# skit-ai/N-Best-ASR-Transformer

Measured on AMD Instinct MI355X. Metric: utterances/sec fine-tune (bert-base, seq128, n_best=5), higher is better.
Workload: dtype bf16

## Files before the change

include/nbest_hip.h:

```cpp
#ifndef NBEST_HIP_H
#define NBEST_HIP_H

#include <stddef.h>
#include <stdint.h>

#ifdef __cplusplus
extern "C" {
#endif

#define NBEST_ABI_VERSION 1

enum { NBEST_OK = 0, NBEST_ERR_ARG = -1, NBEST_ERR_SHAPE = -2, NBEST_ERR_DTYPE = -3, NBEST_ERR_ALIGN = -4,
       NBEST_ERR_LAUNCH = -5, NBEST_ERR_WORKSPACE = -6 };
enum { NBEST_F32 = 0, NBEST_BF16 = 1 };

typedef void* nbest_stream_t;

int nbest_version(void);
int nbest_last_error(char* buf, size_t n);

int nbest_embed_ln_fwd(const int64_t* ids, const int64_t* seg, const int64_t* pos, const void* word,
                       const void* type, const void* ptab, const float* gamma, const float* beta, void* out,
                       float* stats, int64_t M, int H, float eps, int dtype, float drop_p, uint64_t seed,
                       uint32_t drop_stream, nbest_stream_t stream);
// ... 192 lines not shown

int nbest_cls_grad_scatter(const float* dcls, void* dhidden, int B, int S, int H, int dtype,
                           nbest_stream_t stream);

int nbest_stc_decode(const float* top, const float* bott, const nbest_label_space* ls,
                     const uint8_t* none_flag, int32_t* pred, int B, nbest_stream_t stream);
int nbest_stream_stamp(int32_t* flag, int32_t value, nbest_stream_t stream);

typedef struct nbest_tensor_desc {
  int64_t offset;
  int64_t numel;
  float lr;
  float wd;
  int32_t active;
  int32_t block_start;
} nbest_tensor_desc;
int nbest_bertadam_chunk(void);
int nbest_bertadam_step(float* p, float* g, float* m, float* v, void* p_lowp, const nbest_tensor_desc* descs,
                        int n_tensors, int n_blocks, float lr_mult, float b1, float b2, float eps,
                        float max_grad_norm, void* ws, size_t ws_bytes, nbest_stream_t stream);
int nbest_bertadam_norms(const float* g, const nbest_tensor_desc* descs, int n_tensors, int n_blocks, int blk_lo, int blk_hi,
                         float* partial, nbest_stream_t stream);
int nbest_bertadam_update(float* p, const float* g, float* m, float* v, void* p_lowp, const nbest_tensor_desc* descs,
                          int n_tensors, int n_blocks, int blk_lo, int blk_hi, const float* partial, float* coef,
                          float lr_mult, float b1, float b2, float eps, float max_grad_norm, nbest_stream_t stream);
enum { NBEST_ADAM_L2 = 0, NBEST_ADAMW = 1 };
int nbest_adam_clip_coef(const float* partial, int n_partial, float max_grad_norm, float* clip, nbest_stream_t stream);
int nbest_adam_update(int mode, float* p, const float* g, float* m, float* v, void* p_lowp, const nbest_tensor_desc* descs,
                      int n_tensors, int n_blocks, int blk_lo, int blk_hi, const float* clip, float lr_mult, float bc1,
                      float bc2_sqrt, double b1, double b2, float eps, nbest_stream_t stream);
int nbest_adam_step(int mode, float* p, float* g, float* m, float* v, void* p_lowp, const nbest_tensor_desc* descs,
                    int n_tensors, int n_blocks, float lr_mult, float bc1, float bc2_sqrt, double b1, double b2, float eps,
                    float max_grad_norm, void* ws, size_t ws_bytes, nbest_stream_t stream);
int nbest_ema_update(float* ema, const float* p, const nbest_tensor_desc* descs, int n_tensors, int n_blocks,
                     float one_minus_decay, nbest_stream_t stream);
int nbest_ema_exchange(float* p, float* ema, void* p_lowp, const nbest_tensor_desc* descs, int n_tensors, int n_blocks,
                       nbest_stream_t stream);
typedef struct nbest_matrix_desc {
  int64_t offset;
  int32_t rows, cols;
  int32_t tile_start, pad;
} nbest_matrix_desc;
#define NBEST_AMAX_TENSOR_WORDS 1024
int nbest_fp8_amax_fold(void* slots, void* out, int32_t n_tensors, nbest_stream_t stream);
int nbest_quantize_weights_fp8(const float* master, void* w8, void* w8t, const nbest_matrix_desc* descs, int n_matrices,
                               int n_tiles, float* inv_scale, void* ws, size_t ws_bytes, nbest_stream_t stream);
int nbest_transpose_weights(const void* src, void* dst, const nbest_matrix_desc* descs, int n_matrices, int n_tiles,
                            nbest_stream_t stream);
int nbest_pack_bn(int64_t N);
int nbest_pack_bn_fp8(int64_t N, int64_t K);
int nbest_pack_weights_fp8(const void* src, void* dst, const nbest_matrix_desc* descs, int n_matrices, int n_stages, nbest_stream_t stream);
int nbest_pack_weights(const void* src, void* dst, const nbest_matrix_desc* descs, int n_matrices, int n_stages, nbest_stream_t stream);
int nbest_cast_f32_to_bf16(const float* src, void* dst, int64_t n, nbest_stream_t stream);

typedef struct nbest_layer_offsets {
  int64_t wqkv, bqkv, wo, bo, ln1_g, ln1_b, w1, b1, w2, b2, ln2_g, ln2_b;
} nbest_layer_offsets;
typedef struct nbest_encoder_desc {
  int32_t dtype, B, S, H, L, heads, F;
  int32_t vocab, max_pos, n_types;
  float ln_eps, hidden_drop, attn_drop;
  int64_t word_pad_id, pos_pad_id;
  int64_t off_word, off_pos, off_type, off_emb_ln_g, off_emb_ln_b;
  const nbest_layer_offsets* layers_host;
  uint64_t seed;
  uint32_t drop_stream_base;
  int32_t wgrad_events_n;
  void** wgrad_events;
  const void* w8;
  const float* w8_inv_scale;
  const void* w8t;
  const uint32_t* gamax_prev;
  uint32_t* gamax_new;
  int32_t fp8_bwd;
  int32_t pad2;
  const void* wpk;
  const void* wpkt;
  const void* w8p;
  const void* w8tp;
  const int32_t* word_perm;
  const uint32_t* aamax_prev;
  uint32_t* aamax_new;
  int32_t fp8_act;
  int32_t pad4;
  int32_t first_trainable;
  int32_t no_input_grad;
  const uint8_t* wgrad_skip_host;
  const float* head_gate;
  float* head_gate_grad;
  const int64_t* base_ids;
  const float* alpha;
  int32_t no_param_grad;
  int32_t wgrad_group;
} nbest_encoder_desc;
enum { NBEST_WGRAD_GROUP_PLAN = 0, NBEST_WGRAD_GROUP_NEVER = 1, NBEST_WGRAD_GROUP_ALWAYS = 2, NBEST_WGRAD_GROUP_WINDOW = 3 };
size_t nbest_encoder_act_bytes(const nbest_encoder_desc* d);
int nbest_encoder_act_view(const nbest_encoder_desc* d, void* act, int layer, void** qkv, float** lse);
size_t nbest_encoder_ws_bytes(const nbest_encoder_desc* d);
int nbest_encoder_wgrad_launches_per_layer(const nbest_encoder_desc* d);
int nbest_encoder_wgrad_plan(const nbest_encoder_desc* d, int layer_begin, int layer_end, int32_t* out, int cap);
int nbest_encoder_forward(const nbest_encoder_desc* d, const void* wts, const float* prm, const int64_t* ids,
                          const int64_t* seg, const int64_t* pos, const uint8_t* key_mask, void* act,
                          size_t act_bytes, void* ws, size_t ws_bytes, void** hidden_out, nbest_stream_t stream);
int nbest_encoder_backward(const nbest_encoder_desc* d, const void* wts, const void* wts_t, const float* prm, float* grad,
                           const int64_t* ids, const int64_t* seg, const int64_t* pos, const uint8_t* key_mask,
                           void* act, size_t act_bytes, void* dhidden, void* ws, size_t ws_bytes, int accumulate,
                           int layer_begin, int layer_end, int with_embeddings, nbest_stream_t stream);

size_t nbest_encoder_infer_ws_bytes(const nbest_encoder_desc* d);
int nbest_encoder_infer(const nbest_encoder_desc* d, const void* wts, const float* prm, const int64_t* ids, const int64_t* seg,
                        const int64_t* pos, const uint8_t* key_mask, void* ws, size_t ws_bytes, void* cls_out, nbest_stream_t stream);
int nbest_encoder_infer_attn(const nbest_encoder_desc* d, const void* wts, const float* prm, const int64_t* ids, const int64_t* seg,
                             const int64_t* pos, const uint8_t* key_mask, void* ws, size_t ws_bytes, void* cls_out, float* cls_attn,
                             nbest_stream_t stream);

#ifdef __cplusplus
}
#endif
#endif
```

n-best-asr-transformer_amd/csrc/attention.hip:

```cpp
#include "common.h"

namespace {

__device__ __forceinline__ int crow(int reg, int hh) { return (reg & 3) + 8 * (reg >> 2) + 4 * hh; }
__device__ __forceinline__ int gsw(int row) { return ((row >> 2) & 3) | (((row >> 1) & 1) << 2); }

__global__ __launch_bounds__(128) void attn_fwd_f32_kernel(const float* __restrict__ qkv, const uint8_t* __restrict__ mask,
                                                           float* __restrict__ ctx, float* __restrict__ lse, int S, int heads,
                                                           int H, float scale, DropCfg drop) {
  const int bh = blockIdx.x, b = bh / heads, h = bh - b * heads;
  const int i = blockIdx.y * blockDim.x + threadIdx.x;
  if (i >= S) return;
  const int64_t ld = 3 * (int64_t)H;
  const float* base = qkv + (int64_t)b * S * ld;
  const float* qp = base + i * ld + h * 64;
  float q[64];
#pragma unroll
  for (int d = 0; d < 64; ++d) q[d] = qp[d];
  float mx = -INFINITY, l = 0.f;
  for (int j = 0; j < S; ++j) {
    if (!mask[b * S + j]) continue;
    const float* kp = base + j * ld + H + h * 64;
    float s = 0.f;
#pragma unroll
// ... 1017 lines not shown
      for (int r = 0; r < 16; ++r) { ck0 += dk0[r]; ck1 += dk1[r]; cv0 += dv0[r]; cv1 += dv1[r]; }
      const int r0 = key0 + 32 * wave;
      const int64_t goff = ((int64_t)b * S + r0) * ld + h * 64;
      bf16* g = dqkv ? dqkv + goff : nullptr;
      uint8_t* g8 = f8.out8 ? f8.out8 + goff : nullptr;
      store_tile(Kt + wave * 4096, 0, dk0, dk1, lane, g ? g + H : nullptr, ld, S - r0, g8 ? g8 + H : nullptr, s8, amax8, am);
      store_tile(Kt + wave * 4096, 0, dv0, dv1, lane, g ? g + 2 * H : nullptr, ld, S - r0, g8 ? g8 + 2 * H : nullptr, s8, amax8, am);
    }
  }
  __syncthreads();
  if (colpart) {
    float* cs = (float*)dSb;
    float cq0 = 0.f, cq1 = 0.f;
#pragma unroll
    for (int r = 0; r < 16; ++r) { cq0 += dqa0[r] + dqb0[r]; cq1 += dqa1[r] + dqb1[r]; }
    float v6[6] = {cq0, cq1, ck0, ck1, cv0, cv1};
#pragma unroll
    for (int t6 = 0; t6 < 6; ++t6) {
      float x = v6[t6];
      x += __shfl_xor(x, 32, 64);
      if (lane < 32) cs[(wave * 3 + (t6 >> 1)) * 64 + (t6 & 1) * 32 + lane] = x;
    }
    __syncthreads();
    if (tid < 192) {
      const int which = tid >> 6, dcol = tid & 63;
      float x = 0.f;
#pragma unroll
      for (int w2 = 0; w2 < NW; ++w2) x += cs[(w2 * 3 + which) * 64 + dcol];
      colpart[(int64_t)b * 3 * H + which * H + h * 64 + dcol] = x;
    }
  }
  if (wave < nkb) {
    const int r0 = 32 * wave;
    const int64_t goff = ((int64_t)b * S + r0) * ld + h * 64;
    store_tile(Kt + wave * 4096, 0, dqa0, dqa1, lane, dqkv ? dqkv + goff : nullptr, ld, S - r0, f8.out8 ? f8.out8 + goff : nullptr, s8, amax8, am);
  }
  if (wave + 8 < nkb) {
    const int r0 = 32 * (wave + 8);
    const int64_t goff = ((int64_t)b * S + r0) * ld + h * 64;
    store_tile(Kt + wave * 4096, 0, dqb0, dqb1, lane, dqkv ? dqkv + goff : nullptr, ld, S - r0, f8.out8 ? f8.out8 + goff : nullptr, s8, amax8, am);
  }
  if (f8.amax_new) {
    amax8 = wave_max(amax8);
    if (lane == 0) amax_update(f8.amax_new, amax8);
  }
}

static size_t bwd2_lds_bytes(int nkb) {
  const int Sp = nkb * 32;
  return (size_t)Sp * 128 * 4 + (size_t)Sp * 8 + (size_t)nkb * Sp * 4;
}
template <int NKB>
static void launch_bwd2(const bf16* qkv, const uint8_t* mask, const bf16* ctx, const bf16* dctx, const float* lse, bf16* dqkv,
                        float* colpart, int B, int S, int heads, int H, float scale, DropCfg d, hipStream_t st, Fp8Grad f8,
                        const uint32_t* keep) {
  const size_t sm = bwd2_lds_bytes(NKB);
  if (keep && d.thr16) {
    (void)hipFuncSetAttribute((const void*)attn_bwd2_bf16_kernel<NKB, true>, hipFuncAttributeMaxDynamicSharedMemorySize, (int)sm);
    attn_bwd2_bf16_kernel<NKB, true><<<B * heads, (NKB <= 4 ? 4 : 8) * 64, sm, st>>>(qkv, mask, ctx, dctx, lse, dqkv, colpart, S, heads, H, scale, d, f8, keep);
  } else {
    (void)hipFuncSetAttribute((const void*)attn_bwd2_bf16_kernel<NKB, false>, hipFuncAttributeMaxDynamicSharedMemorySize, (int)sm);
    attn_bwd2_bf16_kernel<NKB, false><<<B * heads, (NKB <= 4 ? 4 : 8) * 64, sm, st>>>(qkv, mask, ctx, dctx, lse, dqkv, colpart, S, heads, H, scale, d, f8, nullptr);
  }
}

static size_t fwd_lds_bytes(int nkb) {
  const size_t kv = (size_t)nkb * 32 * 256, madd = (size_t)nkb * 32 * 4;
  return (nkb <= 4) ? kv + madd : kv + madd + 4 * 4096;
}

template <int NKB>
static void launch_fwd(const bf16* qkv, const uint8_t* mask, bf16* ctx, float* lse, int B, int S, int heads, int H, float scale,
                       DropCfg d, hipStream_t st, uint8_t* ctx8, uint32_t* keep, const uint32_t* a_prev, uint32_t* a_new) {
  const size_t sm = fwd_lds_bytes(NKB);
  if (d.thr16) {
    (void)hipFuncSetAttribute((const void*)attn_fwd_bf16_kernel<NKB, true>, hipFuncAttributeMaxDynamicSharedMemorySize, (int)sm);
    attn_fwd_bf16_kernel<NKB, true><<<B * heads, 256, sm, st>>>(qkv, mask, ctx, lse, S, heads, H, scale, d, ctx8, keep, a_prev, a_new);
  } else {
    (void)hipFuncSetAttribute((const void*)attn_fwd_bf16_kernel<NKB, false>, hipFuncAttributeMaxDynamicSharedMemorySize, (int)sm);
    attn_fwd_bf16_kernel<NKB, false><<<B * heads, 256, sm, st>>>(qkv, mask, ctx, lse, S, heads, H, scale, d, ctx8, keep, a_prev, a_new);
  }
}

template <typename T, bool PROBS>
__global__ __launch_bounds__(256) void attn_cls_fwd_kernel(const T* __restrict__ q, int64_t ldq, const T* __restrict__ kv, int64_t ldkv,
                                                           const uint8_t* __restrict__ mask, T* __restrict__ ctx, int64_t ldctx, int S,
                                                           int heads, int H, float scale, float* __restrict__ probs, int64_t ldp) {
  constexpr bool kF32 = sizeof(T) == 4;
  constexpr int VEC = 16 / (int)sizeof(T);
  constexpr int LPK = 64 / VEC;
  constexpr int KPP = 256 / LPK;
  __shared__ float sc[512];
  __shared__ float qs[64];
  __shared__ float part[KPP][65];
  __shared__ float red[8];
  const int tid = threadIdx.x, sub = tid % LPK, kg = tid / LPK, lane = tid & 63, wave = tid >> 6;
  const int bh = blockIdx.x, b = bh / heads, h = bh - b * heads;
  auto load = [](const T* p, float* v) {
    if constexpr (kF32) {
      const f32x4 x = *(const f32x4*)p;
#pragma unroll
      for (int e = 0; e < 4; ++e) v[e] = x[e];
    } else {
      const bf16x8 x = __builtin_bit_cast(bf16x8, *(const i32x4*)p);
#pragma unroll
      for (int e = 0; e < 8; ++e) v[e] = (float)x[e];
    }
  };
  if (tid < 64) qs[tid] = (float)q[(int64_t)b * ldq + h * 64 + tid];
  __syncthreads();
  const T* kbase = kv + (int64_t)b * S * ldkv + h * 64;
  const T* vbase = kbase + H;
  const uint8_t* mk = mask + (int64_t)b * S;
  const bool log2u = !kF32 && S <= 256;
  const float sf = log2u ? scale * 1.4426950408889634f : scale;
  float mloc = -INFINITY;
  for (int j = tid; j < S; j += 256) {
    const T* kp = kbase + (int64_t)j * ldkv;
    float d = 0.f;
#pragma unroll
    for (int c = 0; c < 64; c += VEC) {
      float kr[VEC];
      load(kp + c, kr);
#pragma unroll
      for (int e = 0; e < VEC; ++e) d = fmaf(qs[c + e], kr[e], d);
    }
    const float sv = mk[j] ? d * sf : -INFINITY;
    sc[j] = sv;
    mloc = fmaxf(mloc, sv);
  }
  mloc = wave_max(mloc);
  if (lane == 0) red[wave] = mloc;
  __syncthreads();
  const float mx = fmaxf(fmaxf(red[0], red[1]), fmaxf(red[2], red[3]));
  const float mxs = (mx == -INFINITY) ? 0.f : mx;
  auto ex = [&](float v) { return log2u ? __builtin_amdgcn_exp2f(v - mxs) : (kF32 ? expf(v - mxs) : __expf(v - mxs)); };
  float sum = 0.f;
  for (int j = tid; j < S; j += 256) sum += ex(sc[j]);
  sum = wave_sum(sum);
  if (lane == 0) red[4 + wave] = sum;
  __syncthreads();
  sum = (red[4] + red[5]) + (red[6] + red[7]);
  const float lse = mxs + logf(sum), inv = 1.0f / sum;
  if constexpr (PROBS) {
    float* pr = probs + (int64_t)bh * ldp;
    for (int j = tid; j < S; j += 256) {
      const float v = sc[j];
      pr[j] = (v == -INFINITY) ? 0.f : (kF32 ? expf(v - lse) : ex(v) * inv);
    }
    return;
  }
  for (int j = tid; j < S; j += 256) {
    const float v = sc[j];
    sc[j] = kF32 ? (v == -INFINITY ? 0.f : expf(v - lse)) : (float)(bf16)(ex(v) * inv);
  }
  __syncthreads();
  float o[VEC];
#pragma unroll
  for (int e = 0; e < VEC; ++e) o[e] = 0.f;
#pragma unroll 4
  for (int j = kg; j < S; j += KPP) {
    float vr[VEC];
    load(vbase + (int64_t)j * ldkv + sub * VEC, vr);
    const float pv = sc[j];
#pragma unroll
    for (int e = 0; e < VEC; ++e) o[e] = fmaf(pv, vr[e], o[e]);
  }
#pragma unroll
  for (int e = 0; e < VEC; ++e) part[kg][sub * VEC + e] = o[e];
  __syncthreads();
  if (tid < 64) {
    float acc = 0.f;
#pragma unroll
    for (int g = 0; g < KPP; ++g) acc += part[g][tid];
    T* op = ctx + (int64_t)b * ldctx + h * 64 + tid;
    if constexpr (kF32) *op = acc;
    else *op = (bf16)acc;
  }
}

template <bool VEC>
__global__ __launch_bounds__(256) void attn_probs_bf16_kernel(const bf16* __restrict__ qkv, const uint8_t* __restrict__ mask,
                                                              const float* __restrict__ lse, float* __restrict__ probs, int S,
                                                              int heads, int H, float scale) {
  constexpr int LDI = 68;
  __shared__ __attribute__((aligned(16))) float img[4][16 * LDI];
  const int tid = threadIdx.x, lane = tid & 63, wave = tid >> 6, c = lane & 15, g = lane >> 4;
  const int bh = blockIdx.x, b = bh / heads, h = bh - b * heads;
  const int q0 = 64 * blockIdx.y + 16 * wave;
  if (q0 >= S) return;
  const int64_t ld = 3 * (int64_t)H;
  const bf16* base = qkv + (int64_t)b * S * ld;
  const uint8_t* mk = mask + (int64_t)b * S;
  float* im = img[wave];
  const int qrow = q0 + c;
  bf16x8 qf[2];
#pragma unroll
  for (int ks = 0; ks < 2; ++ks) {
    const i32x4 raw = (qrow < S) ? *(const i32x4*)(base + (int64_t)qrow * ld + h * 64 + 32 * ks + 8 * g) : i32x4{0, 0, 0, 0};
    qf[ks] = __builtin_bit_cast(bf16x8, raw);
  }
  const float lq = (qrow < S) ? lse[(int64_t)bh * S + qrow] : 0.f;
  float* out = probs + (int64_t)bh * S * S;
  const int nkb = (S + 63) / 64;
  for (int kb = 0; kb < nkb; ++kb) {
    f32x4 acc[4];
#pragma unroll
    for (int t = 0; t < 4; ++t) {
      const int key = 64 * kb + 16 * t + c;
      acc[t] = f32x4{0.f, 0.f, 0.f, 0.f};
#pragma unroll
      for (int ks = 0; ks < 2; ++ks) {
        const i32x4 raw = (key < S) ? *(const i32x4*)(base + (int64_t)key * ld + H + h * 64 + 32 * ks + 8 * g) : i32x4{0, 0, 0, 0};
        acc[t] = __builtin_amdgcn_mfma_f32_16x16x32_bf16(__builtin_bit_cast(bf16x8, raw), qf[ks], acc[t], 0, 0, 0);
      }
    }
#pragma unroll
    for (int t = 0; t < 4; ++t) {
      f32x4 p;
#pragma unroll
      for (int r = 0; r < 4; ++r) {
        const int key = 64 * kb + 16 * t + 4 * g + r;
        p[r] = (key < S && mk[key]) ? expf(acc[t][r] * scale - lq) : 0.f;
      }
      *(f32x4*)(im + c * LDI + 16 * t + 4 * g) = p;
    }
    asm volatile("s_waitcnt lgkmcnt(0)" ::: "memory");
#pragma unroll
    for (int i = 0; i < 4; ++i) {
      const int row = 4 * i + g, q = q0 + row, key = 64 * kb + 4 * c;
      const f32x4 v = *(const f32x4*)(im + row * LDI + 4 * c);
      if (q < S && key < S) {
        float* dst = out + (int64_t)q * S + key;
        if (VEC) {
          *(f32x4*)dst = v;
        } else {
#pragma unroll
          for (int e = 0; e < 4; ++e)
            if (key + e < S) dst[e] = v[e];
        }
      }
    }
    asm volatile("s_waitcnt lgkmcnt(0)" ::: "memory");
  }
}

template <bool VEC>
__global__ __launch_bounds__(256) void attn_probs_f32_kernel(const float* __restrict__ qkv, const uint8_t* __restrict__ mask,
                                                             const float* __restrict__ lse, float* __restrict__ probs, int S, int heads,
                                                             int H, float scale) {
  const int bh = blockIdx.x, b = bh / heads, h = bh - b * heads;
  const int n4 = (S + 3) / 4;
  const int idx = blockIdx.y * 256 + threadIdx.x;
  if (idx >= S * n4) return;
  const int i = idx / n4, j0 = 4 * (idx - i * n4);
  const int64_t ld = 3 * (int64_t)H;
  const float* base = qkv + (int64_t)b * S * ld;
  const float* qp = base + i * ld + h * 64;
  float q[64];
#pragma unroll
  for (int d = 0; d < 64; d += 4) {
    const f32x4 x = *(const f32x4*)(qp + d);
    q[d] = x[0]; q[d + 1] = x[1]; q[d + 2] = x[2]; q[d + 3] = x[3];
  }
  const float lse_i = lse[(int64_t)bh * S + i];
  f32x4 p;
#pragma unroll
  for (int e = 0; e < 4; ++e) {
    const int j = j0 + e;
    float pv = 0.f;
    if (j < S && mask[b * S + j]) {
      const float* kp = base + j * ld + H + h * 64;
      float s = 0.f;
#pragma unroll
      for (int d = 0; d < 64; ++d) s = fmaf(q[d], kp[d], s);
      pv = expf(s * scale - lse_i);
    }
    p[e] = pv;
  }
  float* dst = probs + ((int64_t)bh * S + i) * S + j0;
  if (VEC) {
    *(f32x4*)dst = p;
  } else {
#pragma unroll
    for (int e = 0; e < 4; ++e)
      if (j0 + e < S) dst[e] = p[e];
  }
}

static int check_common(const char* who, int B, int S, int heads, int d, int dtype) {
  NB_CHECK(B > 0 && S > 0 && heads > 0, NBEST_ERR_SHAPE, "%s: bad shape", who);
  NB_CHECK(d == 64, NBEST_ERR_SHAPE, "%s: head dimension %d not supported (64 only)", who, d);
  NB_CHECK(dtype == NBEST_F32 || dtype == NBEST_BF16, NBEST_ERR_DTYPE, "%s: bad dtype %d", who, dtype);
  NB_CHECK((int64_t)B * heads * S * S < ((int64_t)1 << 32), NBEST_ERR_SHAPE, "%s: B*heads*S*S overflows the dropout counter", who);
  return NBEST_OK;
}

}

size_t nbest_internal_attention_keep_bytes(int B, int S, int heads) {
  const size_t nkb = (size_t)(S + 31) / 32;
  return (S <= 256) ? (size_t)B * heads * nkb * nkb * 32 * sizeof(uint32_t) : 0;
}
int nbest_internal_attention_fwd8(const void* qkv, const uint8_t* key_mask, void* ctx, void* ctx8, float* lse, int B, int S, int heads,
                                  int d, int dtype, float drop_p, uint64_t seed, uint32_t drop_stream, nbest_stream_t stream,
                                  uint32_t* keep, const uint32_t* a_prev, uint32_t* a_new) {
  NB_CHECK(qkv && key_mask && ctx && lse, NBEST_ERR_ARG, "attention_fwd: null pointer");
  if (int e = check_common("attention_fwd", B, S, heads, d, dtype)) return e;
  hipStream_t st = (hipStream_t)stream;
  const int H = heads * d;
  const float scale = 1.0f / sqrtf((float)d);
  const DropCfg dc = make_drop(drop_p, seed, drop_stream);
  if (dtype == NBEST_F32) {
    NB_CHECK(S <= 512, NBEST_ERR_SHAPE, "attention_fwd(f32): S=%d > 512", S);
    attn_fwd_f32_kernel<<<dim3(B * heads, (S + 127) / 128), 128, 0, st>>>((const float*)qkv, key_mask, (float*)ctx, lse, S, heads, H, scale, dc);
  } else {
    NB_CHECK(S <= 512, NBEST_ERR_SHAPE, "attention_fwd(bf16): S=%d > 512", S);
    NB_CHECK((int64_t)S * 3 * H * 2 < ((int64_t)1 << 31), NBEST_ERR_SHAPE, "attention_fwd: sequence too large");
    const int nkb = (S + 31) / 32;
    if (nkb > 8) {
      const size_t sm = fwd_lds_bytes(nkb);
      (void)hipFuncSetAttribute((const void*)attn_fwd_long_bf16_kernel, hipFuncAttributeMaxDynamicSharedMemorySize, (int)sm);
      attn_fwd_long_bf16_kernel<<<B * heads, 256, sm, st>>>((const bf16*)qkv, key_mask, (bf16*)ctx, lse, S, nkb, heads, H, scale, dc, (uint8_t*)ctx8, a_prev, a_new);
      NB_LAUNCH_CHECK();
      return NBEST_OK;
    }
#define F(N) case N: launch_fwd<N>((const bf16*)qkv, key_mask, (bf16*)ctx, lse, B, S, heads, H, scale, dc, st, (uint8_t*)ctx8, keep, a_prev, a_new); break;
    switch (nkb) { F(1) F(2) F(3) F(4) F(5) F(6) F(7) F(8) }
#undef F
  }
  NB_LAUNCH_CHECK();
  return NBEST_OK;
}

extern "C" int nbest_attention_fwd(const void* qkv, const uint8_t* key_mask, void* ctx, float* lse, int B, int S, int heads,
                                   int d, int dtype, float drop_p, uint64_t seed, uint32_t drop_stream, nbest_stream_t stream) {
  return nbest_internal_attention_fwd8(qkv, key_mask, ctx, nullptr, lse, B, S, heads, d, dtype, drop_p, seed, drop_stream, stream, nullptr, nullptr, nullptr);
}

int nbest_attention_cls_fwd_internal(const void* q, int64_t ldq, const void* kv, int64_t ldkv, const uint8_t* key_mask, void* ctx,
                                     int64_t ldctx, int B, int S, int heads, int d, int dtype, nbest_stream_t stream) {
  NB_CHECK(q && kv && key_mask && ctx, NBEST_ERR_ARG, "attention_cls_fwd: null pointer");
  NB_CHECK(B > 0 && S > 0 && heads > 0, NBEST_ERR_SHAPE, "attention_cls_fwd: bad shape");
  NB_CHECK(d == 64, NBEST_ERR_SHAPE, "attention_cls_fwd: head dimension %d not supported (64 only)", d);
  NB_CHECK(dtype == NBEST_F32 || dtype == NBEST_BF16, NBEST_ERR_DTYPE, "attention_cls_fwd: bad dtype %d", dtype);
  NB_CHECK(S <= 512, NBEST_ERR_SHAPE, "attention_cls_fwd: S=%d > 512", S);
  const int H = heads * d;
  const int vec = dtype == NBEST_BF16 ? 8 : 4;
  NB_CHECK(ldq >= H && ldkv >= 2 * H && ldctx >= H && ldq % vec == 0 && ldkv % vec == 0, NBEST_ERR_ALIGN,
           "attention_cls_fwd: leading dimensions must cover the heads and be multiples of %d elements", vec);
  NB_CHECK(((uintptr_t)q & 15) == 0 && ((uintptr_t)kv & 15) == 0, NBEST_ERR_ALIGN, "attention_cls_fwd: q and kv must be 16-byte aligned");
  const float scale = 1.0f / sqrtf((float)d);
  hipStream_t st = (hipStream_t)stream;
  if (dtype == NBEST_F32)
    attn_cls_fwd_kernel<float, false><<<B * heads, 256, 0, st>>>((const float*)q, ldq, (const float*)kv, ldkv, key_mask, (float*)ctx, ldctx, S,
                                                                 heads, H, scale, nullptr, 0);
  else
    attn_cls_fwd_kernel<bf16, false><<<B * heads, 256, 0, st>>>((const bf16*)q, ldq, (const bf16*)kv, ldkv, key_mask, (bf16*)ctx, ldctx, S,
                                                                heads, H, scale, nullptr, 0);
  NB_LAUNCH_CHECK();
  return NBEST_OK;
}

extern "C" int nbest_attention_cls_fwd(const void* q, int64_t ldq, const void* kv, int64_t ldkv, const uint8_t* key_mask, void* ctx,
                                       int64_t ldctx, int B, int S, int heads, int d, int dtype, nbest_stream_t stream) {
  return nbest_attention_cls_fwd_internal(q, ldq, kv, ldkv, key_mask, ctx, ldctx, B, S, heads, d, dtype, stream);
}

extern "C" int nbest_attention_probs(const void* qkv, const uint8_t* key_mask, const float* lse, float* probs, int B, int S, int heads,
                                     int d, int dtype, nbest_stream_t stream) {
  NB_CHECK(qkv && key_mask && lse && probs, NBEST_ERR_ARG, "attention_probs: null pointer");
  if (int e = check_common("attention_probs", B, S, heads, d, dtype)) return e;
  NB_CHECK(S <= 512, NBEST_ERR_SHAPE, "attention_probs: S=%d > 512", S);
  NB_CHECK(((uintptr_t)qkv & 15) == 0, NBEST_ERR_ALIGN, "attention_probs: qkv must be 16-byte aligned");
  hipStream_t st = (hipStream_t)stream;
  const int H = heads * d;
  const float scale = 1.0f / sqrtf((float)d);
  const bool vec = (S % 4) == 0 && ((uintptr_t)probs & 15) == 0;
  if (dtype == NBEST_F32) {
    const dim3 grid(B * heads, (S * ((S + 3) / 4) + 255) / 256);
    if (vec) attn_probs_f32_kernel<true><<<grid, 256, 0, st>>>((const float*)qkv, key_mask, lse, probs, S, heads, H, scale);
    else attn_probs_f32_kernel<false><<<grid, 256, 0, st>>>((const float*)qkv, key_mask, lse, probs, S, heads, H, scale);
  } else {
    const dim3 grid(B * heads, (S + 63) / 64);
    if (vec) attn_probs_bf16_kernel<true><<<grid, 256, 0, st>>>((const bf16*)qkv, key_mask, lse, probs, S, heads, H, scale);
    else attn_probs_bf16_kernel<false><<<grid, 256, 0, st>>>((const bf16*)qkv, key_mask, lse, probs, S, heads, H, scale);
  }
  NB_LAUNCH_CHECK();
  return NBEST_OK;
}

int nbest_internal_attention_cls_probs(const void* q, int64_t ldq, const void* kv, int64_t ldkv, const uint8_t* key_mask, float* probs,
                                       int64_t ldp, int B, int S, int heads, int d, int dtype, nbest_stream_t stream) {
  NB_CHECK(q && kv && key_mask && probs, NBEST_ERR_ARG, "attention_cls_probs: null pointer");
  NB_CHECK(B > 0 && S > 0 && heads > 0, NBEST_ERR_SHAPE, "attention_cls_probs: bad shape");
  NB_CHECK(d == 64, NBEST_ERR_SHAPE, "attention_cls_probs: head dimension %d not supported (64 only)", d);
  NB_CHECK(dtype == NBEST_F32 || dtype == NBEST_BF16, NBEST_ERR_DTYPE, "attention_cls_probs: bad dtype %d", dtype);
  NB_CHECK(S <= 512, NBEST_ERR_SHAPE, "attention_cls_probs: S=%d > 512", S);
  const int H = heads * d;
  const int vec = dtype == NBEST_BF16 ? 8 : 4;
  NB_CHECK(ldq >= H && ldkv >= 2 * H && ldp >= S && ldq % vec == 0 && ldkv % vec == 0, NBEST_ERR_ALIGN,
           "attention_cls_probs: leading dimensions must cover the heads / keys and be multiples of %d elements", vec);
  NB_CHECK(((uintptr_t)q & 15) == 0 && ((uintptr_t)kv & 15) == 0, NBEST_ERR_ALIGN, "attention_cls_probs: q and kv must be 16-byte aligned");
  const float scale = 1.0f / sqrtf((float)d);
  hipStream_t st = (hipStream_t)stream;
  if (dtype == NBEST_F32)
    attn_cls_fwd_kernel<float, true><<<B * heads, 256, 0, st>>>((const float*)q, ldq, (const float*)kv, ldkv, key_mask, nullptr, 0, S,
                                                                heads, H, scale, probs, ldp);
  else
    attn_cls_fwd_kernel<bf16, true><<<B * heads, 256, 0, st>>>((const bf16*)q, ldq, (const bf16*)kv, ldkv, key_mask, nullptr, 0, S,
                                                               heads, H, scale, probs, ldp);
  NB_LAUNCH_CHECK();
  return NBEST_OK;
}

extern "C" int nbest_attention_cls_probs(const void* q, int64_t ldq, const void* kv, int64_t ldkv, const uint8_t* key_mask, float* probs,
                                         int64_t ldp, int B, int S, int heads, int d, int dtype, nbest_stream_t stream) {
  return nbest_internal_attention_cls_probs(q, ldq, kv, ldkv, key_mask, probs, ldp, B, S, heads, d, dtype, stream);
}

extern "C" size_t nbest_attention_bwd_ws_bytes(int B, int S, int heads) {
  const size_t a = (size_t)B * 3 * heads * 64 * sizeof(float);
  const size_t b = nbest_rowred_ws_bytes((int64_t)B * S, (int64_t)3 * heads * 64);
  return a > b ? a : b;
}

int nbest_internal_attention_bwd8(const void* qkv, const uint8_t* key_mask, const void* ctx, const void* dctx, const float* lse,
                                  void* dqkv, float* dbias, int accumulate, void* ws, size_t ws_bytes, int B, int S, int heads,
                                  int d, int dtype, float drop_p, uint64_t seed, uint32_t drop_stream, nbest_stream_t stream, Fp8Grad f8,
                                  const uint32_t* keep) {
  NB_CHECK(qkv && key_mask && ctx && dctx && lse && (dqkv || (f8.out8 && dtype == NBEST_BF16)), NBEST_ERR_ARG, "attention_bwd: null pointer");
  if (int e = check_common("attention_bwd", B, S, heads, d, dtype)) return e;
  NB_CHECK(!dbias || (ws && ws_bytes >= nbest_attention_bwd_ws_bytes(B, S, heads)), NBEST_ERR_WORKSPACE,
           "attention_bwd: bias-gradient workspace too small");
  hipStream_t st = (hipStream_t)stream;
  const int H = heads * d;
  const float scale = 1.0f / sqrtf((float)d);
  const DropCfg dc = make_drop(drop_p, seed, drop_stream);
  if (dtype == NBEST_F32) {
    NB_CHECK(S <= 512, NBEST_ERR_SHAPE, "attention_bwd(f32): S=%d > 512", S);
    attn_bwd_f32_kernel<<<dim3(B * heads, (S + 127) / 128), 128, 0, st>>>((const float*)qkv, key_mask, (const float*)ctx,
                                                                          (const float*)dctx, lse, (float*)dqkv, S, heads, H, scale, dc);
    NB_LAUNCH_CHECK();
    attn_bwd_f32_kv_kernel<<<dim3(B * heads, (S + 127) / 128), 128, 0, st>>>((const float*)qkv, key_mask, (const float*)ctx,
                                                                             (const float*)dctx, lse, (float*)dqkv, S, heads, H, scale, dc);
    NB_LAUNCH_CHECK();
    if (dbias) return nbest_colsum(dqkv, dbias, (int64_t)B * S, 3 * H, 3 * H, NBEST_F32, accumulate, ws, ws_bytes, stream);
    return NBEST_OK;
  }
  NB_CHECK(S <= 512, NBEST_ERR_SHAPE, "attention_bwd(bf16): S=%d > 512", S);
  const int nkb = (S + 31) / 32;
  float* colpart = dbias ? (float*)ws : nullptr;
  if (nkb > 8) {
    const size_t sm = (size_t)2 * 4096 * 2 + 256 * 128 + 2 * 32 * 512 + (size_t)nkb * 32 * 8;
    (void)hipFuncSetAttribute((const void*)attn_bwd_long_bf16_kernel, hipFuncAttributeMaxDynamicSharedMemorySize, (int)sm);
    attn_bwd_long_bf16_kernel<<<B * heads, 512, sm, st>>>((const bf16*)qkv, key_mask, (const bf16*)ctx, (const bf16*)dctx, lse,
                                                         (bf16*)dqkv, colpart, S, nkb, heads, H, scale, dc, f8);
    NB_LAUNCH_CHECK();
    if (dbias) return nbest_internal_partial_rows_sum(colpart, B, 3 * H, dbias, accumulate, st);
    return NBEST_OK;
  }
  if (nkb == 4) {
    const size_t sm = bwd2_lds_bytes(4);
#define G(K_)                                                                                                                           \
    do {                                                                                                                                \
      (void)hipFuncSetAttribute((const void*)attn_bwd3_bf16_kernel<4, K_>, hipFuncAttributeMaxDynamicSharedMemorySize, (int)sm);        \
      attn_bwd3_bf16_kernel<4, K_><<<B * heads, 4 * 128, sm, st>>>((const bf16*)qkv, key_mask, (const bf16*)ctx, (const bf16*)dctx, lse, \
                                                                   (bf16*)dqkv, colpart, S, heads, H, scale, dc, f8, K_ ? keep : nullptr); \
    } while (0)
    if (keep && dc.thr16) G(true); else G(false);
#undef G
  } else {
#define F(N) case N: launch_bwd2<N>((const bf16*)qkv, key_mask, (const bf16*)ctx, (const bf16*)dctx, lse, (bf16*)dqkv, colpart, B, S, heads, H, scale, dc, st, f8, keep); break;
    switch (nkb) { F(1) F(2) F(3) F(5) F(6) F(7) F(8) }
#undef F
  }
  NB_LAUNCH_CHECK();
  if (dbias) return nbest_internal_partial_rows_sum(colpart, B, 3 * H, dbias, accumulate, st);
  return NBEST_OK;
}

extern "C" int nbest_attention_bwd(const void* qkv, const uint8_t* key_mask, const void* ctx, const void* dctx, const float* lse,
                                   void* dqkv, float* dbias, int accumulate, void* ws, size_t ws_bytes, int B, int S, int heads,
                                   int d, int dtype, float drop_p, uint64_t seed, uint32_t drop_stream, nbest_stream_t stream) {
  return nbest_internal_attention_bwd8(qkv, key_mask, ctx, dctx, lse, dqkv, dbias, accumulate, ws, ws_bytes, B, S, heads, d, dtype, drop_p,
                                       seed, drop_stream, stream, Fp8Grad{nullptr, nullptr, nullptr}, nullptr);
}

extern "C" size_t nbest_attention_keep_bytes(int B, int S, int heads) { return nbest_internal_attention_keep_bytes(B, S, heads); }
extern "C" int nbest_attention_fwd_keep(const void* qkv, const uint8_t* key_mask, void* ctx, float* lse, int B, int S, int heads,
                                        int d, int dtype, float drop_p, uint64_t seed, uint32_t drop_stream, void* keep,
                                        nbest_stream_t stream) {
  const bool ok = keep && dtype == NBEST_BF16 && nbest_internal_attention_keep_bytes(B, S, heads) > 0;
  return nbest_internal_attention_fwd8(qkv, key_mask, ctx, nullptr, lse, B, S, heads, d, dtype, drop_p, seed, drop_stream, stream,
// ... 11 lines not shown
```

n-best-asr-transformer_amd/csrc/encoder.hip:

```cpp
#include <algorithm>
#include <vector>

#include "common.h"

namespace {

static inline size_t al(size_t x) { return (x + 255) & ~(size_t)255; }
static inline size_t take(size_t& o, size_t bytes) { const size_t at = o; o += bytes; return at; }

struct Sizes {
  size_t esz, MH, MF, M3H, MH8, MF8, st, lse;
  int64_t M;
};

static Sizes sizes(const nbest_encoder_desc* d) {
  Sizes z;
  z.esz = d->dtype == NBEST_BF16 ? 2 : 4;
  z.M = (int64_t)d->B * d->S;
  const size_t MHe = (size_t)z.M * d->H, MFe = (size_t)z.M * d->F;
  z.MH = al(MHe * z.esz); z.MF = al(MFe * z.esz); z.M3H = al(3 * MHe * z.esz);
  z.MH8 = al(MHe); z.MF8 = al(MFe);
  z.st = al((size_t)z.M * 2 * sizeof(float));
  z.lse = al((size_t)d->B * d->heads * d->S * sizeof(float));
  return z;
// ... 104 lines not shown
  }
  std::vector<WinEntry> q;
  size_t head = 0;
  int64_t pending = 0;
  auto emit = [&](int after) {
    WinLaunch w = {};
    w.after_layer = after;
    while (head < q.size() && w.tiles < kWinTiles && w.n < kWinEntries) {
      WinEntry& f = q[head];
      const int c = std::min(f.count, kWinTiles - w.tiles);
      w.e[w.n++] = WinEntry{f.layer, f.j, f.first, c};
      w.tiles += c; f.first += c; f.count -= c; pending -= c;
      if (f.count == 0) ++head;
    }
    wp.launches.push_back(w);
  };
  for (int l = layer_end - 1; l >= layer_begin; --l) {
    const int n_live = head < q.size() ? q[head].layer - l : 0;
    wp.max_live = std::max(wp.max_live, n_live);
    if (n_live >= sets)
      while (pending > 0) emit(l + 1);
    for (int j = 0; j < 4; ++j)
      if (live(l, j) && !(l == wp.peel_layer && j < 2)) { q.push_back(WinEntry{l, j, 0, t[j]}); pending += t[j]; }
    while (pending >= kWinTiles) emit(l);
  }
  while (pending > 0) emit(layer_begin);
  return wp;
}
static bool window_shapes_ok(const nbest_encoder_desc* d) {
  if (d->dtype != NBEST_BF16 || d->w8 || d->H % 256 || d->F % 256) return false;
  return (4 * (int64_t)d->H * d->H + 2 * (int64_t)d->H * d->F) / (256 * 256) <= kWinTiles;
}
struct WindowModel { int sets; double us; };
static WindowModel window_model(const nbest_encoder_desc* d) {
  const int64_t H = d->H, M = (int64_t)d->B * d->S;
  const WinPlan wp = window_plan(d, first_trainable(d), d->L, nullptr, false, true, kMaxSets);
  const double round = kWgA + kWgB * (double)((M + 31) / 32);
  double us = 0.0;
  if (wp.peel_layer >= 0) us = wgrad_paired(d, false) ? wgrad_splitk_us(4 * H, H, M) : wgrad_splitk_us(3 * H, H, M) + wgrad_splitk_us(H, H, M);
  for (const WinLaunch& w : wp.launches) us += round * (w.tiles > 216 ? kWgFull : 1.0);
  return WindowModel{std::min(wp.max_live + 1, kMaxSets), us};
}

struct WgradMode { int mode, gl, sets; };
static WgradMode wgrad_mode(const nbest_encoder_desc* d) {
  const WgradMode never = {NBEST_WGRAD_GROUP_NEVER, 0, 0};
  if (d->wgrad_group == NBEST_WGRAD_GROUP_NEVER) return never;
  if (d->dtype != NBEST_BF16 || d->w8 || d->H % 256 || d->F % 256) return never;
  const int64_t H = d->H, F = d->F, M = (int64_t)d->B * d->S;
  const int64_t tiles = (4 * H * H + 2 * H * F) / (256 * 256);
  if (d->wgrad_group == NBEST_WGRAD_GROUP_ALWAYS) return WgradMode{NBEST_WGRAD_GROUP_ALWAYS, 2 * tiles <= 256 ? 2 : 1, 0};
  if (d->wgrad_group == NBEST_WGRAD_GROUP_WINDOW)
    return window_shapes_ok(d) ? WgradMode{NBEST_WGRAD_GROUP_WINDOW, 0, window_model(d).sets} : never;
  const int nl = d->L - first_trainable(d);
  const double today = wgrad_splitk_us(4 * H, H, M) + wgrad_splitk_us(F, H, M) + wgrad_splitk_us(H, F, M);
  const double round = kWgA + kWgB * (double)((M + 31) / 32);
  if (window_shapes_ok(d) && nl > 0) {
    const int gl = 2 * tiles <= 256 ? 2 : 1;
    const WindowModel wm = window_model(d);
    if (wm.us < 0.95 * std::min(today * nl, round * ((nl + gl - 1) / gl))) return WgradMode{NBEST_WGRAD_GROUP_WINDOW, 0, wm.sets};
  }
  if (2 * tiles > 256 || !wgrad_paired(d, false)) return never;
  return round / 2.0 < 0.95 * today ? WgradMode{NBEST_WGRAD_GROUP_ALWAYS, 2, 0} : never;
}
static WsLayout ws_layout(const nbest_encoder_desc* d, const Sizes& z, const WgradMode& wm) {
  WsLayout w;
  const int64_t M = z.M;
  size_t o = 0;
  w.dR = take(o, z.MH); w.dRd = take(o, z.MH); w.dB1 = take(o, z.MH); w.dctx = take(o, z.MH);
  w.dBig = take(o, z.MF); w.dqkv = take(o, z.M3H);
  static_assert(sizeof(w.gset) / sizeof(w.gset[0]) == kMaxSets, "one row per buffer set");
  for (int s = 0; s < kMaxSets; ++s) { w.gset[s][0] = w.dRd; w.gset[s][1] = w.dBig; w.gset[s][2] = w.dRd; w.gset[s][3] = w.dqkv; }
  const int n_sets = wm.gl + wm.sets;
  if (n_sets > 0) {
    w.gset[0][2] = take(o, z.MH);
    for (int s = 1; s < n_sets; ++s) { w.gset[s][0] = take(o, z.MH); w.gset[s][1] = take(o, z.MF); w.gset[s][2] = take(o, z.MH); w.gset[s][3] = take(o, z.M3H); }
  }
  const int64_t maxN = d->F > 3 * d->H ? d->F : 3 * d->H;
  w.red_bytes = al(nbest_rowred_ws_bytes(M, maxN));
  w.red_bytes = std::max(w.red_bytes, al(nbest_attention_bwd_ws_bytes(d->B, d->S, d->heads)));
  w.red_bytes = std::max(w.red_bytes, al((size_t)((M + 127) / 128) * 2 * d->F * sizeof(float)));
  w.red = take(o, 4 * w.red_bytes);
  w.slab_bytes = al(max_splitk_bytes(d, M));
  w.slab = take(o, w.slab_bytes);
  w.emb_bytes = al(nbest_embed_bwd_ws_bytes(M, d->H));
  w.emb = take(o, w.emb_bytes);
  w.f8_bytes = (d->dtype == NBEST_BF16) ? 4 * z.MH8 + z.MF8 : 0;
  w.f8 = take(o, w.f8_bytes);
  w.fz_x0 = w.fz_x1 = w.fz_emb_stats = w.fz_lse = w.fz_st1 = w.fz_st2 = w.fz_u = o;
  if (first_trainable(d) > 0) {
    w.fz_x0 = take(o, z.MH); w.fz_x1 = take(o, z.MH); w.fz_emb_stats = take(o, z.st);
    w.fz_lse = take(o, z.lse); w.fz_st1 = take(o, z.st); w.fz_st2 = take(o, z.st);
    w.fz_u = take(o, d->w8 ? z.MF8 : 0);
  }
  w.total = o;
  return w;
}

static bool fp8_forward_active(const nbest_encoder_desc* d) {
  return d->dtype == NBEST_BF16 && d->w8 && d->w8_inv_scale && d->fp8_act && d->aamax_prev;
}
static bool fp8_backward_active(const nbest_encoder_desc* d) {
  return fp8_forward_active(d) && d->fp8_bwd && d->w8t && d->gamax_prev && d->gamax_new;
}

static int check_desc(const nbest_encoder_desc* d) {
  NB_CHECK(d && d->layers_host, NBEST_ERR_ARG, "encoder: null descriptor");
  NB_CHECK(d->dtype == NBEST_F32 || d->dtype == NBEST_BF16, NBEST_ERR_DTYPE, "encoder: bad dtype %d", d->dtype);
  NB_CHECK(d->B > 0 && d->S > 0 && d->L > 0 && d->heads > 0, NBEST_ERR_SHAPE, "encoder: bad shape");
  NB_CHECK(d->H == d->heads * 64, NBEST_ERR_SHAPE, "encoder: hidden %d != heads %d x 64", d->H, d->heads);
  NB_CHECK(d->S + (d->pos_pad_id >= 0 ? (int)d->pos_pad_id + 1 : 0) <= d->max_pos, NBEST_ERR_SHAPE,
           "encoder: S=%d does not fit the position table (%d rows)", d->S, d->max_pos);
  NB_CHECK(d->S <= 512, NBEST_ERR_SHAPE, "encoder: S=%d > 512", d->S);
  if (d->dtype == NBEST_BF16)
    NB_CHECK(d->H % 128 == 0 && d->F % 128 == 0, NBEST_ERR_SHAPE, "encoder(bf16): H and F must be multiples of 128");
  if (d->w8) NB_CHECK(d->dtype == NBEST_BF16 && d->w8_inv_scale && d->H % 256 == 0 && d->H <= 1024 && d->F % 256 == 0, NBEST_ERR_SHAPE,
                      "encoder(fp8 forward): needs the bf16 path, inverse scales and H, F multiples of 256");
  NB_CHECK(0 <= d->first_trainable && d->first_trainable <= d->L, NBEST_ERR_ARG, "encoder: first_trainable %d outside [0, L=%d]",
           d->first_trainable, d->L);
  NB_CHECK(!d->base_ids == !d->alpha, NBEST_ERR_ARG, "encoder: interpolated embeddings need both base_ids and alpha (or neither)");
  NB_CHECK(!d->head_gate || !d->w8, NBEST_ERR_ARG, "encoder: head_gate is not supported with the fp8 forward (desc.w8)");
  NB_CHECK(!d->head_gate || d->first_trainable == 0, NBEST_ERR_ARG, "encoder: head_gate needs first_trainable == 0 (got %d)", d->first_trainable);
  NB_CHECK(!d->head_gate_grad || d->head_gate, NBEST_ERR_ARG, "encoder: head_gate_grad without head_gate");
  return NBEST_OK;
}

struct Ptrs {
  const char* wts;
  const float* prm;
  size_t esz;
  const void* W(int64_t off) const { return wts + (size_t)off * esz; }
  const float* P(int64_t off) const { return prm + off; }
};

#define RUN(x) do { int rc__ = (x); if (rc__) return rc__; } while (0)

static nbest_gemm_args gemm_nt(int dtype, const void* A, const void* B, void* C, int64_t M, int64_t N, int64_t K) {
  nbest_gemm_args g = {};
  g.A = A; g.B = B; g.C = C; g.dtype = dtype;
  g.M = M; g.N = N; g.K = K; g.lda = K; g.ldb = K; g.ldc = N;
  return g;
}

static void use_packed(nbest_gemm_args& g, const void* arena, int64_t off) {
  if (!arena || g.dtype != NBEST_BF16 || g.trans_a || g.trans_b) return;
  g.B_packed = (const char*)arena + off * 2;
  g.b_pack_bn = nbest_pack_bn(g.N);
}
static void use_packed(nbest_gemm_fp8_args& g, const void* arena, int64_t off) {
  if (!arena) return;
  g.B_packed = (const uint8_t*)arena + off;
  g.b_pack_bn = nbest_pack_bn_fp8(g.N, g.K);
}

struct GemmPass {
  int dtype; int64_t M; nbest_stream_t stream;
  uint64_t seed;
  Ptrs W; const void* packed; bool b_kn;
  bool fp8; const void *w8, *w8_packed; const float* inv_scale; const uint32_t* amax_prev; uint32_t* amax_new;
  void* colsum_ws; size_t colsum_ws_bytes; int accumulate;
};
struct GemmOp {
  const void* A; const uint8_t* A8; int a_idx;
  int64_t w_off; int mat;
  void* C; int64_t N, K; int epilogue;
  const float* bias;
  const void* R; float drop_p; uint32_t drop_stream;
  void* U; float* colsum;
  uint8_t* C8; int c_idx;
};

static int layer_gemm(const GemmPass& c, const GemmOp& o) {
  if (c.fp8) {
    nbest_gemm_fp8_args g = {};
    g.A = o.A8; g.B = (const uint8_t*)c.w8 + o.w_off; g.C = o.C; g.bias = o.bias; g.R = o.R; g.U = o.U; g.C8 = o.C8;
    g.M = c.M; g.N = o.N; g.K = o.K;
    g.lda = g.ldb = o.K; g.ldc = g.ldr = g.ldu = g.ldc8 = o.N;
    use_packed(g, c.w8_packed, o.w_off);
    g.epilogue = o.epilogue; g.out_scale = 1.f; g.out_scale_dev = c.inv_scale + o.mat;
    g.drop_p = o.drop_p; g.drop_stream = o.drop_stream; g.seed = c.seed;
    g.a_amax = c.amax_prev + o.a_idx;
    if (o.C8) {
      g.c8_amax_prev = c.amax_prev + o.c_idx;
      g.c8_amax_new = c.amax_new ? c.amax_new + (int64_t)o.c_idx * NBEST_AMAX_TENSOR_WORDS : nullptr;
    }
    g.colsum_out = o.colsum; g.colsum_accumulate = c.accumulate; g.ws = c.colsum_ws; g.ws_bytes = c.colsum_ws_bytes;
    return nbest_gemm_fp8(&g, c.stream);
  }
  nbest_gemm_args g = gemm_nt(c.dtype, o.A, c.W.W(o.w_off), o.C, c.M, o.N, o.K);
  if (c.b_kn) { g.trans_b = 1; g.ldb = o.N; }
  g.epilogue = o.epilogue; g.bias = o.bias;
  if (o.R) { g.R = o.R; g.ldr = o.N; }
  if (o.epilogue == NBEST_EPI_BIAS_DROP_RES) { g.drop_p = o.drop_p; g.drop_stream = o.drop_stream; g.seed = c.seed; }
  if (o.epilogue == NBEST_EPI_BIAS_GELU || o.epilogue == NBEST_EPI_DGELU) { g.U = o.U; g.ldu = o.N; }
  if (o.epilogue == NBEST_EPI_DGELU) {
    g.colsum_out = o.colsum; g.colsum_accumulate = g.accumulate = c.accumulate; g.ws = c.colsum_ws; g.ws_bytes = c.colsum_ws_bytes;
  }
  use_packed(g, c.packed, o.w_off);
  return nbest_gemm(&g, c.stream);
}

struct LayerBufs {
  void *qkv, *ctx, *r1, *x1, *u, *hact, *r2;
  float *lse, *st1, *st2;
  uint32_t* keep;
  uint8_t *x8, *ctx8, *x18, *h8;
};
// ... 8 lines not shown
  if (a.keep_bytes && d->attn_drop > 0.f) b.keep = (uint32_t*)(Lb + a.o_keep);
  if (fp8_forward_active(d)) {
    b.x8 = (uint8_t*)(Lb + a.o_x8); b.ctx8 = (uint8_t*)(Lb + a.o_ctx8);
    b.x18 = (uint8_t*)(Lb + a.o_x18); b.h8 = (uint8_t*)(Lb + a.o_h8);
  }
  return b;
}

static LayerBufs frozen_layer(const nbest_encoder_desc* d, const WsLayout& w, const Sizes& z, void* ws) {
  char* W = (char*)ws;
  const bool f8 = fp8_forward_active(d);
  LayerBufs b = {};
  b.qkv = W + w.dqkv; b.ctx = W + w.dctx; b.lse = (float*)(W + w.fz_lse);
  b.r1 = W + w.dR; b.st1 = (float*)(W + w.fz_st1); b.x1 = W + w.dRd;
  b.r2 = W + w.dB1; b.st2 = (float*)(W + w.fz_st2);
  b.u = f8 ? W + w.fz_u : nullptr; b.hact = f8 ? nullptr : W + w.dBig;
  if (f8) { b.x8 = (uint8_t*)(W + w.f8); b.ctx8 = b.x8 + z.MH8; b.x18 = b.ctx8 + z.MH8; b.h8 = b.x18 + z.MH8; }
  return b;
}

struct Fwd {
  const nbest_encoder_desc* d;
  GemmPass g;
  const uint8_t* key_mask;
  bool arec;
  void* gated_ctx;
  const uint32_t* AP(int idx) const { return g.fp8 ? d->aamax_prev + idx : nullptr; }
  uint32_t* AN(int idx) const { return (g.fp8 && arec) ? d->aamax_new + (int64_t)idx * NBEST_AMAX_TENSOR_WORDS : nullptr; }
  int calib(const void* t, int64_t n, int idx) const {
    if (!arec || g.fp8) return NBEST_OK;
    return nbest_internal_amax_bf16(t, n, d->aamax_new + (int64_t)idx * NBEST_AMAX_TENSOR_WORDS, (hipStream_t)g.stream);
  }
};

static Fwd make_fwd(const nbest_encoder_desc* d, const void* wts, const float* prm, const Sizes& z, const uint8_t* key_mask,
                    nbest_stream_t stream) {
  const GemmPass g = {d->dtype, z.M, stream, d->seed, Ptrs{(const char*)wts, prm, z.esz}, d->wpk, false, fp8_forward_active(d),
                      d->w8, d->w8p, d->w8_inv_scale, d->aamax_prev, d->aamax_new, nullptr, 0, 0};
  return Fwd{d, g, key_mask, d->w8 && d->aamax_new && d->dtype == NBEST_BF16, nullptr};
}

static int layer_forward(const Fwd& c, int l, const void* xin, void* xout, const LayerBufs& b, uint8_t* x8_next, float* cls_probs) {
  const nbest_encoder_desc* d = c.d;
  const nbest_layer_offsets& o = d->layers_host[l];
  const Ptrs& P = c.g.W;
  const nbest_stream_t stream = c.g.stream;
  const int64_t M = c.g.M;
  const int H = d->H, F = d->F, dt = d->dtype, t = 4 * l;
  const uint32_t s0 = d->drop_stream_base + 1 + 4 * l;
  if (c.g.fp8 && l == 0)
    RUN(nbest_internal_cast_bf16_to_fp8(xin, b.x8, M * H, c.AP(0), c.AN(0), (hipStream_t)stream));
  const GemmOp wqkv = {xin, b.x8, t + 0, o.wqkv, t + 0, b.qkv, 3 * H, H, NBEST_EPI_BIAS, P.P(o.bqkv)};
  RUN(layer_gemm(c.g, wqkv));
  if (cls_probs)
    RUN(nbest_internal_attention_cls_probs(b.qkv, (int64_t)d->S * H * 3, (const char*)b.qkv + H * P.esz, 3 * H, c.key_mask, cls_probs, d->S,
                                           d->B, d->S, d->heads, 64, dt, stream));
  RUN(c.calib(xin, M * H, t + 0));
  RUN(nbest_internal_attention_fwd8(b.qkv, c.key_mask, b.ctx, b.ctx8, b.lse, d->B, d->S, d->heads, 64, dt, d->attn_drop, d->seed, s0 + 0,
                                    stream, b.keep, c.AP(t + 1), c.AN(t + 1)));
  RUN(c.calib(b.ctx, M * H, t + 1));
  const void* ctx = b.ctx;
  if (d->head_gate) {
    void* gated = c.gated_ctx ? c.gated_ctx : b.ctx;
    RUN(nbest_head_gate_fwd(b.ctx, H, gated, H, d->head_gate + (int64_t)l * d->heads, M, d->heads, 64, dt, stream));
    ctx = gated;
  }
  GemmOp wo = {ctx, b.ctx8, t + 1, o.wo, t + 1, b.r1, H, H, NBEST_EPI_BIAS_DROP_RES, P.P(o.bo)};
  wo.R = xin; wo.drop_p = d->hidden_drop; wo.drop_stream = s0 + 1;
  RUN(layer_gemm(c.g, wo));
  RUN(nbest_internal_layernorm_fwd8(b.r1, P.P(o.ln1_g), P.P(o.ln1_b), b.x1, b.x18, b.st1, M, H, d->ln_eps, dt, stream, c.AP(t + 2), c.AN(t + 2)));
  RUN(c.calib(b.x1, M * H, t + 2));
  GemmOp w1 = {b.x1, b.x18, t + 2, o.w1, t + 2, b.hact, F, H, NBEST_EPI_BIAS_GELU, P.P(o.b1)};
  w1.U = b.u; w1.C8 = b.h8; w1.c_idx = t + 3;
  RUN(layer_gemm(c.g, w1));
  GemmOp w2 = {b.hact, b.h8, t + 3, o.w2, t + 3, b.r2, H, F, NBEST_EPI_BIAS_DROP_RES, P.P(o.b2)};
  w2.R = b.x1; w2.drop_p = d->hidden_drop; w2.drop_stream = s0 + 2;
  RUN(layer_gemm(c.g, w2));
  RUN(c.calib(b.hact, M * F, t + 3));
  RUN(nbest_internal_layernorm_fwd8(b.r2, P.P(o.ln2_g), P.P(o.ln2_b), xout, x8_next, b.st2, M, H, d->ln_eps, dt, stream,
                                    x8_next ? c.AP(t + 4) : nullptr, x8_next ? c.AN(t + 4) : nullptr));
  return NBEST_OK;
}

}

extern "C" size_t nbest_encoder_act_bytes(const nbest_encoder_desc* d) { return d ? act_layout(d, sizes(d)).total : 0; }

extern "C" int nbest_encoder_act_view(const nbest_encoder_desc* d, void* act, int layer, void** qkv, float** lse) {
  RUN(check_desc(d));
  NB_CHECK(act && qkv && lse, NBEST_ERR_ARG, "encoder_act_view: null pointer");
  NB_CHECK(0 <= layer && layer < d->L, NBEST_ERR_ARG, "encoder_act_view: layer %d outside [0, L=%d)", layer, d->L);
  const ActLayout a = act_layout(d, sizes(d));
  NB_CHECK(layer >= a.K, NBEST_ERR_ARG, "encoder_act_view: layer %d < first_trainable %d (frozen layers are not stashed)", layer, a.K);
  const LayerBufs b = stashed_layer(d, a, act, layer);
  *qkv = b.qkv; *lse = b.lse;
  return NBEST_OK;
}
extern "C" size_t nbest_encoder_ws_bytes(const nbest_encoder_desc* d) { return d ? ws_layout(d, sizes(d), wgrad_mode(d)).total : 0; }
extern "C" int nbest_encoder_wgrad_launches_per_layer(const nbest_encoder_desc* d) {
  if (!d) return 0;
  const WgradMode wm = wgrad_mode(d);
  if (wm.gl > 0 || wm.sets > 0) return 1;
  return wgrad_paired(d, fp8_backward_active(d)) ? 3 : 4;
}

extern "C" int nbest_encoder_wgrad_plan(const nbest_encoder_desc* d, int layer_begin, int layer_end, int32_t* out, int cap) {
  NB_CHECK(d && d->B > 0 && d->S > 0 && d->L > 0 && d->H > 0 && d->F > 0, NBEST_ERR_ARG, "encoder_wgrad_plan: bad descriptor");
  NB_CHECK(first_trainable(d) <= layer_begin && layer_begin <= layer_end && layer_end <= d->L, NBEST_ERR_ARG, "encoder_wgrad_plan: bad layer range");
  NB_CHECK(out || cap <= 0, NBEST_ERR_ARG, "encoder_wgrad_plan: null pointer");
  const WgradMode wm = wgrad_mode(d);
  std::vector<int32_t> v = {wm.mode, wm.gl + wm.sets, -1, 0};
  if (wm.sets > 0) {
    const WinPlan wp = window_plan(d, layer_begin, layer_end, d->wgrad_skip_host, d->no_param_grad != 0, true, wm.sets);
    v[2] = wp.peel_layer; v[3] = (int32_t)wp.launches.size();
    for (const WinLaunch& w : wp.launches) {
      v.insert(v.end(), {w.after_layer, w.tiles, w.n});
      for (int i = 0; i < w.n; ++i) v.insert(v.end(), {w.e[i].layer, w.e[i].j, w.e[i].first, w.e[i].count});
    }
  }
  if ((int)v.size() <= cap) std::copy(v.begin(), v.end(), out);
  return (int)v.size();
}

extern "C" int nbest_encoder_forward(const nbest_encoder_desc* d, const void* wts, const float* prm, const int64_t* ids,
                                     const int64_t* seg, const int64_t* pos, const uint8_t* key_mask, void* act, size_t act_bytes,
                                     void* ws, size_t ws_bytes, void** hidden_out, nbest_stream_t stream) {
  RUN(check_desc(d));
  NB_CHECK(wts && prm && ids && pos && key_mask && act, NBEST_ERR_ARG, "encoder_forward: null pointer");
  const Sizes z = sizes(d);
  const ActLayout a = act_layout(d, z);
  NB_CHECK(act_bytes >= a.total, NBEST_ERR_WORKSPACE, "encoder_forward: activation stash too small (%zu < %zu)", act_bytes, a.total);
  Fwd c = make_fwd(d, wts, prm, z, key_mask, stream);
  const WsLayout wl = ws_layout(d, z, wgrad_mode(d));
  const int FT = a.K;
  if (c.g.fp8 || FT > 0 || d->head_gate)
    NB_CHECK(ws && ws_bytes >= wl.total, NBEST_ERR_WORKSPACE, "encoder_forward(%s): workspace too small (%zu < %zu)",
             FT > 0 ? "first_trainable > 0" : d->head_gate ? "head_gate" : "fp8", ws_bytes, wl.total);
  if (d->head_gate) c.gated_ctx = (char*)ws + wl.dctx;
  const Ptrs& P = c.g.W;
  char *A = (char*)act, *W = (char*)ws;
  const int H = d->H, dt = d->dtype;
  auto X = [&](int l) { return l >= FT ? (void*)(A + a.X + (size_t)(l - FT) * z.MH) : (void*)(W + ((l & 1) ? wl.fz_x1 : wl.fz_x0)); };
  auto bufs = [&](int l) { return l >= FT ? stashed_layer(d, a, act, l) : frozen_layer(d, wl, z, ws); };

  float* emb_stats = (float*)(FT > 0 ? W + wl.fz_emb_stats : A + a.emb_stats);
  if (d->base_ids)
    RUN(nbest_embed_ln_fwd_interp(ids, d->base_ids, d->alpha, seg, pos, P.W(d->off_word), P.W(d->off_type), P.W(d->off_pos),
                                  P.P(d->off_emb_ln_g), P.P(d->off_emb_ln_b), X(0), emb_stats, d->B, d->S, H, d->ln_eps, dt,
                                  d->hidden_drop, d->seed, d->drop_stream_base, (hipStream_t)stream));
  else
    RUN(nbest_embed_ln_fwd(ids, seg, pos, P.W(d->off_word), P.W(d->off_type), P.W(d->off_pos), P.P(d->off_emb_ln_g),
                           P.P(d->off_emb_ln_b), X(0), emb_stats, z.M, H, d->ln_eps, dt, d->hidden_drop, d->seed, d->drop_stream_base,
                           (hipStream_t)stream));
  for (int l = 0; l < d->L; ++l) {
    uint8_t* x8_next = (l + 1 < d->L) ? bufs(l + 1).x8 : nullptr;
    RUN(layer_forward(c, l, X(l), X(l + 1), bufs(l), x8_next, nullptr));
  }
  if (hidden_out) *hidden_out = X(d->L);
  return NBEST_OK;
}

namespace {
struct WGrad {
  const void *dY, *X;
  const uint8_t *dY8, *X8;
  int64_t w_off, rows, cols;
  int g_idx, a_idx;
};
}

extern "C" int nbest_encoder_backward(const nbest_encoder_desc* d, const void* wts, const void* wts_t, const float* prm, float* grad,
                                      const int64_t* ids, const int64_t* seg, const int64_t* pos, const uint8_t* key_mask,
                                      void* act, size_t act_bytes, void* dhidden, void* ws, size_t ws_bytes, int accumulate,
                                      int layer_begin, int layer_end, int with_embeddings, nbest_stream_t stream) {
  RUN(check_desc(d));
  NB_CHECK(0 <= layer_begin && layer_begin <= layer_end && layer_end <= d->L, NBEST_ERR_ARG, "encoder_backward: bad layer range");
  const bool npg = d->no_param_grad != 0;
  NB_CHECK(!npg || (!with_embeddings && d->first_trainable == 0 && !d->no_input_grad && !d->w8), NBEST_ERR_ARG,
           "encoder_backward: no_param_grad refuses with_embeddings (%d), first_trainable > 0 (%d), no_input_grad (%d) and the fp8 "
           "forward (w8): it forms the input gradient only, of a full stash", with_embeddings, d->first_trainable, d->no_input_grad);
  NB_CHECK(!d->head_gate || npg, NBEST_ERR_ARG, "encoder_backward: head_gate needs no_param_grad (the attention-output weight gradient would "
           "need the gated context, which the forward does not keep)");
  NB_CHECK(wts && prm && (grad || npg) && ids && pos && key_mask && act && dhidden && ws, NBEST_ERR_ARG, "encoder_backward: null pointer");
  NB_CHECK(!with_embeddings || d->word_perm, NBEST_ERR_ARG, "encoder_backward: desc.word_perm (stable argsort of this pass's ids) is required");
  NB_CHECK(layer_begin >= d->first_trainable, NBEST_ERR_ARG, "encoder_backward: layer_begin %d < first_trainable %d (those layers are not stashed)",
           layer_begin, d->first_trainable);
  NB_CHECK(!with_embeddings || (d->first_trainable == 0 && !d->no_input_grad), NBEST_ERR_ARG,
           "encoder_backward: with_embeddings needs first_trainable == 0 and no_input_grad == 0");
  const Sizes z = sizes(d);
  const ActLayout a = act_layout(d, z);
  const WgradMode wm = wgrad_mode(d);
  const WsLayout w = ws_layout(d, z, wm);
  NB_CHECK(act_bytes >= a.total, NBEST_ERR_WORKSPACE, "encoder_backward: activation stash too small");
  NB_CHECK(ws_bytes >= w.total, NBEST_ERR_WORKSPACE, "encoder_backward: workspace too small (%zu < %zu)", ws_bytes, w.total);
  hipStream_t st = (hipStream_t)stream;
  const Ptrs P{(const char*)wts, prm, z.esz};
  const bool wt = (wts_t != nullptr);
  char *A = (char*)act, *W = (char*)ws;
  const int64_t M = z.M;
  const int H = d->H, F = d->F, dt = d->dtype;
  const int FT = a.K;
  auto X = [&](int l) { return (void*)(A + a.X + (size_t)(l - FT) * z.MH); };
  auto G = [&](int64_t off) { return grad + off; };
  auto GP = [&](int64_t off) -> float* { return npg ? nullptr : grad + off; };
  auto skip = [&](int l, int j) -> bool { return npg || (d->wgrad_skip_host && d->wgrad_skip_host[4 * l + j]); };
  void* dA = dhidden; void* dR = W + w.dR;
  const bool hdrop = d->hidden_drop > 0.f;
  void* dRd = hdrop ? (void*)(W + w.dRd) : dR;
  void* dB1 = W + w.dB1; void* dctx = W + w.dctx; void* dBig = W + w.dBig; void* dqkv = W + w.dqkv;
  void* red = W + w.red; void* slab = W + w.slab;
  void* red1 = W + w.red + w.red_bytes; void* red2 = W + w.red + 2 * w.red_bytes; void* red3 = W + w.red + 3 * w.red_bytes;
  const bool f8b = fp8_backward_active(d);
  const bool paired = wgrad_paired(d, f8b);
  const int gl = wm.gl;
  const bool grouped = gl > 0, window = wm.sets > 0, deferred = grouped || window;
  int ev_i = (deferred ? 1 : paired ? 3 : 4) * (d->L - layer_end);
  auto stamp = [&](int which) {
    if (d->wgrad_events && 2 * ev_i + which < d->wgrad_events_n) (void)hipEventRecord((hipEvent_t)d->wgrad_events[2 * ev_i + which], st);
    ev_i += which;
  };

  const bool rec = !npg && d->gamax_new && dt == NBEST_BF16;
  uint8_t* dqkv8 = f8b ? (uint8_t*)W + w.f8 : nullptr;
  uint8_t* dBig8 = f8b ? dqkv8 + 3 * z.MH8 : nullptr;
  uint8_t* dRd8 = f8b ? dBig8 + z.MF8 : nullptr;
  auto GN = [&](int idx) { return d->gamax_new + (int64_t)idx * NBEST_AMAX_TENSOR_WORDS; };
  auto fg = [&](uint8_t* out8, int idx) -> Fp8Grad {
    if (!rec) return Fp8Grad{nullptr, nullptr, nullptr};
    return Fp8Grad{f8b ? out8 : nullptr, f8b ? d->gamax_prev + idx : nullptr, GN(idx)};
  };
  const GemmPass dg = {dt, M, stream, 0, Ptrs{(const char*)(wt ? wts_t : wts), prm, z.esz}, wt ? d->wpkt : nullptr, !wt, f8b,
                       d->w8t, d->w8tp, d->w8_inv_scale, d->gamax_prev, d->gamax_new, red1, w.red_bytes, accumulate};
  auto wgrad_args_of = [&](const WGrad* x) {
    nbest_gemm_args g = wgrad_args(dt, x->rows, x->cols, M);
    g.A = x->dY; g.B = x->X; g.C = G(x->w_off); g.accumulate = accumulate;
    return g;
  };
  auto wgrad_launch = [&](int l, const WGrad* wg, int j, int j2) -> int {
    const WGrad* p = skip(l, j) ? nullptr : wg + j;
    const WGrad* q = (j2 >= 0 && !skip(l, j2)) ? wg + j2 : nullptr;
    if (!p) { p = q; q = nullptr; }
    if (p && f8b) {
      const uint32_t *gp = d->gamax_prev, *ap = d->aamax_prev;
      if (q)
        RUN(nbest_wgrad_fp8_pair(p->dY8, p->X8, G(p->w_off), p->rows, p->rows, p->cols, p->cols, gp + p->g_idx, ap + p->a_idx, q->dY8, q->X8,
                                 G(q->w_off), q->rows, q->rows, q->cols, q->cols, gp + q->g_idx, ap + q->a_idx, p->cols, M, accumulate, slab,
                                 w.slab_bytes, stream));
      else
        RUN(nbest_wgrad_fp8(p->dY8, p->X8, G(p->w_off), p->rows, p->cols, M, p->rows, p->cols, p->cols, gp + p->g_idx, ap + p->a_idx,
                            accumulate, slab, w.slab_bytes, stream));
    } else if (p) {
      nbest_gemm_args g1 = wgrad_args_of(p), g2 = wgrad_args_of(q ? q : p);
      g1.ws = slab; g1.ws_bytes = w.slab_bytes;
      RUN(q ? nbest_wgrad_pair(&g1, &g2, stream) : nbest_gemm(&g1, stream));
    }
    return NBEST_OK;
  };
  auto wgrad = [&](int l, const WGrad* wg, int j, int j2) -> int {
    stamp(0);
    RUN(wgrad_launch(l, wg, j, j2));
    stamp(1);
    return NBEST_OK;
  };
  nbest_gemm_args pend[8];
  int n_pend = 0;
  const int nl = layer_end - layer_begin;
  WinPlan wp;
  std::vector<nbest_gemm_args> wargs;
  if (window) {
    wp = window_plan(d, layer_begin, layer_end, d->wgrad_skip_host, npg, true, wm.sets);
    wargs.resize((size_t)4 * nl);
  }
  size_t wi = 0;
  int pairs_used = 0;
  bool pair_open = false;
  auto pair_begin = [&] { if (!pair_open && pairs_used < nl) { stamp(0); pair_open = true; } };
  auto pair_end = [&] { if (pair_open) { stamp(1); ++pairs_used; pair_open = false; } };

  struct BatchGuard { ~BatchGuard() { nbest_internal_rowred_batch_abort(); } } batch_guard;
  for (int l = layer_end - 1; l >= layer_begin; --l) {
    const nbest_layer_offsets& o = d->layers_host[l];
    const LayerBufs b = stashed_layer(d, a, act, l);
    const bool input_grad = !(d->no_input_grad && l == FT);
    const int t = 4 * l;
    const uint32_t s0 = d->drop_stream_base + 1 + 4 * l;
    const int gpos = grouped ? (layer_end - 1 - l) % gl : window ? (layer_end - 1 - l) % wm.sets : 0;
    const bool group_ends = grouped && (gpos == gl - 1 || l == layer_begin);
    void *dR2 = dR, *dR1 = dR, *dRd2 = dRd, *dRd1 = dRd, *dBigL = dBig, *dqkvL = dqkv;
    if (deferred) {
      dRd2 = W + w.gset[gpos][0]; dBigL = W + w.gset[gpos][1]; dRd1 = W + w.gset[gpos][2]; dqkvL = W + w.gset[gpos][3];
      if (!hdrop) { dR2 = dRd2; dR1 = dRd1; }
    }
    const WGrad wg[4] = {{dqkvL, X(l), dqkv8, b.x8, o.wqkv, 3 * H, H, t + 3, t + 0},
                         {dRd1, b.ctx, dRd8, b.ctx8, o.wo, H, H, t + 2, t + 1},
                         {dBigL, b.x1, dBig8, b.x18, o.w1, F, H, t + 1, t + 2},
                         {dRd2, b.hact, dRd8, b.h8, o.w2, H, F, t + 0, t + 3}};
    if (!npg) nbest_internal_rowred_batch_begin();
    RUN(nbest_internal_layernorm_bwd8(dA, b.r2, b.st2, P.P(o.ln2_g), dR2, (hdrop && !f8b) ? dRd2 : nullptr, GP(o.ln2_g), GP(o.ln2_b), GP(o.b2), M, H,
                                      dt, accumulate, d->hidden_drop, d->seed, s0 + 2, red, w.red_bytes, stream, fg(dRd8, t + 0)));
    GemmOp dw2 = {dRd2, dRd8, t + 0, o.w2, t + 3, f8b ? nullptr : dBigL, F, H, NBEST_EPI_DGELU};
    dw2.U = b.u; dw2.colsum = GP(o.b1); dw2.C8 = dBig8; dw2.c_idx = t + 1;
    RUN(layer_gemm(dg, dw2));
    if (rec && !f8b) RUN(nbest_internal_amax_bf16(dBigL, M * F, GN(t + 1), st));
    if (!deferred) RUN(wgrad(l, wg, 3, -1));
    GemmOp dw1 = {dBigL, dBig8, t + 1, o.w1, t + 2, dB1, H, F, NBEST_EPI_RES};
    dw1.R = dR2;
    RUN(layer_gemm(dg, dw1));
    if (!deferred) RUN(wgrad(l, wg, 2, -1));
    RUN(nbest_internal_layernorm_bwd8(dB1, b.r1, b.st1, P.P(o.ln1_g), dR1, (hdrop && !f8b) ? dRd1 : nullptr, GP(o.ln1_g), GP(o.ln1_b), GP(o.bo), M, H,
                                      dt, accumulate, d->hidden_drop, d->seed, s0 + 1, red2, w.red_bytes, stream, fg(dRd8, t + 2)));
    const GemmOp dwo = {dRd1, dRd8, t + 2, o.wo, t + 1, dctx, H, H, NBEST_EPI_NONE};
    RUN(layer_gemm(dg, dwo));
    if (!paired && !deferred) RUN(wgrad(l, wg, 1, -1));
    if (d->head_gate)
      RUN(nbest_head_gate_bwd(b.ctx, dctx, d->head_gate + (int64_t)l * d->heads,
                              d->head_gate_grad ? d->head_gate_grad + (int64_t)l * d->B * d->heads : nullptr, d->B, d->S, d->heads, 64, dt, stream));
    RUN(nbest_internal_attention_bwd8(b.qkv, key_mask, b.ctx, dctx, b.lse, f8b ? nullptr : dqkvL, GP(o.bqkv), accumulate, red3, w.red_bytes, d->B, d->S,
                                      d->heads, 64, dt, d->attn_drop, d->seed, s0 + 0, stream, fg(dqkv8, t + 3), b.keep));
    if (input_grad) {
      GemmOp dwqkv = {dqkvL, dqkv8, t + 3, o.wqkv, t + 0, dA, H, 3 * H, NBEST_EPI_RES};
      dwqkv.R = dR1;
      RUN(layer_gemm(dg, dwqkv));
    }
    if (window) {
      for (int j = 0; j < 4; ++j)
        if (!skip(l, j)) wargs[(size_t)4 * (layer_end - 1 - l) + j] = wgrad_args_of(wg + j);
      if (l == wp.peel_layer) {
        pair_begin();
        if (!paired) RUN(wgrad_launch(l, wg, 1, -1));
        RUN(wgrad_launch(l, wg, 0, paired ? 1 : -1));
      }
      for (; wi < wp.launches.size() && wp.launches[wi].after_layer == l; ++wi) {
        const WinLaunch& wl = wp.launches[wi];
        nbest_gemm_args tab[kWinEntries];
        int32_t first[kWinEntries], count[kWinEntries];
        for (int i = 0; i < wl.n; ++i) {
          tab[i] = wargs[(size_t)4 * (layer_end - 1 - wl.e[i].layer) + wl.e[i].j];
          first[i] = wl.e[i].first; count[i] = wl.e[i].count;
        }
        pair_begin();
        RUN(nbest_wgrad_window(tab, first, count, wl.n, stream));
        pair_end();
      }
      pair_end();
      if (l == layer_begin)
        for (; pairs_used < nl; ++pairs_used) { stamp(0); stamp(1); }
    } else if (!grouped) {
      RUN(wgrad(l, wg, 0, paired ? 1 : -1));
    } else if (group_ends && gpos + 1 < gl && d->wgrad_group != NBEST_WGRAD_GROUP_ALWAYS) {
      stamp(0);
      RUN(wgrad_launch(l, wg, 3, -1));
      RUN(wgrad_launch(l, wg, 2, -1));
      if (!paired) RUN(wgrad_launch(l, wg, 1, -1));
      RUN(wgrad_launch(l, wg, 0, paired ? 1 : -1));
      stamp(1);
    } else {
      for (int j = 0; j < 4; ++j)
        if (!skip(l, j)) pend[n_pend++] = wgrad_args_of(wg + j);
      if (group_ends) {
        stamp(0);
        if (n_pend) RUN(nbest_wgrad_group(pend, n_pend, stream));
        stamp(1);
        for (int i = 0; i < gpos; ++i) { stamp(0); stamp(1); }
        n_pend = 0;
      }
    }
    if (!npg) RUN(nbest_internal_rowred_batch_flush(st));
  }
  if (!with_embeddings) return NBEST_OK;
  if (!accumulate) {
    hipError_t e = hipMemsetAsync(G(d->off_word), 0, (size_t)d->vocab * H * sizeof(float), st);
    if (e == hipSuccess) e = hipMemsetAsync(G(d->off_pos), 0, (size_t)d->max_pos * H * sizeof(float), st);
    if (e == hipSuccess) e = hipMemsetAsync(G(d->off_type), 0, (size_t)d->n_types * H * sizeof(float), st);
    NB_CHECK(e == hipSuccess, NBEST_ERR_LAUNCH, "encoder_backward: memset failed: %s", hipGetErrorString(e));
  }
  RUN(nbest_embed_ln_bwd(ids, seg, pos, d->word_perm, P.W(d->off_word), P.W(d->off_type), P.W(d->off_pos), P.P(d->off_emb_ln_g),
                         (const float*)(A + a.emb_stats), dA, G(d->off_word), G(d->off_type), G(d->off_pos), G(d->off_emb_ln_g),
                         G(d->off_emb_ln_b), d->B, d->S, H, d->n_types, dt, d->word_pad_id, d->pos_pad_id, accumulate, accumulate,
                         d->hidden_drop, d->seed, d->drop_stream_base, W + w.emb, w.emb_bytes, stream));
  return NBEST_OK;
}

namespace {
struct InferLayout {
  size_t X0, X1, emb_stats, qkv, ctx, r1, x1, r2, hact, lse, st1, st2, total;
};
static InferLayout infer_layout(const Sizes& z) {
  InferLayout w;
  size_t o = 0;
  w.X0 = take(o, z.MH); w.X1 = take(o, z.MH); w.emb_stats = take(o, z.st);
  w.qkv = take(o, z.M3H); w.ctx = take(o, z.MH); w.r1 = take(o, z.MH); w.x1 = take(o, z.MH); w.r2 = take(o, z.MH);
  w.hact = take(o, z.MF); w.lse = take(o, z.lse); w.st1 = take(o, z.st); w.st2 = take(o, z.st);
  w.total = o;
  return w;
}
static LayerBufs infer_layer(const InferLayout& w, void* ws) {
  char* W = (char*)ws;
  LayerBufs b = {};
  b.qkv = W + w.qkv; b.ctx = W + w.ctx; b.lse = (float*)(W + w.lse);
  b.r1 = W + w.r1; b.st1 = (float*)(W + w.st1); b.x1 = W + w.x1;
  b.hact = W + w.hact; b.r2 = W + w.r2; b.st2 = (float*)(W + w.st2);
  return b;
}
}

extern "C" size_t nbest_encoder_infer_ws_bytes(const nbest_encoder_desc* d) { return d ? infer_layout(sizes(d)).total : 0; }

extern "C" int nbest_encoder_infer_attn(const nbest_encoder_desc* d, const void* wts, const float* prm, const int64_t* ids, const int64_t* seg,
                                        const int64_t* pos, const uint8_t* key_mask, void* ws, size_t ws_bytes, void* cls_out,
                                        float* cls_attn, nbest_stream_t stream) {
  RUN(check_desc(d));
  NB_CHECK(d->hidden_drop == 0.f && d->attn_drop == 0.f, NBEST_ERR_ARG,
           "encoder_infer: dropout must be 0 (hidden_drop=%g, attn_drop=%g): inference has no dropout", d->hidden_drop, d->attn_drop);
  NB_CHECK(!d->w8, NBEST_ERR_ARG, "encoder_infer: the fp8 forward (desc.w8) is not supported; pass the bf16 weights without w8");
  NB_CHECK(!d->base_ids && !d->alpha, NBEST_ERR_ARG, "encoder_infer: interpolated embeddings (desc.base_ids / alpha) are not supported; "
                                                     "run nbest_encoder_forward");
  NB_CHECK(wts && prm && ids && pos && key_mask && ws && cls_out, NBEST_ERR_ARG, "encoder_infer: null pointer");
  const Sizes z = sizes(d);
  const InferLayout w = infer_layout(z);
  NB_CHECK(ws_bytes >= w.total, NBEST_ERR_WORKSPACE, "encoder_infer: workspace too small (%zu < %zu)", ws_bytes, w.total);
  const Fwd c = make_fwd(d, wts, prm, z, key_mask, stream);
  const Ptrs& P = c.g.W;
  char* W = (char*)ws;
  const int64_t M = z.M, B = d->B, SH = (int64_t)d->S * d->H;
  const int H = d->H, F = d->F, dt = d->dtype;
  void* X[2] = {W + w.X0, W + w.X1};
  const LayerBufs b = infer_layer(w, ws);
  auto probs = [&](int l) { return cls_attn ? cls_attn + (int64_t)l * B * d->heads * d->S : nullptr; };

  RUN(nbest_embed_ln_fwd(ids, seg, pos, P.W(d->off_word), P.W(d->off_type), P.W(d->off_pos), P.P(d->off_emb_ln_g), P.P(d->off_emb_ln_b),
                         X[0], (float*)(W + w.emb_stats), M, H, d->ln_eps, dt, d->hidden_drop, d->seed, d->drop_stream_base,
                         (hipStream_t)stream));
  for (int l = 0; l + 1 < d->L; ++l) RUN(layer_forward(c, l, X[l & 1], X[(l + 1) & 1], b, nullptr, probs(l)));
  const int l = d->L - 1;
  const nbest_layer_offsets& o = d->layers_host[l];
  const void* xin = X[l & 1];
  void* kv = b.qkv; void* q = b.ctx; void* cctx = b.r1; void* cx1 = b.x1; void* ch = b.hact; void* cr = b.r2;
  nbest_gemm_args g = gemm_nt(dt, xin, P.W(o.wqkv + (int64_t)H * H), kv, M, 2 * H, H);
  g.epilogue = NBEST_EPI_BIAS; g.bias = P.P(o.bqkv + H);
  RUN(nbest_gemm(&g, stream));
  g = gemm_nt(dt, xin, P.W(o.wqkv), q, B, H, H);
  g.lda = SH; g.epilogue = NBEST_EPI_BIAS; g.bias = P.P(o.bqkv);
  RUN(nbest_gemm(&g, stream));
  if (cls_attn) RUN(nbest_internal_attention_cls_probs(q, H, kv, 2 * H, key_mask, probs(l), d->S, d->B, d->S, d->heads, 64, dt, stream));
  RUN(nbest_attention_cls_fwd_internal(q, H, kv, 2 * H, key_mask, cctx, H, d->B, d->S, d->heads, 64, dt, stream));
  if (d->head_gate) RUN(nbest_head_gate_fwd(cctx, H, cctx, H, d->head_gate + (int64_t)l * d->heads, B, d->heads, 64, dt, stream));
  g = gemm_nt(dt, cctx, P.W(o.wo), cr, B, H, H);
  g.epilogue = NBEST_EPI_BIAS_DROP_RES; g.bias = P.P(o.bo); g.R = xin; g.ldr = SH;
  RUN(nbest_gemm(&g, stream));
  RUN(nbest_internal_layernorm_fwd8(cr, P.P(o.ln1_g), P.P(o.ln1_b), cx1, nullptr, b.st1, B, H, d->ln_eps, dt, stream, nullptr, nullptr));
  g = gemm_nt(dt, cx1, P.W(o.w1), ch, B, F, H);
  g.epilogue = NBEST_EPI_BIAS_GELU; g.bias = P.P(o.b1); g.ldu = F;
  RUN(nbest_gemm(&g, stream));
  g = gemm_nt(dt, ch, P.W(o.w2), cr, B, H, F);
  g.epilogue = NBEST_EPI_BIAS_DROP_RES; g.bias = P.P(o.b2); g.R = cx1; g.ldr = H;
  RUN(nbest_gemm(&g, stream));
  RUN(nbest_internal_layernorm_fwd8(cr, P.P(o.ln2_g), P.P(o.ln2_b), cls_out, nullptr, b.st2, B, H, d->ln_eps, dt, stream, nullptr, nullptr));
  return NBEST_OK;
}

extern "C" int nbest_encoder_infer(const nbest_encoder_desc* d, const void* wts, const float* prm, const int64_t* ids, const int64_t* seg,
                                   const int64_t* pos, const uint8_t* key_mask, void* ws, size_t ws_bytes, void* cls_out,
                                   nbest_stream_t stream) {
  return nbest_encoder_infer_attn(d, wts, prm, ids, seg, pos, key_mask, ws, ws_bytes, cls_out, nullptr, stream);
}
```

n-best-asr-transformer_amd/csrc/internal.h:

```cpp
#pragma once
#include <hip/hip_runtime_api.h>
#include <stddef.h>
#include <stdint.h>

#include "../../include/nbest_hip.h"

struct Fp8Grad;

void nbest_set_error(const char* fmt, ...);

int nbest_internal_layernorm_fwd8(const void* x, const float* gamma, const float* beta, void* y, void* y8, float* stats,
                                  int64_t M, int H, float eps, int dtype, nbest_stream_t stream, const uint32_t* a_prev, uint32_t* a_new);
int nbest_internal_layernorm_bwd8(const void* dy, const void* x, const float* stats, const float* gamma, void* dx,
                                  void* dx_drop, float* dgamma, float* dbeta, float* dbias, int64_t M, int H, int dtype,
                                  int accumulate, float drop_p, uint64_t seed, uint32_t drop_stream, void* ws,
                                  size_t ws_bytes, nbest_stream_t stream, Fp8Grad f8);
int nbest_internal_partial_rows_sum(const float* part, int nrows, int N, float* out, int accumulate, hipStream_t st);
void nbest_internal_rowred_batch_begin();
void nbest_internal_rowred_batch_abort();
int nbest_internal_rowred_batch_flush(hipStream_t st);

int nbest_internal_attention_fwd8(const void* qkv, const uint8_t* key_mask, void* ctx, void* ctx8, float* lse, int B, int S, int heads,
                                  int d, int dtype, float drop_p, uint64_t seed, uint32_t drop_stream, nbest_stream_t stream,
                                  uint32_t* keep, const uint32_t* a_prev, uint32_t* a_new);
int nbest_internal_attention_bwd8(const void* qkv, const uint8_t* key_mask, const void* ctx, const void* dctx, const float* lse,
                                  void* dqkv, float* dbias, int accumulate, void* ws, size_t ws_bytes, int B, int S, int heads,
                                  int d, int dtype, float drop_p, uint64_t seed, uint32_t drop_stream, nbest_stream_t stream, Fp8Grad f8,
                                  const uint32_t* keep);
size_t nbest_internal_attention_keep_bytes(int B, int S, int heads);
int nbest_attention_cls_fwd_internal(const void* q, int64_t ldq, const void* kv, int64_t ldkv, const uint8_t* key_mask, void* ctx,
                                     int64_t ldctx, int B, int S, int heads, int d, int dtype, nbest_stream_t stream);
int nbest_internal_attention_cls_probs(const void* q, int64_t ldq, const void* kv, int64_t ldkv, const uint8_t* key_mask, float* probs,
                                       int64_t ldp, int B, int S, int heads, int d, int dtype, nbest_stream_t stream);

void nb_splitk_plan(int64_t tiles, int64_t K, int64_t slots, int64_t min_blocks, int* splits, int64_t* k_per_split);
int nbest_internal_splitk_reduce(const float* slab, float* C, int64_t M, int64_t N, int64_t ldc, int splits, int accumulate,
                                 float* C2, int64_t m_split, int64_t ldc2, hipStream_t st);

int nbest_gemm_f32_resolve(const nbest_gemm_args* a, nbest_gemm_plan_info* out);
int nbest_gemm_bf16_resolve(const nbest_gemm_args* a, nbest_gemm_plan_info* out);
int nbest_gemm_bf16_v2_resolve(const nbest_gemm_args* a, nbest_gemm_plan_info* out);
int nbest_gemm_f32(const nbest_gemm_args* a, hipStream_t st);
size_t nbest_gemm_bf16_ws_bytes(const nbest_gemm_args* a);
int nbest_gemm_bf16(const nbest_gemm_args* a, hipStream_t st);
size_t nbest_gemm_bf16_v2_ws_bytes(const nbest_gemm_args* a);
int nbest_gemm_bf16_v2(const nbest_gemm_args* a, hipStream_t st);
bool nbest_gemm_bf16_v2_wins(const nbest_gemm_args* a);
size_t nbest_wgrad_pair_bf16_ws_bytes(const nbest_gemm_args* a, const nbest_gemm_args* b);
int nbest_wgrad_pair_bf16(const nbest_gemm_args* a, const nbest_gemm_args* b, hipStream_t st);
int nbest_wgrad_group_bf16(const nbest_gemm_args* problems, int n, hipStream_t st);
int nbest_wgrad_window_bf16(const nbest_gemm_args* problems, const int32_t* tile_first, const int32_t* tile_count, int n, hipStream_t st);
int nbest_pack_bn_internal(int64_t N);
int nbest_pack_weights_bf16(const void* src, void* dst, const nbest_matrix_desc* descs, int n_matrices, int n_stages, hipStream_t st);

int nbest_internal_amax_bf16(const void* x, int64_t n, uint32_t* out, hipStream_t st);
int nbest_internal_cast_bf16_to_fp8(const void* src, void* dst, int64_t n, const uint32_t* a_prev, uint32_t* a_new, hipStream_t st);
```

n-best-asr-transformer_amd/csrc/norm_embed.hip:

```cpp
#include "common.h"

namespace {

constexpr int kMaxRowredBlocks = 512;
constexpr int kMaxLnBwdBlocks = 1024;
static inline int rowred_blocks(int64_t M) {
  int64_t b = (M + 31) / 32;
  if (b < 1) b = 1;
  if (b > kMaxRowredBlocks) b = kMaxRowredBlocks;
  return (int)b;
}

__device__ __forceinline__ float sum4(f32x4 v) { return (v[0] + v[1]) + (v[2] + v[3]); }

template <typename T, int VPL>
__global__ __launch_bounds__(256) void ln_fwd_kernel(const T* __restrict__ x, const float* __restrict__ gamma,
                                                     const float* __restrict__ beta, T* __restrict__ y,
                                                     float* __restrict__ stats, int64_t M, int H, float eps) {
  const int lane = threadIdx.x & 63, wpb = blockDim.x >> 6, nvec = H >> 2;
  const float invH = 1.0f / (float)H;
  for (int64_t row = (int64_t)blockIdx.x * wpb + (threadIdx.x >> 6); row < M; row += (int64_t)gridDim.x * wpb) {
    const T* xr = x + row * H;
    f32x4 v[VPL];
    float s = 0.f;
// ... 1279 lines not shown
  int Y = kMaxLnBwdBlocks / S;
  if (Y > B) Y = B;
  if (Y < 1) Y = 1;
  NB_CHECK((int64_t)S * Y <= kMaxLnBwdBlocks, NBEST_ERR_SHAPE, "embed_ln_bwd: S = %d exceeds %d", S, kMaxLnBwdBlocks);
  float* part = (float*)ws;
  int64_t* colkey = (int64_t*)(part + (size_t)5 * kMaxLnBwdBlocks * H);
  int* mixed = (int*)(colkey + kMaxLnBwdBlocks);
  int* shared = mixed + kMaxLnBwdBlocks;
  float* wpart = (float*)(shared + kMaxLnBwdBlocks);
  const size_t smem = (size_t)5 * H * sizeof(float);
  const dim3 grid(S, Y);
  const int64_t chunks = (M + kEmbTpc - 1) / kEmbTpc;
  const unsigned wgrid = (unsigned)((chunks + 3) / 4);
  int* fixlist = (int*)(wpart + (size_t)chunks * 2 * H);
#define NB_EMB_BWD2(TT, FULL)                                                                                                   \
  DISPATCH_VPL(H, ((void)hipFuncSetAttribute((const void*)embed_bwd_pos_kernel<TT, VPL, FULL>, hipFuncAttributeMaxDynamicSharedMemorySize, (int)smem), \
                   embed_bwd_pos_kernel<TT, VPL, FULL><<<grid, 256, smem, st>>>(ids, seg, pos, (const TT*)word, (const TT*)type, (const TT*)ptab, gamma, \
                                                                                 stats, (const TT*)dout, dtype_tab, dptab, part, fixlist, colkey, mixed, \
                                                                                 shared, B, S, H, pos_pad_id, d), \
                   embed_bwd_word_kernel<TT, VPL, FULL><<<wgrid, 256, 0, st>>>(perm, ids, seg, pos, (const TT*)word, (const TT*)type, (const TT*)ptab, \
                                                                                gamma, stats, (const TT*)dout, dword, wpart, fixlist, M, H,  \
                                                                                kEmbTpc, word_pad_id, tables_accumulate, d)))
#define NB_EMB_BWD(TT)                                   \
  do {                                                   \
    if (H % 256 == 0 && H <= 1024) NB_EMB_BWD2(TT, true); \
    else NB_EMB_BWD2(TT, false);                         \
  } while (0)
  embed_bwd_colkey_kernel<<<S, 256, 0, st>>>(seg, pos, B, S, H, pos_pad_id, tables_accumulate, colkey, mixed, dptab, dtype_tab);
  if (dtype == NBEST_F32) NB_EMB_BWD(float);
  else if (dtype == NBEST_BF16) NB_EMB_BWD(bf16);
  else NB_CHECK(false, NBEST_ERR_DTYPE, "embed_ln_bwd: bad dtype %d", dtype);
#undef NB_EMB_BWD2
#undef NB_EMB_BWD
  NB_LAUNCH_CHECK();
  embed_bwd_wordfix_kernel<<<(unsigned)(chunks < 2048 ? chunks : 2048), 256, (size_t)4 * H * sizeof(float), st>>>(perm, ids, wpart, fixlist, dword, M, H,
                                                                                                                    kEmbTpc, tables_accumulate);
  embed_bwd_finalize_kernel<<<dim3((H + 31) / 32, 4 + (S + 31) / 32), dim3(32, 32), 0, st>>>(part, colkey, shared, S, Y, H, n_types, pos_pad_id, dgamma, dbeta,
                                                                                             dtype_tab, dptab, accumulate, tables_accumulate);
  NB_LAUNCH_CHECK();
  return NBEST_OK;
}

extern "C" int nbest_rows_gather(const float* table, const int64_t* rows, int64_t n_rows, int64_t cap, int64_t* ids_out,
                                 float* vals_out, int H, nbest_stream_t stream) {
  NB_CHECK(table && ids_out && vals_out && (rows || n_rows == 0) && n_rows >= 0 && cap >= n_rows && H > 0 && H % 4 == 0, NBEST_ERR_ARG,
           "rows_gather: bad arguments");
  if (cap == 0) return NBEST_OK;
  rows_gather_kernel<<<(unsigned)cap, 256, 0, (hipStream_t)stream>>>(table, rows, n_rows, ids_out, vals_out, H);
  NB_LAUNCH_CHECK();
  return NBEST_OK;
}

extern "C" int nbest_rows_zero(float* table, const int64_t* ids, int64_t n, int H, nbest_stream_t stream) {
  NB_CHECK(table && (ids || n == 0) && n >= 0 && H > 0 && H % 4 == 0, NBEST_ERR_ARG, "rows_zero: bad arguments");
  if (n == 0) return NBEST_OK;
  rows_update_kernel<<<(unsigned)n, 256, 0, (hipStream_t)stream>>>(table, ids, nullptr, H);
  NB_LAUNCH_CHECK();
  return NBEST_OK;
}

extern "C" int nbest_rows_add(float* table, const int64_t* ids, const float* vals, int64_t n, int H, nbest_stream_t stream) {
  NB_CHECK(table && ((ids && vals) || n == 0) && n >= 0 && H > 0 && H % 4 == 0, NBEST_ERR_ARG, "rows_add: bad arguments");
  if (n == 0) return NBEST_OK;
  rows_update_kernel<<<(unsigned)n, 256, 0, (hipStream_t)stream>>>(table, ids, vals, H);
  NB_LAUNCH_CHECK();
  return NBEST_OK;
}

extern "C" int nbest_cls_grad_scatter(const float* dcls, void* dhidden, int B, int S, int H, int dtype,
                                      nbest_stream_t stream) {
  if (int e = check_h(H)) return e;
  NB_CHECK(dcls && dhidden && B > 0 && S > 0, NBEST_ERR_ARG, "cls_grad_scatter: bad arguments");
  hipStream_t st = (hipStream_t)stream;
  const int64_t nv = (int64_t)B * S * (H >> 2);
  int grid = (int)((nv + 255) / 256);
  if (grid > 4096) grid = 4096;
  if (dtype == NBEST_F32) cls_scatter_kernel<float><<<grid, 256, 0, st>>>(dcls, (float*)dhidden, nv, S, H);
  else if (dtype == NBEST_BF16) cls_scatter_kernel<bf16><<<grid, 256, 0, st>>>(dcls, (bf16*)dhidden, nv, S, H);
  else NB_CHECK(false, NBEST_ERR_DTYPE, "cls_grad_scatter: bad dtype %d", dtype);
  NB_LAUNCH_CHECK();
  return NBEST_OK;
}

extern "C" int nbest_cast_f32_to_bf16(const float* src, void* dst, int64_t n, nbest_stream_t stream) {
  NB_CHECK(src && dst && n >= 0, NBEST_ERR_ARG, "cast: bad arguments");
  if (n == 0) return NBEST_OK;
  int64_t g = ((n >> 3) + 255) / 256;
  if (g > 8192) g = 8192;
  if (g < 1) g = 1;
  cast_bf16_kernel<<<(int)g, 256, 0, (hipStream_t)stream>>>(src, (bf16*)dst, n);
  NB_LAUNCH_CHECK();
  return NBEST_OK;
}
```

n-best-asr-transformer_amd/hipabi.py:

```python
import collections
import ctypes as C
import os

import torch

_HERE = os.path.dirname(os.path.abspath(__file__))
LIB_PATH = os.environ.get("NBEST_LIB") or os.path.join(_HERE, "csrc", "libnbest_hip.so")

F32, BF16 = 0, 1
ADAM_L2, ADAMW = 0, 1
EPI_NONE, EPI_BIAS, EPI_BIAS_GELU, EPI_BIAS_DROP_RES, EPI_DGELU, EPI_RES, EPI_F32_SPLITK = range(7)

EXPORTS = [
    "nbest_version", "nbest_last_error", "nbest_embed_ln_fwd", "nbest_embed_ln_bwd", "nbest_embed_bwd_ws_bytes", "nbest_rows_gather", "nbest_rows_zero", "nbest_rows_add",
    "nbest_gemm_ws_bytes", "nbest_gemm", "nbest_gemm_plan", "nbest_wgrad_pair_ws_bytes", "nbest_wgrad_pair", "nbest_wgrad_group", "nbest_wgrad_window", "nbest_pack_bn", "nbest_pack_weights", "nbest_pack_bn_fp8", "nbest_pack_weights_fp8", "nbest_attention_fwd", "nbest_attention_bwd", "nbest_attention_bwd_ws_bytes", "nbest_attention_keep_bytes", "nbest_attention_fwd_keep", "nbest_attention_bwd_keep", "nbest_layernorm_fwd",
    "nbest_layernorm_bwd", "nbest_rowred_ws_bytes", "nbest_colsum", "nbest_heads_ws_bytes", "nbest_stc_heads", "nbest_stc_heads_kd", "nbest_stc_heads_kd_t", "nbest_stc_heads_logits", "nbest_stc_heads_rdrop",
    "nbest_stc_heads_vjp", "nbest_cls_mse", "nbest_cls_grad_scatter", "nbest_stc_decode", "nbest_stream_stamp", "nbest_fp8_amax_fold", "nbest_bertadam_chunk", "nbest_bertadam_step", "nbest_bertadam_norms", "nbest_bertadam_update",
    "nbest_adam_clip_coef", "nbest_adam_update", "nbest_adam_step", "nbest_ema_update", "nbest_ema_exchange",
    "nbest_cast_f32_to_bf16", "nbest_transpose_weights", "nbest_encoder_act_bytes", "nbest_encoder_ws_bytes", "nbest_encoder_wgrad_launches_per_layer", "nbest_encoder_wgrad_plan", "nbest_encoder_forward",
    "nbest_encoder_backward", "nbest_gemm_fp8", "nbest_gemm_fp8_ws_bytes", "nbest_wgrad_fp8", "nbest_wgrad_fp8_ws_bytes", "nbest_wgrad_fp8_pair", "nbest_wgrad_fp8_pair_ws_bytes", "nbest_cast_bf16_to_fp8", "nbest_quantize_weights_fp8",
    "nbest_attention_cls_fwd", "nbest_encoder_infer_ws_bytes", "nbest_encoder_infer",
    "nbest_attention_probs", "nbest_attention_cls_probs", "nbest_encoder_act_view", "nbest_encoder_infer_attn",
    "nbest_embed_ln_fwd_interp", "nbest_embed_attrib",
    "nbest_head_gate_fwd", "nbest_head_gate_bwd",
]


class GemmArgs(C.Structure):
    _fields_ = [("A", C.c_void_p), ("B", C.c_void_p), ("C", C.c_void_p), ("bias", C.c_void_p), ("R", C.c_void_p),
                ("U", C.c_void_p), ("ws", C.c_void_p), ("ws_bytes", C.c_size_t),
                ("M", C.c_int64), ("N", C.c_int64), ("K", C.c_int64),
                ("lda", C.c_int64), ("ldb", C.c_int64), ("ldc", C.c_int64), ("ldr", C.c_int64), ("ldu", C.c_int64),
                ("trans_a", C.c_int32), ("trans_b", C.c_int32), ("epilogue", C.c_int32), ("dtype", C.c_int32),
                ("accumulate", C.c_int32), ("drop_p", C.c_float), ("drop_stream", C.c_uint32), ("seed", C.c_uint64),
                ("colsum_out", C.c_void_p), ("colsum_accumulate", C.c_int32), ("flags", C.c_int32),
                ("B_packed", C.c_void_p), ("b_pack_bn", C.c_int32), ("pad_", C.c_int32)]


class GemmPlanInfo(C.Structure):
    _fields_ = [("generation", C.c_int32), ("bm", C.c_int32), ("bn", C.c_int32), ("bk", C.c_int32),
                ("wave_rows", C.c_int32), ("wave_cols", C.c_int32), ("stages", C.c_int32), ("form", C.c_int32),
                ("reg_epilogue", C.c_int32), ("splits", C.c_int32), ("k_per_split", C.c_int64),
                ("b_packed", C.c_int32), ("kernel_epilogue", C.c_int32)]


class GemmFp8Args(C.Structure):
    _fields_ = [("A", C.c_void_p), ("B", C.c_void_p), ("C", C.c_void_p), ("bias", C.c_void_p), ("R", C.c_void_p), ("U", C.c_void_p),
                ("C8", C.c_void_p), ("M", C.c_int64), ("N", C.c_int64), ("K", C.c_int64),
                ("lda", C.c_int64), ("ldb", C.c_int64), ("ldc", C.c_int64), ("ldr", C.c_int64), ("ldu", C.c_int64), ("ldc8", C.c_int64),
                ("epilogue", C.c_int32), ("out_scale", C.c_float), ("drop_p", C.c_float), ("drop_stream", C.c_uint32), ("seed", C.c_uint64),
                ("out_scale_dev", C.c_void_p), ("a_amax", C.c_void_p), ("c8_amax_prev", C.c_void_p), ("c8_amax_new", C.c_void_p),
                ("colsum_out", C.c_void_p), ("colsum_accumulate", C.c_int32), ("pad", C.c_int32), ("ws", C.c_void_p), ("ws_bytes", C.c_size_t),
                ("B_packed", C.c_void_p), ("b_pack_bn", C.c_int32), ("pad3", C.c_int32)]


class LabelSpaceC(C.Structure):
    _fields_ = [("n_top", C.c_int32), ("n_bottom", C.c_int32), ("n_rows", C.c_int32),
                ("bottom_off", C.c_void_p), ("bottom_ids", C.c_void_p), ("head_row", C.c_void_p)]


class TensorDesc(C.Structure):
    _fields_ = [("offset", C.c_int64), ("numel", C.c_int64), ("lr", C.c_float), ("wd", C.c_float),
                ("active", C.c_int32), ("block_start", C.c_int32)]


class MatrixDesc(C.Structure):
    _fields_ = [("offset", C.c_int64), ("rows", C.c_int32), ("cols", C.c_int32), ("tile_start", C.c_int32), ("pad", C.c_int32)]


class LayerOffsets(C.Structure):
    _fields_ = [(n, C.c_int64) for n in ("wqkv", "bqkv", "wo", "bo", "ln1_g", "ln1_b", "w1", "b1", "w2", "b2", "ln2_g", "ln2_b")]


class EncoderDesc(C.Structure):
    _fields_ = [("dtype", C.c_int32), ("B", C.c_int32), ("S", C.c_int32), ("H", C.c_int32), ("L", C.c_int32),
                ("heads", C.c_int32), ("F", C.c_int32), ("vocab", C.c_int32), ("max_pos", C.c_int32), ("n_types", C.c_int32),
                ("ln_eps", C.c_float), ("hidden_drop", C.c_float), ("attn_drop", C.c_float),
                ("word_pad_id", C.c_int64), ("pos_pad_id", C.c_int64),
                ("off_word", C.c_int64), ("off_pos", C.c_int64), ("off_type", C.c_int64),
                ("off_emb_ln_g", C.c_int64), ("off_emb_ln_b", C.c_int64),
                ("layers_host", C.POINTER(LayerOffsets)), ("seed", C.c_uint64), ("drop_stream_base", C.c_uint32),
                ("wgrad_events_n", C.c_int32), ("wgrad_events", C.POINTER(C.c_void_p)),
                ("w8", C.c_void_p), ("w8_inv_scale", C.c_void_p), ("w8t", C.c_void_p), ("gamax_prev", C.c_void_p),
                ("gamax_new", C.c_void_p), ("fp8_bwd", C.c_int32), ("pad2", C.c_int32),
                ("wpk", C.c_void_p), ("wpkt", C.c_void_p), ("w8p", C.c_void_p), ("w8tp", C.c_void_p),
                ("word_perm", C.c_void_p), ("aamax_prev", C.c_void_p), ("aamax_new", C.c_void_p), ("fp8_act", C.c_int32), ("pad4", C.c_int32),
                ("first_trainable", C.c_int32), ("no_input_grad", C.c_int32), ("wgrad_skip_host", C.c_void_p),
                ("head_gate", C.c_void_p), ("head_gate_grad", C.c_void_p),
                ("base_ids", C.c_void_p), ("alpha", C.c_void_p), ("no_param_grad", C.c_int32), ("pad5", C.c_int32)]
    wgrad_group = property(lambda self: self.pad5, lambda self, v: setattr(self, "pad5", int(v)))


_lib = None


def lib():
    global _lib
    if _lib is None:
        if not os.path.exists(LIB_PATH):
            raise RuntimeError("nbest_amd: %s is missing - build it with `make -C %s` (hipcc, gfx950). "
                               "There is no CPU fallback for the product path." % (LIB_PATH, os.path.dirname(LIB_PATH)))
        L = C.CDLL(LIB_PATH)
        for name in EXPORTS:
            if not hasattr(L, name):
                raise RuntimeError("nbest_amd: %s does not export %s" % (LIB_PATH, name))
        for name in ("nbest_embed_bwd_ws_bytes", "nbest_gemm_ws_bytes", "nbest_wgrad_pair_ws_bytes", "nbest_rowred_ws_bytes", "nbest_heads_ws_bytes",
                     "nbest_attention_bwd_ws_bytes", "nbest_attention_keep_bytes",
                     "nbest_encoder_act_bytes", "nbest_encoder_ws_bytes", "nbest_encoder_infer_ws_bytes"):
            getattr(L, name).restype = C.c_size_t
        L.nbest_embed_bwd_ws_bytes.argtypes = [C.c_int64, C.c_int64]
        L.nbest_rows_gather.argtypes = [C.c_void_p, C.c_void_p, C.c_int64, C.c_int64, C.c_void_p, C.c_void_p, C.c_int, C.c_void_p]
        L.nbest_rows_zero.argtypes = [C.c_void_p, C.c_void_p, C.c_int64, C.c_int, C.c_void_p]
        L.nbest_rows_add.argtypes = [C.c_void_p, C.c_void_p, C.c_void_p, C.c_int64, C.c_int, C.c_void_p]
        L.nbest_rowred_ws_bytes.argtypes = [C.c_int64, C.c_int64]
        L.nbest_heads_ws_bytes.argtypes = [C.c_int, C.c_int, C.c_int]
        L.nbest_gemm_ws_bytes.argtypes = [C.POINTER(GemmArgs)]
        L.nbest_gemm.argtypes = [C.POINTER(GemmArgs), C.c_void_p]
        L.nbest_gemm_plan.argtypes = [C.POINTER(GemmArgs), C.POINTER(GemmPlanInfo)]
        L.nbest_wgrad_pair_ws_bytes.argtypes = [C.POINTER(GemmArgs), C.POINTER(GemmArgs)]
        L.nbest_wgrad_pair.argtypes = [C.POINTER(GemmArgs), C.POINTER(GemmArgs), C.c_void_p]
        L.nbest_wgrad_group.argtypes = [C.POINTER(GemmArgs), C.c_int32, C.c_void_p]
        L.nbest_wgrad_window.argtypes = [C.POINTER(GemmArgs), C.POINTER(C.c_int32), C.POINTER(C.c_int32), C.c_int32, C.c_void_p]
        L.nbest_encoder_act_bytes.argtypes = [C.POINTER(EncoderDesc)]
        L.nbest_encoder_ws_bytes.argtypes = [C.POINTER(EncoderDesc)]
        L.nbest_encoder_wgrad_launches_per_layer.argtypes = [C.POINTER(EncoderDesc)]
        L.nbest_encoder_wgrad_plan.argtypes = [C.POINTER(EncoderDesc), C.c_int32, C.c_int32, C.POINTER(C.c_int32), C.c_int32]
        vp, i64, i32, f32, u64, u32, sz = C.c_void_p, C.c_int64, C.c_int, C.c_float, C.c_uint64, C.c_uint32, C.c_size_t
        L.nbest_embed_ln_fwd.argtypes = [vp] * 10 + [i64, i32, f32, i32, f32, u64, u32, vp]
        L.nbest_embed_ln_bwd.argtypes = [vp] * 15 + [i32, i32, i32, i32, i32, i64, i64, i32, i32, f32, u64, u32, vp, sz, vp]
        L.nbest_embed_ln_fwd_interp.argtypes = [vp] * 12 + [i32, i32, i32, f32, i32, f32, u64, u32, vp]
        L.nbest_embed_attrib.argtypes = [vp] * 11 + [i32, i32, i32, i32, f32, i32, vp]
        L.nbest_head_gate_fwd.argtypes = [vp, i64, vp, i64, vp, i64, i32, i32, i32, vp]
        L.nbest_head_gate_bwd.argtypes = [vp, vp, vp, vp, i32, i32, i32, i32, i32, vp]
        L.nbest_attention_fwd.argtypes = [vp] * 4 + [i32] * 5 + [f32, u64, u32, vp]
        L.nbest_attention_bwd.argtypes = [vp] * 7 + [i32, vp, sz] + [i32] * 5 + [f32, u64, u32, vp]
        L.nbest_attention_bwd_ws_bytes.argtypes = [i32, i32, i32]
        L.nbest_attention_keep_bytes.argtypes = [i32, i32, i32]
        L.nbest_attention_fwd_keep.argtypes = [vp] * 4 + [i32] * 5 + [f32, u64, u32, vp, vp]
        L.nbest_attention_bwd_keep.argtypes = [vp] * 7 + [i32, vp, sz] + [i32] * 5 + [f32, u64, u32, vp, vp]
        L.nbest_layernorm_fwd.argtypes = [vp] * 5 + [i64, i32, f32, i32, vp]
        L.nbest_layernorm_bwd.argtypes = [vp] * 9 + [i64, i32, i32, i32, f32, u64, u32, vp, sz, vp]
        L.nbest_colsum.argtypes = [vp, vp, i64, i64, i64, i32, i32, vp, sz, vp]
        L.nbest_stc_heads.argtypes = [vp, i64, vp, vp, C.POINTER(LabelSpaceC)] + [vp] * 8 + [i32] * 5 + [f32, u64, u32, vp, sz, vp]
        L.nbest_stc_heads_kd.argtypes = [vp, i64, vp, vp, C.POINTER(LabelSpaceC)] + [vp] * 4 + [f32] + [vp] * 7 + [i32] * 5 + [f32, u64, u32, vp, sz, vp]
        L.nbest_stc_heads_kd_t.argtypes = [vp, i64, vp, vp, C.POINTER(LabelSpaceC)] + [vp] * 2 + [f32, f32] + [vp] * 7 + [i32] * 5 + [f32, u64, u32, vp, sz, vp]
        L.nbest_stc_heads_rdrop.argtypes = [vp, i64, vp, vp, C.POINTER(LabelSpaceC), vp, f32] + [vp] * 7 + [i32] * 5 + [f32, u64, u32, vp, sz, vp]
        L.nbest_stc_heads_logits.argtypes = [vp, i64, vp, vp, C.POINTER(LabelSpaceC), vp, i32, i32, i32, vp]
        L.nbest_stc_heads_vjp.argtypes = [vp, C.POINTER(LabelSpaceC)] + [vp] * 8 + [i32, i32, i32, f32, u64, u32, vp, sz, vp]
        L.nbest_cls_mse.argtypes = [vp, i64, vp, i64, vp, vp, vp, i32, i32, i32, f32, vp]
        L.nbest_cls_grad_scatter.argtypes = [vp, vp, i32, i32, i32, i32, vp]
        L.nbest_stc_decode.argtypes = [vp, vp, C.POINTER(LabelSpaceC), vp, vp, i32, vp]
        L.nbest_stream_stamp.argtypes = [vp, i32, vp]
        L.nbest_fp8_amax_fold.argtypes = [vp, vp, i32, vp]
        L.nbest_bertadam_step.argtypes = [vp] * 6 + [i32, i32, f32, f32, f32, f32, f32, vp, sz, vp]
        L.nbest_bertadam_norms.argtypes = [vp, vp, i32, i32, i32, i32, vp, vp]
        L.nbest_bertadam_update.argtypes = [vp] * 6 + [i32, i32, i32, i32, vp, vp, f32, f32, f32, f32, f32, vp]
        L.nbest_adam_clip_coef.argtypes = [vp, i32, f32, vp, vp]
        f64 = C.c_double
        L.nbest_adam_update.argtypes = [i32] + [vp] * 6 + [i32, i32, i32, i32, vp, f32, f32, f32, f64, f64, f32, vp]
        L.nbest_adam_step.argtypes = [i32] + [vp] * 6 + [i32, i32, f32, f32, f32, f64, f64, f32, f32, vp, sz, vp]
        L.nbest_ema_update.argtypes = [vp, vp, vp, i32, i32, f32, vp]
        L.nbest_ema_exchange.argtypes = [vp, vp, vp, vp, i32, i32, vp]
        L.nbest_cast_f32_to_bf16.argtypes = [vp, vp, i64, vp]
        L.nbest_encoder_forward.argtypes = [C.POINTER(EncoderDesc)] + [vp] * 7 + [sz, vp, sz, C.POINTER(C.c_void_p), vp]
        L.nbest_encoder_infer_ws_bytes.argtypes = [C.POINTER(EncoderDesc)]
        L.nbest_encoder_infer.argtypes = [C.POINTER(EncoderDesc)] + [vp] * 7 + [sz, vp, vp]
        L.nbest_attention_cls_fwd.argtypes = [vp, i64, vp, i64, vp, vp, i64, i32, i32, i32, i32, i32, vp]
        L.nbest_encoder_infer_attn.argtypes = [C.POINTER(EncoderDesc)] + [vp] * 7 + [sz, vp, vp, vp]
        L.nbest_encoder_act_view.argtypes = [C.POINTER(EncoderDesc), vp, i32, C.POINTER(C.c_void_p), C.POINTER(C.c_void_p)]
# ... 659 lines not shown
```

n-best-asr-transformer_amd/model.py:

```python
import collections
import ctypes as C
import math
import os

import torch
import torch.nn as nn

from . import hipabi as hb
from .arena import ParamArena
from .config import EncoderConfig, LabelSpace, NAMED


def position_ids_for(cfg, input_ids):
    B, S = input_ids.shape
    if cfg.family in ("roberta", "xlm-roberta"):
        nonpad = input_ids.ne(cfg.pad_token_id).long()
        return (torch.cumsum(nonpad, dim=1) * nonpad + cfg.pad_token_id).contiguous()
    return torch.arange(S, dtype=torch.long, device=input_ids.device).unsqueeze(0).expand(B, S).contiguous()


class _Holder(nn.Module):
    """module tree node that only carries arena-backed parameters under HF names"""


def _attach(root, dotted, param):
    mod = root
    parts = dotted.split(".")
    for p in parts[:-1]:
        if not hasattr(mod, p):
            mod.add_module(p, _Holder())
        mod = getattr(mod, p)
    mod.register_parameter(parts[-1], param)


class FreezePlan(collections.namedtuple("FreezePlan", "key trainable first_trainable no_input_grad with_embeddings skip")):
    __slots__ = ()

    @property
    def skip_ptr(self):
        return None if self.skip is None else C.cast(self.skip, C.c_void_p)


def freeze_plan(model):
    flags = tuple(p.requires_grad and "pooler" not in n for n, p in model._params)
    plan = model._plans.get(flags)
    if plan is not None:
        return plan
    trainable = frozenset(n for (n, _), f in zip(model._params, flags) if f)
    L = model.cfg.num_hidden_layers
    emb = any(n.startswith("bert_encoder.embeddings.") for n in trainable)
    layer = [any(n.startswith("bert_encoder.encoder.layer.%d." % l) for n in trainable) for l in range(L)]
    first = 0 if emb else next((l for l in range(L) if layer[l]), L)
    pre = "bert_encoder.encoder.layer.%d."
    mats = (["attention.self.%s.weight" % q for q in ("query", "key", "value")], ["attention.output.dense.weight"],
            ["intermediate.dense.weight"], ["output.dense.weight"])
    skip = [int(not any((pre % l) + m in trainable for m in ms)) for l in range(L) for ms in mats]
    plan = FreezePlan(flags, trainable, first, int(not emb), emb, (C.c_uint8 * len(skip))(*skip) if any(skip) else None)
    if len(model._plans) >= 64:
        model._plans.clear()
    model._plans[flags] = plan
    return plan


class _Pass:

    def __init__(self, model, B, S, slot, first_trainable=0):
        a, cfg = model.arena, model.cfg
        train = isinstance(slot, int)
        d = hb.EncoderDesc()
        d.dtype = hb.dtype_code(model.compute_dtype)
        d.B, d.S, d.H, d.L, d.heads, d.F = B, S, cfg.hidden_size, cfg.num_hidden_layers, cfg.num_attention_heads, cfg.intermediate_size
        d.vocab, d.max_pos, d.n_types = cfg.vocab_size, cfg.max_position_embeddings, cfg.type_vocab_size
        d.ln_eps = cfg.layer_norm_eps
        d.word_pad_id = cfg.pad_token_id
        d.pos_pad_id = cfg.pad_token_id if cfg.family in ("roberta", "xlm-roberta") else -1
        pre = "bert_encoder.embeddings."
        d.off_word = a.by_name[pre + "word_embeddings.weight"].offset
        d.off_pos = a.by_name[pre + "position_embeddings.weight"].offset
        d.off_type = a.by_name[pre + "token_type_embeddings.weight"].offset
        d.off_emb_ln_g = a.by_name[pre + "LayerNorm.weight"].offset
        d.off_emb_ln_b = a.by_name[pre + "LayerNorm.bias"].offset
        d.layers_host = C.cast(a.layer_offsets, C.POINTER(hb.LayerOffsets))
        d.drop_stream_base = 1000 * slot if train else 0
        d.first_trainable = first_trainable
        d.wgrad_group = model.wgrad_group
        if model.fp8_forward and train:
            d.w8, d.w8_inv_scale = a.w8.data_ptr(), a.w8_inv_scale.data_ptr()
        self.desc = d
        self.act_bytes = hb.lib().nbest_encoder_act_bytes(C.byref(d))
        self.B, self.S = B, S


class _PassRecord(collections.namedtuple("_PassRecord", "ps slot inputs perm hidden gen plan")):
    __slots__ = ()

    @property
    def cls(self):
        return self.hidden.view(self.ps.B, self.ps.S, -1)[:, 0, :]


class _STCBridge(torch.autograd.Function):

    @staticmethod
    def forward(ctx, anchor, model, input_ids, trans_input_ids, seg_ids, trans_seg_ids, feats_from_transcript):
        ctx.set_materialize_grads(False)
        from_t = bool(feats_from_transcript and trans_input_ids is not None)
        ws = hb.heads_ws(input_ids.shape[0], model.dls.n_rows, model.cfg.hidden_size, model.device)
        plan = model._training_plan()
        ra, rt, (top, bott, fin, _, _, _, _) = model._passes_and_heads(input_ids, seg_ids, trans_input_ids, trans_seg_ids, True,
                                                                       from_transcript=from_t, ws=ws, plan=plan)
        ctx.model, ctx.ra, ctx.rt, ctx.ws, ctx.seed, ctx.from_t = model, ra, rt, ws, model._step_seed(), from_t
        ctx.save_for_backward(top, bott)
        trans_cls = rt.cls.float() if rt is not None else torch.zeros(0, device=model.device)
        return top, bott, fin, ra.cls.float(), trans_cls

    @staticmethod
    def backward(ctx, dtop, dbott, dfin, dasr, dtrans):
        m = ctx.model
        m._check_stash(ctx.ra, ctx.rt)
        _require_trainable(ctx.ra.plan)
        top, bott = ctx.saved_tensors
        B, H = top.shape[0], m.cfg.hidden_size
        z = lambda g, like: torch.zeros_like(like) if g is None else g.contiguous().float()
        fin_like = torch.empty(B, m.labels.n_bottom, dtype=torch.float32, device=m.device)
        dWh, dbh = m.arena.heads_grad_wb()
        dcls = hb.stc_heads_vjp(m.arena.heads_wb()[0], m.dls, top, bott, z(dtop, top), z(dbott, bott), z(dfin, fin_like), B, H, dWh, dbh, ctx.ws,
                                accumulate=True, drop_p=m.dropout, seed=ctx.seed, drop_stream=900)
        d_asr = dasr.contiguous().float() if dasr is not None else None
        d_tr = dtrans.contiguous().float() if (dtrans is not None and ctx.rt is not None) else None
        if ctx.from_t:
            d_tr = dcls if d_tr is None else d_tr + dcls
        else:
            d_asr = dcls if d_asr is None else d_asr + dcls
        if d_tr is not None and ctx.rt is not None:
            m._backward_pass(ctx.rt, d_tr, accumulate=True)
        if d_asr is not None:
            m._backward_pass(ctx.ra, d_asr, accumulate=True)
        m._end_of_step(True)
        return (None,) * 7


def _check_distill(distill, B, dls):
    if not isinstance(distill, dict) or set(distill) not in ({"top", "bott", "final", "alpha"}, {"logits", "alpha", "temperature"}):
        raise ValueError("nbest_amd: distill must be dict(top=, bott=, final=, alpha=) (a teacher's predict() scores and the weight "
                         "of the soft loss) or dict(logits=, alpha=, temperature=) (its predict(return_logits=True) logits)")
    alpha = float(distill["alpha"])
    if not 0.0 <= alpha <= 1.0:
        raise ValueError("nbest_amd: distill alpha %r: must be in [0, 1]" % (distill["alpha"],))
    if "logits" in distill:
        try:
            T = float(distill["temperature"])
        except (TypeError, ValueError):
            T = float("nan")
        if not (T > 0.0 and math.isfinite(T)):
            raise ValueError("nbest_amd: distill temperature %r: must be a finite number > 0" % (distill["temperature"],))
        t = distill["logits"]
        if not torch.is_tensor(t) or t.dtype != torch.float32 or not t.is_cuda or tuple(t.shape) != (B, dls.n_rows):
            raise ValueError("nbest_amd: distill['logits'] must be an fp32 device tensor of shape [%d, %d] (the teacher's "
                             "predict(return_logits=True)['logits'])" % (B, dls.n_rows))
        return dict(logits=t.contiguous(), alpha=alpha, temperature=T)
    widths = dict(top=dls.labels.n_top, bott=dls.n_rows - dls.labels.n_top, final=dls.labels.n_bottom)
    for k in ("top", "bott", "final"):
        t = distill[k]
        if not torch.is_tensor(t) or t.dtype != torch.float32 or not t.is_cuda or tuple(t.shape) != (B, widths[k]):
            raise ValueError("nbest_amd: distill[%r] must be an fp32 device tensor of shape [%d, %d] (the teacher's predict()[%r])"
                             % (k, B, widths[k], k))
    return dict(top=distill["top"].contiguous(), bott=distill["bott"].contiguous(), final=distill["final"].contiguous(), alpha=alpha)


def _check_rdrop(rdrop, B, distill=None):
    if not isinstance(rdrop, dict) or set(rdrop) != {"alpha"}:
        raise ValueError("nbest_amd: rdrop must be dict(alpha=) (the weight of the twins' consistency term)")
    if distill is not None:
        raise ValueError("nbest_amd: rdrop together with distill is not built (one soft term per step: loss_parts[3] carries it)")
    try:
        alpha = float(rdrop["alpha"])
    except (TypeError, ValueError):
        alpha = float("nan")
    if not (alpha >= 0.0 and math.isfinite(alpha)):
        raise ValueError("nbest_amd: rdrop alpha %r: must be a finite number >= 0" % (rdrop["alpha"],))
    if B < 2 or B % 2:
        raise ValueError("nbest_amd: rdrop needs a batch of 2 P rows (rows b and b + P are twins), got %d rows" % B)
    return dict(alpha=alpha)


def _require_trainable(plan):
    if plan is not None and not plan.trainable:
        raise RuntimeError("nbest_amd: no parameter requires grad: a backward has nothing to compute (every tensor of the model "
                           "has requires_grad=False)")


class NBestSTCModel(nn.Module):
    def __init__(self, cfg: EncoderConfig, labels: LabelSpace, device="cuda", compute_dtype=torch.bfloat16, dropout=0.0,
                 seed=999, fp8_forward=False, fp8_backward=None, wgrad_group=hb.WGRAD_GROUP_PLAN):
        super().__init__()
        self.cfg, self.labels, self.compute_dtype = cfg, labels, compute_dtype
        self.dropout = float(dropout)
        self.device = torch.device(device)
        self.wgrad_group = int(wgrad_group)
        self.arena = ParamArena(cfg, labels, self.device, compute_dtype)
        self.fp8_forward = bool(fp8_forward)
        self.fp8_backward = self.fp8_forward if fp8_backward is None else bool(fp8_backward)
        self._gamax_valid = False
        self._aamax_valid = False
        if self.fp8_forward:
            if compute_dtype != torch.bfloat16:
                raise RuntimeError("nbest_amd: fp8_forward rides on the bf16 path")
            self.arena.enable_fp8_forward()
        elif self.fp8_backward:
            raise RuntimeError("nbest_amd: fp8_backward needs fp8_forward (it shares the e4m3 weight copy)")
        self.bert_encoder = _Holder()
        self.clf = _Holder()
        for s in self.arena.slots:
            p = nn.Parameter(self.arena.view(self.arena.p, s.name), requires_grad="pooler" not in s.name)
            if p.requires_grad:
                p.grad = self.arena.view(self.arena.g, s.name)
            root, rest = s.name.split(".", 1)
            _attach(getattr(self, root), rest, p)
        self._params = [(s.name, self.get_parameter(s.name)) for s in self.arena.slots]
        self._plans = {}
        self._plan_key = None
        self.dls = hb.DeviceLabelSpace(labels, self.device)
        self.seed = int(seed)
        self.step_counter = 0
        self._passes = {}
        self._stash = {}
        self._stash_gen = collections.Counter()
        self._ws = None
        self._dh = None
        self._infer_ws = None
        self._anchor = None
        self._head_mask = None

    def zero_grad(self, set_to_none=False):
        self.arena.g.zero_()

    def _drop_fp8_history(self):
        if self.fp8_backward and self._gamax_valid:
            self._gamax_valid = False
            self.arena.gamax.zero_()
            self.arena.gamax_slots.zero_()
        if self.fp8_forward and self._aamax_valid:
            self._aamax_valid = False
            self.arena.aamax.zero_()
            self.arena.aamax_slots.zero_()

    def load_reference_state(self, sd, strict=True):
        self._drop_fp8_history()
        return self.arena.load_state(sd, strict)

    def save_model(self, path):
        torch.save({k: v.detach().cpu() for k, v in self.state_dict().items()}, path)

    def load_model(self, path):
        self._drop_fp8_history()
        self.arena.load_state(torch.load(path, map_location="cpu", weights_only=True))

    def load_pretrained_encoder(self, path):
        import os
        if os.path.isdir(path):
            cands = [os.path.join(path, f) for f in ("model.safetensors", "pytorch_model.bin")]
            found = [c for c in cands if os.path.exists(c)]
            if not found:
                raise FileNotFoundError("no model.safetensors / pytorch_model.bin under %s" % path)
            path = found[0]
        self._drop_fp8_history()
        if path.endswith(".safetensors"):
            from safetensors.torch import load_file
            raw = load_file(path, device="cpu")
        else:
            raw = torch.load(path, map_location="cpu", weights_only=True)
        sd = {}
        for k, v in raw.items():
            for pre in ("bert_encoder.", "bert.", "roberta.", "xlm_roberta."):
                if k.startswith(pre):
                    k = k[len(pre):]
                    break
            k = k.replace("LayerNorm.gamma", "LayerNorm.weight").replace("LayerNorm.beta", "LayerNorm.bias")
            if k.startswith(("embeddings.", "encoder.", "pooler.")) and not k.endswith("position_ids"):
                sd["bert_encoder." + k] = v
        want = [s.name for s in self.arena.slots if s.name.startswith("bert_encoder.")]
        missing = [n for n in want if n not in sd]
        hard = [n for n in missing if "pooler" not in n]
# ... 7 lines not shown
        return self._head_mask

    def set_head_mask(self, mask):
        if mask is None:
            self._head_mask = None
            return
        L, heads = self.cfg.num_hidden_layers, self.cfg.num_attention_heads
        m = torch.as_tensor(mask)
        if tuple(m.shape) != (L, heads):
            raise ValueError("nbest_amd set_head_mask: the mask must be [L=%d, heads=%d] (got %s)" % (L, heads, list(m.shape)))
        self._head_mask = m.detach().to(device=self.device, dtype=torch.float32).contiguous().clone()

    def _refuse_training_under_mask(self, what):
        if self._head_mask is not None:
            raise RuntimeError("nbest_amd: %s with a head mask set: training under a head mask is not built (the attention-output "
                               "weight gradient needs the gated context); call set_head_mask(None) first" % what)

    def _set_head_gate(self, d, grad=None):
        d.head_gate = None if self._head_mask is None else self._head_mask.data_ptr()
        d.head_gate_grad = None if grad is None else grad.data_ptr()

    def _desc(self, B, S, slot, first_trainable=0):
        key = (B, S, slot, first_trainable)
        if key not in self._passes:
            if len(self._passes) >= 4096:
                self._passes.clear()
            self._passes[key] = _Pass(self, B, S, slot, first_trainable)
        return self._passes[key]

    def _training_plan(self):
        plan = freeze_plan(self)
        if plan.key != self._plan_key:
            for (n, p), f in zip(self._params, plan.key):
                if "pooler" in n:
                    continue
                if not f:
                    p.grad = None
                elif p.grad is None:
                    p.grad = self.arena.view(self.arena.g, n)
            if self._plan_key is not None and self.fp8_backward and self._gamax_valid:
                self._gamax_valid = False
                self.arena.gamax.zero_()
                self.arena.gamax_slots.zero_()
            self._plan_key = plan.key
        return plan

    def _grow(self, table, key, n, dtype=torch.uint8):
        buf = table.get(key)
        if buf is None or buf.numel() < n:
            table[key] = buf = None
            table[key] = buf = torch.empty(n, dtype=dtype, device=self.device)
        return buf

    def _pass(self, B, S, slot, first_trainable=0):
        ps = self._desc(B, S, slot, first_trainable)
        self._grow(self._stash, slot, ps.act_bytes)
        self._grow(vars(self), "_ws", hb.lib().nbest_encoder_ws_bytes(C.byref(ps.desc)))
        self._stash_gen[slot] += 1
        return ps

    def _check_stash(self, *records):
        for r in records:
            if r is not None and r.gen != self._stash_gen[r.slot]:
                raise RuntimeError("nbest_amd: another forward ran on this model between this forward() and its backward(): the "
                                   "activations of its %s pass are overwritten" % ("ASR", "transcript")[r.slot])

    def _step_seed(self):
        rank = 0
        if torch.distributed.is_available() and torch.distributed.is_initialized():
            rank = torch.distributed.get_rank()
        return self.seed + 7919 * self.step_counter + 15485863 * rank

    def _inputs(self, ids, seg):
        cfg = self.cfg
        ids = ids.contiguous()
        mask = (ids > 0).to(torch.uint8)
        pos = position_ids_for(cfg, ids)
        if cfg.family == "xlm-roberta":
            seg = None
        elif seg is not None:
            seg = seg.contiguous()
        return ids, seg, pos, mask

    def _encode(self, slot, ids, seg, train, perm=None, plan=None):
        B, S = ids.shape
        ps = self._pass(B, S, slot, plan.first_trainable if plan is not None else 0)
        ids, seg, pos, mask = inputs = self._inputs(ids, seg)
        d = ps.desc
        d.hidden_drop = self.cfg.hidden_dropout_prob if train else 0.0
        d.attn_drop = self.cfg.attention_probs_dropout_prob if train else 0.0
        d.seed = self._step_seed()
        self._set_head_gate(d)
        self._set_weights(d, "forward")
        act, ws = self._stash[slot][:ps.act_bytes], self._ws
        out = C.c_void_p()
        hb.check(hb.lib().nbest_encoder_forward(C.byref(d), hb.ptr(self.arena.weights), hb.ptr(self.arena.p), hb.ptr(ids),
                                                hb.ptr(seg), hb.ptr(pos), hb.ptr(mask), hb.ptr(act), act.numel(),
                                                hb.ptr(ws), ws.numel(), C.byref(out), hb.stream_ptr()),
                 "encoder_forward")
        off = out.value - act.data_ptr()
        M, H = B * S, self.cfg.hidden_size
        esz = 2 if self.compute_dtype == torch.bfloat16 else 4
        hidden = act[off:off + M * H * esz].view(self.compute_dtype).view(M, H)
        return _PassRecord(ps, slot, inputs, perm, hidden, self._stash_gen[slot], plan)

    def _packed_bf16_ok(self):
        return self.arena.wpk is not None and not self.arena.w16t_stale

    def _set_weights(self, d, call):
        a = self.arena
        fp8_bwd = self.fp8_backward and call != "infer" and self._gamax_valid and self._aamax_valid
        if call == "backward" and a.w16t_stale and not fp8_bwd:
            a.refresh_w16t()
        ok = self._packed_bf16_ok()
        d.wpk = a.wpk.data_ptr() if ok else None
        d.wpkt = a.wpkt.data_ptr() if ok else None
        if call == "infer":
            return
        ok8 = a.w8p is not None
        d.w8p = a.w8p.data_ptr() if ok8 else None
        d.w8tp = a.w8tp.data_ptr() if ok8 else None
        if self.fp8_forward and call == "forward":
            d.aamax_prev, d.aamax_new = a.aamax.data_ptr(), a.aamax_slots.data_ptr()
            d.fp8_act = int(self._aamax_valid)
        if self.fp8_backward:
            d.w8t = a.w8t.data_ptr()
            d.gamax_prev, d.gamax_new = a.gamax.data_ptr(), a.gamax_slots.data_ptr()
            d.fp8_bwd = int(fp8_bwd)
            a.lazy_w16t = fp8_bwd

    def _end_of_step(self, ran_backward, advance=True):
        if self.fp8_forward:
            hb.fp8_amax_fold(self.arena.aamax_slots, self.arena.aamax)
            self._aamax_valid = True
        if ran_backward and self.fp8_backward:
            hb.fp8_amax_fold(self.arena.gamax_slots, self.arena.gamax)
            self._gamax_valid = True
        if advance:
            self.step_counter += 1

    def _backward_pass(self, rec, dcls, accumulate, chunks=None, on_chunk_done=None):
        ps, d = rec.ps, rec.ps.desc
        B, S, H = ps.B, ps.S, self.cfg.hidden_size
        self._set_weights(d, "backward")
        dh = self._grow(vars(self), "_dh", B * S * H, self.compute_dtype)[:B * S * H].view(B * S, H)
        dh = hb.cls_grad_scatter(dcls, B, S, H, self.compute_dtype, out=dh)
        ids, seg, pos, mask = rec.inputs
        perm = rec.perm if rec.perm is not None else hb.word_perm(ids)
        d.word_perm = perm.data_ptr()
        act, ws = self._stash[rec.slot][:ps.act_bytes], self._ws
        plan = rec.plan
        ft = plan.first_trainable if plan is not None else 0
        d.no_input_grad = plan.no_input_grad if plan is not None else 0
        d.wgrad_skip_host = plan.skip_ptr if plan is not None else None
        with_emb = plan.with_embeddings if plan is not None else True
        bounds = chunks or [(0, self.cfg.num_hidden_layers)]
        for (lo, hi) in sorted(bounds, reverse=True):
            lo_t = max(lo, ft)
            if hi > lo_t:
                hb.check(hb.lib().nbest_encoder_backward(C.byref(d), hb.ptr(self.arena.weights), hb.ptr(self.arena.w16t),
                                                         hb.ptr(self.arena.p),
                                                         hb.ptr(self.arena.g), hb.ptr(ids), hb.ptr(seg), hb.ptr(pos), hb.ptr(mask),
                                                         hb.ptr(act), act.numel(), hb.ptr(dh), hb.ptr(ws), ws.numel(),
                                                         int(accumulate), lo_t, hi, int(lo_t == 0 and with_emb), hb.stream_ptr()),
                         "encoder_backward")
            if on_chunk_done is not None:
                on_chunk_done(lo, hi)

    def _heads(self, hidden, S, labels_f, need_grad, train, accumulate=False, ws=None, distill=None, rdrop=None):
        B, H = hidden.shape[0] // S, self.cfg.hidden_size
        Wh, bh = self.arena.heads_wb()
        dWh, dbh = self.arena.heads_grad_wb()
        if labels_f is None:
            labels_f = torch.zeros(B, self.labels.n_bottom, dtype=torch.float32, device=self.device)
        soft = None
        if rdrop is not None:
            soft = hb.SoftTerm("rdrop", rdrop["alpha"])
        elif distill is not None and "logits" in distill:
            soft = hb.SoftTerm("kd_t", distill["alpha"], distill["temperature"], (distill["logits"],))
        elif distill is not None:
            soft = hb.SoftTerm("kd", distill["alpha"], None, (distill["top"], distill["bott"], distill["final"]))
        return hb.stc_heads(hidden, S * H, Wh, bh, self.dls, labels_f.contiguous(), B, H, need_grad=need_grad,
                            accumulate=accumulate, drop_p=self.dropout if train else 0.0,
                            seed=self._step_seed(), drop_stream=900, dWh=dWh, dbh=dbh, ws=ws, soft=soft)

    def _passes_and_heads(self, ids, seg, trans_ids, trans_seg, train, from_transcript=False, labels_f=None, need_grad=False,
                          accumulate=False, perm=None, trans_perm=None, ws=None, plan=None, after_asr=None, distill=None, rdrop=None):
        ra = self._encode(0, ids, seg, train, perm, plan)
        if after_asr is not None:
            after_asr(ra)
        rt = None if trans_ids is None else self._encode(1, trans_ids, trans_seg, train, trans_perm, plan)
        r = rt if from_transcript else ra
        return ra, rt, self._heads(r.hidden, r.ps.S, labels_f, need_grad, train, accumulate, ws, distill, rdrop)

    def _bottoms_dict(self, bott):
        out, col = {}, 0
        for t in self.labels.multi:
            n = len(self.labels.top2bottom[t])
            out["lin_%d" % t] = bott[:, col:col + n]
            col += n
        return out

    def forward(self, opt, input_ids, trans_input_ids=None, seg_ids=None, trans_seg_ids=None, return_attns=False,
                classifier_input_type="asr", distill=None):
        if distill is not None:
            raise RuntimeError("nbest_amd: distill= belongs to forward_backward (the fused step: train_step, the CLI); the forward "
                               "returns scores - build the soft loss from them and a teacher's predict() yourself")
        if self.training and torch.is_grad_enabled():
            if return_attns:
                raise RuntimeError("nbest_amd: return_attns=True: attention maps are an eval / predict output - call model.eval() "
                                   "or run the forward under torch.no_grad() (a training forward has no post-dropout maps)")
            self._refuse_training_under_mask("the training forward (autograd bridge)")
            if self._anchor is None:
                self._anchor = torch.zeros(1, device=self.device, requires_grad=True)
            top, bott, fin, asr_cls, trans_cls = _STCBridge.apply(self._anchor, self, input_ids.contiguous(),
                                                                  None if trans_input_ids is None else trans_input_ids.contiguous(), seg_ids,
                                                                  trans_seg_ids, classifier_input_type == "transcript")
            return top, self._bottoms_dict(bott), fin, asr_cls, (trans_cls if trans_input_ids is not None else None)
        with torch.no_grad():
            return self._forward_plain(input_ids, trans_input_ids, seg_ids, trans_seg_ids, classifier_input_type, return_attns)

    def _forward_plain(self, input_ids, trans_input_ids, seg_ids, trans_seg_ids, classifier_input_type, return_attns=False):
        attns = []
        after = (lambda rec: attns.extend(self._attention_maps(rec))) if return_attns else None
        ra, rt, (top, bott, fin, _, _, _, _) = self._passes_and_heads(input_ids, seg_ids, trans_input_ids, trans_seg_ids, self.training,
                                                                      from_transcript=classifier_input_type == "transcript",
                                                                      after_asr=after)
        self._end_of_step(False, advance=False)
        trans_cls = None if rt is None else rt.cls.float()
        if return_attns:
            return top, self._bottoms_dict(bott), fin, tuple(attns), ra.cls.float(), trans_cls
        return top, self._bottoms_dict(bott), fin, ra.cls.float(), trans_cls

    def _attention_maps(self, rec):
        self._check_stash(rec)
        ps = rec.ps
        B, S, H, heads = ps.B, ps.S, self.cfg.hidden_size, self.cfg.num_attention_heads
        act = self._stash[rec.slot]
        base, esz = act.data_ptr(), (2 if self.compute_dtype == torch.bfloat16 else 4)
        n_qkv, n_lse = B * S * 3 * H * esz, B * heads * S * 4
        out = []
        for l in range(self.cfg.num_hidden_layers):
            qp, lp = hb.encoder_act_view(ps.desc, act, l)
            qkv = act[qp - base:qp - base + n_qkv].view(self.compute_dtype)
            lse = act[lp - base:lp - base + n_lse].view(torch.float32)
            out.append(hb.attention_probs(qkv, rec.inputs[3], lse, B, S, heads))
        return out

    def forward_backward(self, input_ids, labels_f, seg_ids=None, trans_input_ids=None, trans_seg_ids=None,
                         add_l2_loss=False, mse_grad_scale=1.0, chunks=None, on_chunk_done=None, need_grad=True,
                         accumulate=False, encoder_grad_scale=1.0, tok_perm=None, trans_tok_perm=None, distill=None, rdrop=None):
        if rdrop is not None:
            rdrop = _check_rdrop(rdrop, input_ids.shape[0], distill)
        if distill is not None:
            distill = _check_distill(distill, input_ids.shape[0], self.dls)
        plan = None
        if need_grad:
            self._refuse_training_under_mask("forward_backward(need_grad=True)")
            plan = self._training_plan()
            _require_trainable(plan)
        ra, rt, (top, bott, fin, loss, dcls, _, _) = self._passes_and_heads(
            input_ids, seg_ids, trans_input_ids if add_l2_loss else None, trans_seg_ids, self.training, labels_f=labels_f,
            need_grad=need_grad, accumulate=accumulate, perm=tok_perm, trans_perm=trans_tok_perm, plan=plan, distill=distill, rdrop=rdrop)
        B, H = ra.ps.B, self.cfg.hidden_size
        dt = mse = None
        if rt is not None:
            dt = torch.empty(B, H, dtype=torch.float32, device=self.device) if need_grad else None
            mse = hb.cls_mse(ra.hidden, ra.ps.S * H, rt.hidden, rt.ps.S * H, B, H, dcls, dt, grad_scale=mse_grad_scale)
            if distill is None and rdrop is None:
                loss[3:4].copy_(mse)
        if need_grad and encoder_grad_scale != 1.0:
            dcls.mul_(encoder_grad_scale)
            if dt is not None:
                dt.mul_(encoder_grad_scale)
        if need_grad:
            if rt is not None:
                self._backward_pass(rt, dt, accumulate=accumulate)
                self._backward_pass(ra, dcls, accumulate=True, chunks=chunks, on_chunk_done=on_chunk_done)
            else:
                self._backward_pass(ra, dcls, accumulate=accumulate, chunks=chunks, on_chunk_done=on_chunk_done)
        self._end_of_step(need_grad)
        out = dict(top=top, bott=bott, final=fin, loss_parts=loss, asr_cls=ra.cls, trans_cls=None if rt is None else rt.cls)
        if (distill is not None or rdrop is not None) and mse is not None:
            out["mse"] = mse
        return out

    def predict(self, input_ids, seg_ids=None, return_attns=False, return_logits=False):
        cfg = self.cfg
        B, S = input_ids.shape
        H = cfg.hidden_size
        first_pos = cfg.pad_token_id + 1 if cfg.family in ("roberta", "xlm-roberta") else 0
        if S > 512 or S + first_pos > cfg.max_position_embeddings:
            raise RuntimeError("nbest_amd predict: S=%d does not fit the position table (%d rows)" % (S, cfg.max_position_embeddings))
        d = self._desc(B, S, "infer").desc
        ids, seg, pos, mask = self._inputs(input_ids, seg_ids)
        d.hidden_drop = d.attn_drop = 0.0
        d.seed = 0
        self._set_head_gate(d)
        self._set_weights(d, "infer")
        ws = self._grow(vars(self), "_infer_ws", hb.lib().nbest_encoder_infer_ws_bytes(C.byref(d)))
        a = self.arena
        cls = torch.empty(B, H, dtype=self.compute_dtype, device=self.device)
        cls_attn = torch.empty(cfg.num_hidden_layers, B, cfg.num_attention_heads, S, dtype=torch.float32,
                               device=self.device) if return_attns else None
        hb.encoder_infer(d, a.weights, a.p, ids, seg, pos, mask, ws, cls, cls_attn)
        Wh, bh = a.heads_wb()
        labels_f = torch.zeros(B, self.labels.n_bottom, dtype=torch.float32, device=self.device)
        top, bott, fin, _, _, _, _ = hb.stc_heads(cls, H, Wh, bh, self.dls, labels_f, B, H, need_grad=False, drop_p=0.0)
        out = dict(top=top, bott=bott, final=fin, cls=cls, pred=self.decode(top, bott))
        if return_attns:
# ... 183 lines not shown
```

Baseline: 12780.

## Compute only the CLS row in the final encoder layer during training

Adds a cls_top mode where the last encoder layer runs its attention, output projection, layernorms and FFN only for the CLS token, since the classifier heads read only the CLS hidden state. It adds single-query attention forward and backward kernels with dropout, a row dropout+residual kernel, and wgrad skip entries for the last layer. The aim is to remove roughly (S-1)/S of the last layer's post-QKV work in both forward and backward. Non-CLS hidden states of the top layer are no longer computed, so the path is restricted to training without fp8, head masks or attention-map output.

```diff
diff --git a/include/nbest_hip.h b/include/nbest_hip.h
--- a/include/nbest_hip.h
+++ b/include/nbest_hip.h
@@ -298,7 +298,7 @@
   const uint32_t* aamax_prev;
   uint32_t* aamax_new;
   int32_t fp8_act;
-  int32_t pad4;
+  int32_t cls_top;
   int32_t first_trainable;
   int32_t no_input_grad;
   const uint8_t* wgrad_skip_host;
diff --git a/n-best-asr-transformer_amd/csrc/attention.hip b/n-best-asr-transformer_amd/csrc/attention.hip
--- a/n-best-asr-transformer_amd/csrc/attention.hip
+++ b/n-best-asr-transformer_amd/csrc/attention.hip
@@ -1123,10 +1123,11 @@
   }
 }
 
-template <typename T, bool PROBS>
+template <typename T, bool PROBS, bool DROP = false>
 __global__ __launch_bounds__(256) void attn_cls_fwd_kernel(const T* __restrict__ q, int64_t ldq, const T* __restrict__ kv, int64_t ldkv,
                                                            const uint8_t* __restrict__ mask, T* __restrict__ ctx, int64_t ldctx, int S,
-                                                           int heads, int H, float scale, float* __restrict__ probs, int64_t ldp) {
+                                                           int heads, int H, float scale, float* __restrict__ probs, int64_t ldp,
+                                                           DropCfg drop) {
   constexpr bool kF32 = sizeof(T) == 4;
   constexpr int VEC = 16 / (int)sizeof(T);
   constexpr int LPK = 64 / VEC;
@@ -1191,9 +1192,19 @@
     }
     return;
   }
-  for (int j = tid; j < S; j += 256) {
-    const float v = sc[j];
-    sc[j] = kF32 ? (v == -INFINITY ? 0.f : expf(v - lse)) : (float)(bf16)(ex(v) * inv);
+  if constexpr (DROP) {
+    const float ids = inv * drop.scale;
+    for (int j = tid; j < S; j += 256) {
+      const float v = sc[j];
+      const bool keep = nb_keep(drop, (uint32_t)((bh * S) * S + j));
+      if constexpr (kF32) sc[j] = (v == -INFINITY || !keep) ? 0.f : expf(v - lse) * drop.scale;
+      else sc[j] = keep ? (float)(bf16)(ex(v) * ids) : 0.f;
+    }
+  } else {
+    for (int j = tid; j < S; j += 256) {
+      const float v = sc[j];
+      sc[j] = kF32 ? (v == -INFINITY ? 0.f : expf(v - lse)) : (float)(bf16)(ex(v) * inv);
+    }
   }
   __syncthreads();
   float o[VEC];
@@ -1217,6 +1228,134 @@
     T* op = ctx + (int64_t)b * ldctx + h * 64 + tid;
     if constexpr (kF32) *op = acc;
     else *op = (bf16)acc;
+  }
+}
+
+template <typename T>
+__global__ __launch_bounds__(256) void attn_cls_bwd_kernel(const T* __restrict__ qkv, const uint8_t* __restrict__ mask,
+                                                           const T* __restrict__ ctx, const T* __restrict__ dctx, T* __restrict__ dqkv,
+                                                           float* __restrict__ colpart, int S, int heads, int H, float scale, DropCfg drop) {
+  constexpr bool kF32 = sizeof(T) == 4;
+  constexpr int VEC = 16 / (int)sizeof(T);
+  constexpr int LPK = 64 / VEC;
+  constexpr int KPP = 256 / LPK;
+  __shared__ float sp[512];
+  __shared__ float spt[512];
+  __shared__ float qs[64], dos[64];
+  __shared__ float part[3][KPP][65];
+  __shared__ float red[9];
+  const int tid = threadIdx.x, sub = tid % LPK, kg = tid / LPK, lane = tid & 63, wave = tid >> 6;
+  const int bh = blockIdx.x, b = bh / heads, h = bh - b * heads;
+  const int64_t ld = 3 * (int64_t)H;
+  const T* base = qkv + (int64_t)b * S * ld + h * 64;
+  T* dbase = dqkv + (int64_t)b * S * ld + h * 64;
+  const uint8_t* mk = mask + (int64_t)b * S;
+  auto load = [](const T* p, float* v) {
+    if constexpr (kF32) {
+      const f32x4 x = *(const f32x4*)p;
+#pragma unroll
+      for (int e = 0; e < 4; ++e) v[e] = x[e];
+    } else {
+      const bf16x8 x = __builtin_bit_cast(bf16x8, *(const i32x4*)p);
+#pragma unroll
+      for (int e = 0; e < 8; ++e) v[e] = (float)x[e];
+    }
+  };
+  auto store = [](T* p, const float* v) {
+    if constexpr (kF32) {
+      f32x4 x;
+#pragma unroll
+      for (int e = 0; e < 4; ++e) x[e] = v[e];
+      *(f32x4*)p = x;
+    } else {
+      bf16x8 x;
+#pragma unroll
+      for (int e = 0; e < 8; ++e) x[e] = (bf16)v[e];
+      *(i32x4*)p = __builtin_bit_cast(i32x4, x);
+    }
+  };
+  if (wave == 0) {
+    const float qv = (float)base[lane], dv = (float)dctx[(int64_t)b * H + h * 64 + lane];
+    qs[lane] = qv; dos[lane] = dv;
+    const float dl = wave_sum(dv * (float)ctx[(int64_t)b * H + h * 64 + lane]);
+    if (lane == 0) red[8] = dl;
+  }
+  __syncthreads();
+  float mloc = -INFINITY;
+  for (int j = tid; j < S; j += 256) {
+    const T* kp = base + (int64_t)j * ld + H;
+    float d = 0.f, dv = 0.f;
+#pragma unroll
+    for (int c = 0; c < 64; c += VEC) {
+      float kr[VEC], vr[VEC];
+      load(kp + c, kr);
+      load(kp + H + c, vr);
+#pragma unroll
+      for (int e = 0; e < VEC; ++e) { d = fmaf(qs[c + e], kr[e], d); dv = fmaf(dos[c + e], vr[e], dv); }
+    }
+    const float sv = mk[j] ? d * scale : -INFINITY;
+    sp[j] = sv; spt[j] = dv;
+    mloc = fmaxf(mloc, sv);
+  }
+  mloc = wave_max(mloc);
+  if (lane == 0) red[wave] = mloc;
+  __syncthreads();
+  const float mx = fmaxf(fmaxf(red[0], red[1]), fmaxf(red[2], red[3]));
+  const float mxs = (mx == -INFINITY) ? 0.f : mx;
+  auto ex = [&](float v) { return kF32 ? expf(v - mxs) : __expf(v - mxs); };
+  float sum = 0.f;
+  for (int j = tid; j < S; j += 256) sum += ex(sp[j]);
+  sum = wave_sum(sum);
+  if (lane == 0) red[4 + wave] = sum;
+  __syncthreads();
+  sum = (red[4] + red[5]) + (red[6] + red[7]);
+  const float lse = mxs + logf(sum), inv = 1.0f / sum, delta = red[8];
+  for (int j = tid; j < S; j += 256) {
+    const float v = sp[j];
+    const float p = (v == -INFINITY) ? 0.f : (kF32 ? expf(v - lse) : ex(v) * inv);
+    float ks = 1.f;
+    if (drop.thr16) ks = nb_keep(drop, (uint32_t)((bh * S) * S + j)) ? drop.scale : 0.f;
+    const float ds = p * (spt[j] * ks - delta) * scale;
+    sp[j] = kF32 ? ds : (float)(bf16)ds;
+    spt[j] = kF32 ? p * ks : (float)(bf16)(p * ks);
+  }
+  __syncthreads();
+  float dq[VEC], ck[VEC], cv[VEC], zero[VEC];
+#pragma unroll
+  for (int e = 0; e < VEC; ++e) dq[e] = ck[e] = cv[e] = zero[e] = 0.f;
+  for (int j = kg; j < S; j += KPP) {
+    const float ds = sp[j], pt = spt[j];
+    float kr[VEC], ok[VEC], ov[VEC];
+    load(base + (int64_t)j * ld + H + sub * VEC, kr);
+#pragma unroll
+    for (int e = 0; e < VEC; ++e) {
+      ok[e] = ds * qs[sub * VEC + e];
+      ov[e] = pt * dos[sub * VEC + e];
+      dq[e] = fmaf(ds, kr[e], dq[e]);
+      ck[e] += ok[e]; cv[e] += ov[e];
+    }
+    T* row = dbase + (int64_t)j * ld + sub * VEC;
+    if (j > 0) store(row, zero);
+    store(row + H, ok);
+    store(row + 2 * H, ov);
+  }
+#pragma unroll
+  for (int e = 0; e < VEC; ++e) {
+    part[0][kg][sub * VEC + e] = dq[e];
+    part[1][kg][sub * VEC + e] = ck[e];
+    part[2][kg][sub * VEC + e] = cv[e];
+  }
+  __syncthreads();
+  if (tid < 192) {
+    const int which = tid >> 6;
+    float acc = 0.f;
+#pragma unroll
+    for (int g = 0; g < KPP; ++g) acc += part[which][g][lane];
+    if (which == 0) {
+      if constexpr (kF32) dbase[lane] = acc;
+      else dbase[lane] = (bf16)acc;
+    }
+    if (colpart) colpart[(int64_t)b * 3 * H + which * H + h * 64 + lane] = acc;
   }
 }
 
@@ -1380,7 +1519,8 @@
 }
 
 int nbest_attention_cls_fwd_internal(const void* q, int64_t ldq, const void* kv, int64_t ldkv, const uint8_t* key_mask, void* ctx,
-                                     int64_t ldctx, int B, int S, int heads, int d, int dtype, nbest_stream_t stream) {
+                                     int64_t ldctx, int B, int S, int heads, int d, int dtype, nbest_stream_t stream, float drop_p,
+                                     uint64_t seed, uint32_t drop_stream) {
   NB_CHECK(q && kv && key_mask && ctx, NBEST_ERR_ARG, "attention_cls_fwd: null pointer");
   NB_CHECK(B > 0 && S > 0 && heads > 0, NBEST_ERR_SHAPE, "attention_cls_fwd: bad shape");
   NB_CHECK(d == 64, NBEST_ERR_SHAPE, "attention_cls_fwd: head dimension %d not supported (64 only)", d);
@@ -1393,19 +1533,53 @@
   NB_CHECK(((uintptr_t)q & 15) == 0 && ((uintptr_t)kv & 15) == 0, NBEST_ERR_ALIGN, "attention_cls_fwd: q and kv must be 16-byte aligned");
   const float scale = 1.0f / sqrtf((float)d);
   hipStream_t st = (hipStream_t)stream;
-  if (dtype == NBEST_F32)
+  const DropCfg dc = make_drop(drop_p, seed, drop_stream);
+  if (dc.thr16) {
+    if (int e = check_common("attention_cls_fwd", B, S, heads, d, dtype)) return e;
+    if (dtype == NBEST_F32)
+      attn_cls_fwd_kernel<float, false, true><<<B * heads, 256, 0, st>>>((const float*)q, ldq, (const float*)kv, ldkv, key_mask, (float*)ctx,
+                                                                         ldctx, S, heads, H, scale, nullptr, 0, dc);
+    else
+      attn_cls_fwd_kernel<bf16, false, true><<<B * heads, 256, 0, st>>>((const bf16*)q, ldq, (const bf16*)kv, ldkv, key_mask, (bf16*)ctx,
+                                                                        ldctx, S, heads, H, scale, nullptr, 0, dc);
+  } else if (dtype == NBEST_F32)
     attn_cls_fwd_kernel<float, false><<<B * heads, 256, 0, st>>>((const float*)q, ldq, (const float*)kv, ldkv, key_mask, (float*)ctx, ldctx, S,
-                                                                 heads, H, scale, nullptr, 0);
+                                                                 heads, H, scale, nullptr, 0, DropCfg{});
   else
     attn_cls_fwd_kernel<bf16, false><<<B * heads, 256, 0, st>>>((const bf16*)q, ldq, (const bf16*)kv, ldkv, key_mask, (bf16*)ctx, ldctx, S,
-                                                                heads, H, scale, nullptr, 0);
+                                                                heads, H, scale, nullptr, 0, DropCfg{});
   NB_LAUNCH_CHECK();
   return NBEST_OK;
 }
 
 extern "C" int nbest_attention_cls_fwd(const void* q, int64_t ldq, const void* kv, int64_t ldkv, const uint8_t* key_mask, void* ctx,
                                        int64_t ldctx, int B, int S, int heads, int d, int dtype, nbest_stream_t stream) {
-  return nbest_attention_cls_fwd_internal(q, ldq, kv, ldkv, key_mask, ctx, ldctx, B, S, heads, d, dtype, stream);
+  return nbest_attention_cls_fwd_internal(q, ldq, kv, ldkv, key_mask, ctx, ldctx, B, S, heads, d, dtype, stream, 0.f, 0, 0);
+}
+
+int nbest_internal_attention_cls_bwd(const void* qkv, const uint8_t* key_mask, const void* ctx, const void* dctx, void* dqkv, float* dbias,
+                                     int accumulate, void* ws, size_t ws_bytes, int B, int S, int heads, int d, int dtype, float drop_p,
+                                     uint64_t seed, uint32_t drop_stream, nbest_stream_t stream) {
+  NB_CHECK(qkv && key_mask && ctx && dctx && dqkv, NBEST_ERR_ARG, "attention_cls_bwd: null pointer");
+  if (int e = check_common("attention_cls_bwd", B, S, heads, d, dtype)) return e;
+  NB_CHECK(S <= 512, NBEST_ERR_SHAPE, "attention_cls_bwd: S=%d > 512", S);
+  const int H = heads * d;
+  NB_CHECK(((uintptr_t)qkv & 15) == 0 && ((uintptr_t)dqkv & 15) == 0 && ((uintptr_t)ctx & 15) == 0 && ((uintptr_t)dctx & 15) == 0,
+           NBEST_ERR_ALIGN, "attention_cls_bwd: pointers must be 16-byte aligned");
+  NB_CHECK(!dbias || (ws && ws_bytes >= (size_t)B * 3 * H * sizeof(float)), NBEST_ERR_WORKSPACE, "attention_cls_bwd: workspace too small");
+  const float scale = 1.0f / sqrtf((float)d);
+  const DropCfg dc = make_drop(drop_p, seed, drop_stream);
+  float* colpart = dbias ? (float*)ws : nullptr;
+  hipStream_t st = (hipStream_t)stream;
+  if (dtype == NBEST_F32)
+    attn_cls_bwd_kernel<float><<<B * heads, 256, 0, st>>>((const float*)qkv, key_mask, (const float*)ctx, (const float*)dctx, (float*)dqkv,
+                                                          colpart, S, heads, H, scale, dc);
+  else
+    attn_cls_bwd_kernel<bf16><<<B * heads, 256, 0, st>>>((const bf16*)qkv, key_mask, (const bf16*)ctx, (const bf16*)dctx, (bf16*)dqkv,
+                                                         colpart, S, heads, H, scale, dc);
+  NB_LAUNCH_CHECK();
+  if (dbias) return nbest_internal_partial_rows_sum(colpart, B, 3 * H, dbias, accumulate, st);
+  return NBEST_OK;
 }
 
 extern "C" int nbest_attention_probs(const void* qkv, const uint8_t* key_mask, const float* lse, float* probs, int B, int S, int heads,
@@ -1447,10 +1621,10 @@
   hipStream_t st = (hipStream_t)stream;
   if (dtype == NBEST_F32)
     attn_cls_fwd_kernel<float, true><<<B * heads, 256, 0, st>>>((const float*)q, ldq, (const float*)kv, ldkv, key_mask, nullptr, 0, S,
-                                                                heads, H, scale, probs, ldp);
+                                                                heads, H, scale, probs, ldp, DropCfg{});
   else
     attn_cls_fwd_kernel<bf16, true><<<B * heads, 256, 0, st>>>((const bf16*)q, ldq, (const bf16*)kv, ldkv, key_mask, nullptr, 0, S,
-                                                               heads, H, scale, probs, ldp);
+                                                               heads, H, scale, probs, ldp, DropCfg{});
   NB_LAUNCH_CHECK();
   return NBEST_OK;
 }
diff --git a/n-best-asr-transformer_amd/csrc/encoder.hip b/n-best-asr-transformer_amd/csrc/encoder.hip
--- a/n-best-asr-transformer_amd/csrc/encoder.hip
+++ b/n-best-asr-transformer_amd/csrc/encoder.hip
@@ -210,6 +210,7 @@
   w.red_bytes = std::max(w.red_bytes, al((size_t)((M + 127) / 128) * 2 * d->F * sizeof(float)));
   w.red = take(o, 4 * w.red_bytes);
   w.slab_bytes = al(max_splitk_bytes(d, M));
+  w.slab_bytes = std::max(w.slab_bytes, al(max_splitk_bytes(d, d->B)));
   w.slab = take(o, w.slab_bytes);
   w.emb_bytes = al(nbest_embed_bwd_ws_bytes(M, d->H));
   w.emb = take(o, w.emb_bytes);
@@ -251,6 +252,25 @@
   NB_CHECK(!d->head_gate || d->first_trainable == 0, NBEST_ERR_ARG, "encoder: head_gate needs first_trainable == 0 (got %d)", d->first_trainable);
   NB_CHECK(!d->head_gate_grad || d->head_gate, NBEST_ERR_ARG, "encoder: head_gate_grad without head_gate");
   return NBEST_OK;
+}
+
+static int check_cls_top(const nbest_encoder_desc* d) {
+  if (!d->cls_top) return NBEST_OK;
+  NB_CHECK(!d->w8, NBEST_ERR_ARG, "encoder: cls_top is not supported with the fp8 forward / backward (desc.w8)");
+  NB_CHECK(!d->head_gate, NBEST_ERR_ARG, "encoder: cls_top is not supported with head_gate (the gate runs on the full-width context)");
+  NB_CHECK(!d->base_ids && !d->alpha, NBEST_ERR_ARG, "encoder: cls_top is not supported with interpolated embeddings (base_ids / alpha)");
+  NB_CHECK(!d->no_param_grad, NBEST_ERR_ARG, "encoder: cls_top is not supported with no_param_grad");
+  NB_CHECK(d->S >= 2, NBEST_ERR_SHAPE, "encoder: cls_top needs S >= 2 (got %d)", d->S);
+  return NBEST_OK;
+}
+static bool cls_layer_of(const nbest_encoder_desc* d, int l) { return d->cls_top && l == d->L - 1; }
+
+static std::vector<uint8_t> queue_skip(const nbest_encoder_desc* d, int layer_end) {
+  std::vector<uint8_t> s((size_t)4 * d->L, 0);
+  if (d->wgrad_skip_host) std::copy(d->wgrad_skip_host, d->wgrad_skip_host + (size_t)4 * d->L, s.begin());
+  if (d->cls_top && layer_end == d->L)
+    for (int j = 1; j < 4; ++j) s[(size_t)4 * (d->L - 1) + j] = 1;
+  return s;
 }
 
 struct Ptrs {
@@ -425,16 +445,55 @@
   return NBEST_OK;
 }
 
+static int layer_forward_cls(const Fwd& c, int l, const void* xin, void* xout, const LayerBufs& b) {
+  const nbest_encoder_desc* d = c.d;
+  const nbest_layer_offsets& o = d->layers_host[l];
+  const Ptrs& P = c.g.W;
+  const nbest_stream_t stream = c.g.stream;
+  hipStream_t st = (hipStream_t)stream;
+  const int H = d->H, F = d->F, dt = d->dtype, t = 4 * l;
+  const int64_t B = d->B, SH = (int64_t)d->S * H;
+  const uint32_t s0 = d->drop_stream_base + 1 + 4 * l;
+  const bool hdrop = d->hidden_drop > 0.f;
+  void* tmp = (char*)b.r2 + (size_t)B * H * P.esz;
+  const GemmOp wqkv = {xin, nullptr, t + 0, o.wqkv, t + 0, b.qkv, 3 * H, H, NBEST_EPI_BIAS, P.P(o.bqkv)};
+  RUN(layer_gemm(c.g, wqkv));
+  RUN(nbest_attention_cls_fwd_internal(b.qkv, SH * 3, (const char*)b.qkv + H * P.esz, 3 * H, c.key_mask, b.ctx, H, d->B, d->S, d->heads, 64, dt,
+                                       stream, d->attn_drop, d->seed, s0 + 0));
+  auto dense_drop_res = [&](const void* A, int64_t w_off, const float* bias, int64_t N, int64_t K, const void* R, int64_t ldr, uint32_t ds,
+                            void* out) -> int {
+    nbest_gemm_args g = gemm_nt(dt, A, P.W(w_off), hdrop ? tmp : out, B, N, K);
+    g.bias = bias;
+    if (hdrop) {
+      g.epilogue = NBEST_EPI_BIAS;
+      RUN(nbest_gemm(&g, stream));
+      return nbest_internal_rows_drop_res(tmp, N, R, ldr, out, N, B, (int)N, d->S, dt, d->hidden_drop, d->seed, ds, st);
+    }
+    g.epilogue = NBEST_EPI_BIAS_DROP_RES; g.R = R; g.ldr = ldr;
+    return nbest_gemm(&g, stream);
+  };
+  RUN(dense_drop_res(b.ctx, o.wo, P.P(o.bo), H, H, xin, SH, s0 + 1, b.r1));
+  RUN(nbest_internal_layernorm_fwd8(b.r1, P.P(o.ln1_g), P.P(o.ln1_b), b.x1, nullptr, b.st1, B, H, d->ln_eps, dt, stream, nullptr, nullptr));
+  nbest_gemm_args g = gemm_nt(dt, b.x1, P.W(o.w1), b.hact, B, F, H);
+  g.epilogue = NBEST_EPI_BIAS_GELU; g.bias = P.P(o.b1); g.U = b.u; g.ldu = F;
+  RUN(nbest_gemm(&g, stream));
+  RUN(dense_drop_res(b.hact, o.w2, P.P(o.b2), H, F, b.x1, H, s0 + 2, b.r2));
+  RUN(nbest_internal_layernorm_fwd8(b.r2, P.P(o.ln2_g), P.P(o.ln2_b), tmp, nullptr, b.st2, B, H, d->ln_eps, dt, stream, nullptr, nullptr));
+  return nbest_internal_rows_drop_res(tmp, H, nullptr, 0, xout, SH, B, H, 1, dt, 0.f, 0, 0, st);
+}
+
 }
 
 extern "C" size_t nbest_encoder_act_bytes(const nbest_encoder_desc* d) { return d ? act_layout(d, sizes(d)).total : 0; }
 
 extern "C" int nbest_encoder_act_view(const nbest_encoder_desc* d, void* act, int layer, void** qkv, float** lse) {
   RUN(check_desc(d));
+  RUN(check_cls_top(d));
   NB_CHECK(act && qkv && lse, NBEST_ERR_ARG, "encoder_act_view: null pointer");
   NB_CHECK(0 <= layer && layer < d->L, NBEST_ERR_ARG, "encoder_act_view: layer %d outside [0, L=%d)", layer, d->L);
   const ActLayout a = act_layout(d, sizes(d));
   NB_CHECK(layer >= a.K, NBEST_ERR_ARG, "encoder_act_view: layer %d < first_trainable %d (frozen layers are not stashed)", layer, a.K);
+  NB_CHECK(!cls_layer_of(d, layer), NBEST_ERR_ARG, "encoder_act_view: layer %d of a cls_top stash has no lse (its attention ran on the CLS rows only)", layer);
   const LayerBufs b = stashed_layer(d, a, act, layer);
   *qkv = b.qkv; *lse = b.lse;
   return NBEST_OK;
@@ -451,10 +510,12 @@
   NB_CHECK(d && d->B > 0 && d->S > 0 && d->L > 0 && d->H > 0 && d->F > 0, NBEST_ERR_ARG, "encoder_wgrad_plan: bad descriptor");
   NB_CHECK(first_trainable(d) <= layer_begin && layer_begin <= layer_end && layer_end <= d->L, NBEST_ERR_ARG, "encoder_wgrad_plan: bad layer range");
   NB_CHECK(out || cap <= 0, NBEST_ERR_ARG, "encoder_wgrad_plan: null pointer");
+  RUN(check_cls_top(d));
   const WgradMode wm = wgrad_mode(d);
   std::vector<int32_t> v = {wm.mode, wm.gl + wm.sets, -1, 0};
   if (wm.sets > 0) {
-    const WinPlan wp = window_plan(d, layer_begin, layer_end, d->wgrad_skip_host, d->no_param_grad != 0, true, wm.sets);
+    const std::vector<uint8_t> qskip = queue_skip(d, layer_end);
+    const WinPlan wp = window_plan(d, layer_begin, layer_end, qskip.data(), d->no_param_grad != 0, true, wm.sets);
     v[2] = wp.peel_layer; v[3] = (int32_t)wp.launches.size();
     for (const WinLaunch& w : wp.launches) {
       v.insert(v.end(), {w.after_layer, w.tiles, w.n});
@@ -469,6 +530,7 @@
                                      const int64_t* seg, const int64_t* pos, const uint8_t* key_mask, void* act, size_t act_bytes,
                                      void* ws, size_t ws_bytes, void** hidden_out, nbest_stream_t stream) {
   RUN(check_desc(d));
+  RUN(check_cls_top(d));
   NB_CHECK(wts && prm && ids && pos && key_mask && act, NBEST_ERR_ARG, "encoder_forward: null pointer");
   const Sizes z = sizes(d);
   const ActLayout a = act_layout(d, z);
@@ -497,7 +559,8 @@
                            (hipStream_t)stream));
   for (int l = 0; l < d->L; ++l) {
     uint8_t* x8_next = (l + 1 < d->L) ? bufs(l + 1).x8 : nullptr;
-    RUN(layer_forward(c, l, X(l), X(l + 1), bufs(l), x8_next, nullptr));
+    if (cls_layer_of(d, l)) RUN(layer_forward_cls(c, l, X(l), X(l + 1), bufs(l)));
+    else RUN(layer_forward(c, l, X(l), X(l + 1), bufs(l), x8_next, nullptr));
   }
   if (hidden_out) *hidden_out = X(d->L);
   return NBEST_OK;
@@ -517,6 +580,7 @@
                                       void* act, size_t act_bytes, void* dhidden, void* ws, size_t ws_bytes, int accumulate,
                                       int layer_begin, int layer_end, int with_embeddings, nbest_stream_t stream) {
   RUN(check_desc(d));
+  RUN(check_cls_top(d));
   NB_CHECK(0 <= layer_begin && layer_begin <= layer_end && layer_end <= d->L, NBEST_ERR_ARG, "encoder_backward: bad layer range");
   const bool npg = d->no_param_grad != 0;
   NB_CHECK(!npg || (!with_embeddings && d->first_trainable == 0 && !d->no_input_grad && !d->w8), NBEST_ERR_ARG,
@@ -546,7 +610,9 @@
   auto X = [&](int l) { return (void*)(A + a.X + (size_t)(l - FT) * z.MH); };
   auto G = [&](int64_t off) { return grad + off; };
   auto GP = [&](int64_t off) -> float* { return npg ? nullptr : grad + off; };
-  auto skip = [&](int l, int j) -> bool { return npg || (d->wgrad_skip_host && d->wgrad_skip_host[4 * l + j]); };
+  const std::vector<uint8_t> qskip = queue_skip(d, layer_end);
+  auto skip = [&](int l, int j) -> bool { return npg || qskip[4 * l + j]; };
+  auto frozen = [&](int l, int j) -> bool { return npg || (d->wgrad_skip_host && d->wgrad_skip_host[4 * l + j]); };
   void* dA = dhidden; void* dR = W + w.dR;
   const bool hdrop = d->hidden_drop > 0.f;
   void* dRd = hdrop ? (void*)(W + w.dRd) : dR;
@@ -606,12 +672,12 @@
     return NBEST_OK;
   };
   nbest_gemm_args pend[8];
-  int n_pend = 0;
+  int n_pend = 0, cls_pair = 0;
   const int nl = layer_end - layer_begin;
   WinPlan wp;
   std::vector<nbest_gemm_args> wargs;
   if (window) {
-    wp = window_plan(d, layer_begin, layer_end, d->wgrad_skip_host, npg, true, wm.sets);
+    wp = window_plan(d, layer_begin, layer_end, qskip.data(), npg, true, wm.sets);
     wargs.resize((size_t)4 * nl);
   }
   size_t wi = 0;
@@ -634,40 +700,101 @@
       dRd2 = W + w.gset[gpos][0]; dBigL = W + w.gset[gpos][1]; dRd1 = W + w.gset[gpos][2]; dqkvL = W + w.gset[gpos][3];
       if (!hdrop) { dR2 = dRd2; dR1 = dRd1; }
     }
+    const bool cls = cls_layer_of(d, l);
+    if (cls) {
+      const size_t bh = (size_t)d->B * H * z.esz;
+      dR2 = W + w.dR; dR1 = W + w.dB1 + bh; dBigL = dBig;
+      dRd2 = hdrop ? (void*)(W + w.dRd) : dR2; dRd1 = hdrop ? (void*)(W + w.dRd + bh) : dR1;
+    }
     const WGrad wg[4] = {{dqkvL, X(l), dqkv8, b.x8, o.wqkv, 3 * H, H, t + 3, t + 0},
                          {dRd1, b.ctx, dRd8, b.ctx8, o.wo, H, H, t + 2, t + 1},
                          {dBigL, b.x1, dBig8, b.x18, o.w1, F, H, t + 1, t + 2},
                          {dRd2, b.hact, dRd8, b.h8, o.w2, H, F, t + 0, t + 3}};
+    auto cls_wgrad = [&](int j) -> int {
+      if (frozen(l, j)) return NBEST_OK;
+      nbest_gemm_args g = wgrad_args(dt, wg[j].rows, wg[j].cols, d->B);
+      g.A = wg[j].dY; g.B = wg[j].X; g.C = G(wg[j].w_off); g.accumulate = accumulate;
+      g.ws = slab; g.ws_bytes = w.slab_bytes;
+      return nbest_gemm(&g, stream);
+    };
+    auto cls_wgrads = [&]() -> int {
+      RUN(cls_wgrad(3));
+      RUN(cls_wgrad(2));
+      return cls_wgrad(1);
+    };
     if (!npg) nbest_internal_rowred_batch_begin();
-    RUN(nbest_internal_layernorm_bwd8(dA, b.r2, b.st2, P.P(o.ln2_g), dR2, (hdrop && !f8b) ? dRd2 : nullptr, GP(o.ln2_g), GP(o.ln2_b), GP(o.b2), M, H,
-                                      dt, accumulate, d->hidden_drop, d->seed, s0 + 2, red, w.red_bytes, stream, fg(dRd8, t + 0)));
-    GemmOp dw2 = {dRd2, dRd8, t + 0, o.w2, t + 3, f8b ? nullptr : dBigL, F, H, NBEST_EPI_DGELU};
-    dw2.U = b.u; dw2.colsum = GP(o.b1); dw2.C8 = dBig8; dw2.c_idx = t + 1;
-    RUN(layer_gemm(dg, dw2));
-    if (rec && !f8b) RUN(nbest_internal_amax_bf16(dBigL, M * F, GN(t + 1), st));
-    if (!deferred) RUN(wgrad(l, wg, 3, -1));
-    GemmOp dw1 = {dBigL, dBig8, t + 1, o.w1, t + 2, dB1, H, F, NBEST_EPI_RES};
-    dw1.R = dR2;
-    RUN(layer_gemm(dg, dw1));
-    if (!deferred) RUN(wgrad(l, wg, 2, -1));
-    RUN(nbest_internal_layernorm_bwd8(dB1, b.r1, b.st1, P.P(o.ln1_g), dR1, (hdrop && !f8b) ? dRd1 : nullptr, GP(o.ln1_g), GP(o.ln1_b), GP(o.bo), M, H,
-                                      dt, accumulate, d->hidden_drop, d->seed, s0 + 1, red2, w.red_bytes, stream, fg(dRd8, t + 2)));
-    const GemmOp dwo = {dRd1, dRd8, t + 2, o.wo, t + 1, dctx, H, H, NBEST_EPI_NONE};
-    RUN(layer_gemm(dg, dwo));
-    if (!paired && !deferred) RUN(wgrad(l, wg, 1, -1));
-    if (d->head_gate)
-      RUN(nbest_head_gate_bwd(b.ctx, dctx, d->head_gate + (int64_t)l * d->heads,
-                              d->head_gate_grad ? d->head_gate_grad + (int64_t)l * d->B * d->heads : nullptr, d->B, d->S, d->heads, 64, dt, stream));
-    RUN(nbest_internal_attention_bwd8(b.qkv, key_mask, b.ctx, dctx, b.lse, f8b ? nullptr : dqkvL, GP(o.bqkv), accumulate, red3, w.red_bytes, d->B, d->S,
-                                      d->heads, 64, dt, d->attn_drop, d->seed, s0 + 0, stream, fg(dqkv8, t + 3), b.keep));
-    if (input_grad) {
-      GemmOp dwqkv = {dqkvL, dqkv8, t + 3, o.wqkv, t + 0, dA, H, 3 * H, NBEST_EPI_RES};
-      dwqkv.R = dR1;
-      RUN(layer_gemm(dg, dwqkv));
+    if (cls) {
+      const int64_t Bn = d->B, SH = (int64_t)d->S * H;
+      const size_t bh = (size_t)Bn * H * z.esz, half = w.red_bytes / 2;
+      void* dAc = W + w.dR + bh;
+      GemmPass dgc = dg;
+      dgc.M = Bn; dgc.packed = nullptr;
+      const Fp8Grad nof8 = {nullptr, nullptr, nullptr};
+      RUN(nbest_internal_rows_drop_res(dA, SH, nullptr, 0, dAc, H, Bn, H, 1, dt, 0.f, 0, 0, st));
+      RUN(nbest_internal_layernorm_bwd8(dAc, b.r2, b.st2, P.P(o.ln2_g), dR2, nullptr, G(o.ln2_g), G(o.ln2_b), hdrop ? nullptr : G(o.b2), Bn, H, dt,
+                                        accumulate, 0.f, 0, 0, red, half, stream, nof8));
+      if (hdrop) {
+        RUN(nbest_internal_rows_drop_res(dR2, H, nullptr, 0, dRd2, H, Bn, H, d->S, dt, d->hidden_drop, d->seed, s0 + 2, st));
+        RUN(nbest_colsum(dRd2, G(o.b2), Bn, H, H, dt, accumulate, (char*)red + half, half, stream));
+      }
+      GemmOp dw2 = {dRd2, nullptr, t + 0, o.w2, t + 3, dBigL, F, H, NBEST_EPI_DGELU};
+      dw2.U = b.u; dw2.colsum = G(o.b1);
+      RUN(layer_gemm(dgc, dw2));
+      GemmOp dw1 = {dBigL, nullptr, t + 1, o.w1, t + 2, dB1, H, F, NBEST_EPI_RES};
+      dw1.R = dR2;
+      RUN(layer_gemm(dgc, dw1));
+      RUN(nbest_internal_layernorm_bwd8(dB1, b.r1, b.st1, P.P(o.ln1_g), dR1, nullptr, G(o.ln1_g), G(o.ln1_b), hdrop ? nullptr : G(o.bo), Bn, H, dt,
+                                        accumulate, 0.f, 0, 0, red2, half, stream, nof8));
+      if (hdrop) {
+        RUN(nbest_internal_rows_drop_res(dR1, H, nullptr, 0, dRd1, H, Bn, H, d->S, dt, d->hidden_drop, d->seed, s0 + 1, st));
+        RUN(nbest_colsum(dRd1, G(o.bo), Bn, H, H, dt, accumulate, (char*)red2 + half, half, stream));
+      }
+      const GemmOp dwo = {dRd1, nullptr, t + 2, o.wo, t + 1, dctx, H, H, NBEST_EPI_NONE};
+      RUN(layer_gemm(dgc, dwo));
+      RUN(nbest_internal_attention_cls_bwd(b.qkv, key_mask, b.ctx, dctx, dqkvL, G(o.bqkv), accumulate, red3, w.red_bytes, d->B, d->S, d->heads, 64,
+                                           dt, d->attn_drop, d->seed, s0 + 0, stream));
+      if (input_grad) {
+        NB_CHECK(hipMemsetAsync(dctx, 0, (size_t)M * H * z.esz, st) == hipSuccess, NBEST_ERR_LAUNCH, "encoder_backward: memset failed");
+        RUN(nbest_internal_rows_drop_res(dR1, H, nullptr, 0, dctx, SH, Bn, H, 1, dt, 0.f, 0, 0, st));
+        GemmOp dwqkv = {dqkvL, nullptr, t + 3, o.wqkv, t + 0, dA, H, 3 * H, NBEST_EPI_RES};
+        dwqkv.R = dctx;
+        RUN(layer_gemm(dg, dwqkv));
+      }
+    } else {
+      RUN(nbest_internal_layernorm_bwd8(dA, b.r2, b.st2, P.P(o.ln2_g), dR2, (hdrop && !f8b) ? dRd2 : nullptr, GP(o.ln2_g), GP(o.ln2_b), GP(o.b2), M, H,
+                                        dt, accumulate, d->hidden_drop, d->seed, s0 + 2, red, w.red_bytes, stream, fg(dRd8, t + 0)));
+      GemmOp dw2 = {dRd2, dRd8, t + 0, o.w2, t + 3, f8b ? nullptr : dBigL, F, H, NBEST_EPI_DGELU};
+      dw2.U = b.u; dw2.colsum = GP(o.b1); dw2.C8 = dBig8; dw2.c_idx = t + 1;
+      RUN(layer_gemm(dg, dw2));
+      if (rec && !f8b) RUN(nbest_internal_amax_bf16(dBigL, M * F, GN(t + 1), st));
+      if (!deferred) RUN(wgrad(l, wg, 3, -1));
+      GemmOp dw1 = {dBigL, dBig8, t + 1, o.w1, t + 2, dB1, H, F, NBEST_EPI_RES};
+      dw1.R = dR2;
+      RUN(layer_gemm(dg, dw1));
+      if (!deferred) RUN(wgrad(l, wg, 2, -1));
+      RUN(nbest_internal_layernorm_bwd8(dB1, b.r1, b.st1, P.P(o.ln1_g), dR1, (hdrop && !f8b) ? dRd1 : nullptr, GP(o.ln1_g), GP(o.ln1_b), GP(o.bo), M, H,
+                                        dt, accumulate, d->hidden_drop, d->seed, s0 + 1, red2, w.red_bytes, stream, fg(dRd8, t + 2)));
+      const GemmOp dwo = {dRd1, dRd8, t + 2, o.wo, t + 1, dctx, H, H, NBEST_EPI_NONE};
+      RUN(layer_gemm(dg, dwo));
+      if (!paired && !deferred) RUN(wgrad(l, wg, 1, -1));
+      if (d->head_gate)
+        RUN(nbest_head_gate_bwd(b.ctx, dctx, d->head_gate + (int64_t)l * d->heads,
+                                d->head_gate_grad ? d->head_gate_grad + (int64_t)l * d->B * d->heads : nullptr, d->B, d->S, d->heads, 64, dt, stream));
+      RUN(nbest_internal_attention_bwd8(b.qkv, key_mask, b.ctx, dctx, b.lse, f8b ? nullptr : dqkvL, GP(o.bqkv), accumulate, red3, w.red_bytes, d->B, d->S,
+                                        d->heads, 64, dt, d->attn_drop, d->seed, s0 + 0, stream, fg(dqkv8, t + 3), b.keep));
+      if (input_grad) {
+        GemmOp dwqkv = {dqkvL, dqkv8, t + 3, o.wqkv, t + 0, dA, H, 3 * H, NBEST_EPI_RES};
+        dwqkv.R = dR1;
+        RUN(layer_gemm(dg, dwqkv));
+      }
     }
     if (window) {
       for (int j = 0; j < 4; ++j)
         if (!skip(l, j)) wargs[(size_t)4 * (layer_end - 1 - l) + j] = wgrad_args_of(wg + j);
+      if (cls) {
+        pair_begin();
+        RUN(cls_wgrads());
+      }
       if (l == wp.peel_layer) {
         pair_begin();
         if (!paired) RUN(wgrad_launch(l, wg, 1, -1));
@@ -688,10 +815,19 @@
       pair_end();
       if (l == layer_begin)
         for (; pairs_used < nl; ++pairs_used) { stamp(0); stamp(1); }
+    } else if (!grouped && cls) {
+      stamp(0); RUN(cls_wgrad(3)); stamp(1);
+      stamp(0); RUN(cls_wgrad(2)); stamp(1);
+      if (!paired) { stamp(0); RUN(cls_wgrad(1)); stamp(1); }
+      stamp(0);
+      if (paired) RUN(cls_wgrad(1));
+      RUN(wgrad_launch(l, wg, 0, -1));
+      stamp(1);
     } else if (!grouped) {
       RUN(wgrad(l, wg, 0, paired ? 1 : -1));
     } else if (group_ends && gpos + 1 < gl && d->wgrad_group != NBEST_WGRAD_GROUP_ALWAYS) {
       stamp(0);
+      if (cls) RUN(cls_wgrads());
       RUN(wgrad_launch(l, wg, 3, -1));
       RUN(wgrad_launch(l, wg, 2, -1));
       if (!paired) RUN(wgrad_launch(l, wg, 1, -1));
@@ -700,12 +836,19 @@
     } else {
       for (int j = 0; j < 4; ++j)
         if (!skip(l, j)) pend[n_pend++] = wgrad_args_of(wg + j);
+      if (cls && !group_ends) {
+        stamp(0);
+        RUN(cls_wgrads());
+        stamp(1);
+        cls_pair = 1;
+      }
       if (group_ends) {
         stamp(0);
+        if (cls) RUN(cls_wgrads());
         if (n_pend) RUN(nbest_wgrad_group(pend, n_pend, stream));
         stamp(1);
-        for (int i = 0; i < gpos; ++i) { stamp(0); stamp(1); }
-        n_pend = 0;
+        for (int i = 0; i < gpos - cls_pair; ++i) { stamp(0); stamp(1); }
+        n_pend = 0; cls_pair = 0;
       }
     }
     if (!npg) RUN(nbest_internal_rowred_batch_flush(st));
@@ -786,7 +929,7 @@
   g.lda = SH; g.epilogue = NBEST_EPI_BIAS; g.bias = P.P(o.bqkv);
   RUN(nbest_gemm(&g, stream));
   if (cls_attn) RUN(nbest_internal_attention_cls_probs(q, H, kv, 2 * H, key_mask, probs(l), d->S, d->B, d->S, d->heads, 64, dt, stream));
-  RUN(nbest_attention_cls_fwd_internal(q, H, kv, 2 * H, key_mask, cctx, H, d->B, d->S, d->heads, 64, dt, stream));
+  RUN(nbest_attention_cls_fwd_internal(q, H, kv, 2 * H, key_mask, cctx, H, d->B, d->S, d->heads, 64, dt, stream, 0.f, 0, 0));
   if (d->head_gate) RUN(nbest_head_gate_fwd(cctx, H, cctx, H, d->head_gate + (int64_t)l * d->heads, B, d->heads, 64, dt, stream));
   g = gemm_nt(dt, cctx, P.W(o.wo), cr, B, H, H);
   g.epilogue = NBEST_EPI_BIAS_DROP_RES; g.bias = P.P(o.bo); g.R = xin; g.ldr = SH;
diff --git a/n-best-asr-transformer_amd/csrc/internal.h b/n-best-asr-transformer_amd/csrc/internal.h
--- a/n-best-asr-transformer_amd/csrc/internal.h
+++ b/n-best-asr-transformer_amd/csrc/internal.h
@@ -16,6 +16,8 @@
                                   int accumulate, float drop_p, uint64_t seed, uint32_t drop_stream, void* ws,
                                   size_t ws_bytes, nbest_stream_t stream, Fp8Grad f8);
 int nbest_internal_partial_rows_sum(const float* part, int nrows, int N, float* out, int accumulate, hipStream_t st);
+int nbest_internal_rows_drop_res(const void* x, int64_t ldx, const void* R, int64_t ldr, void* y, int64_t ldy, int64_t rows, int N,
+                                 int64_t row_mul, int dtype, float drop_p, uint64_t seed, uint32_t drop_stream, hipStream_t st);
 void nbest_internal_rowred_batch_begin();
 void nbest_internal_rowred_batch_abort();
 int nbest_internal_rowred_batch_flush(hipStream_t st);
@@ -29,7 +31,11 @@
                                   const uint32_t* keep);
 size_t nbest_internal_attention_keep_bytes(int B, int S, int heads);
 int nbest_attention_cls_fwd_internal(const void* q, int64_t ldq, const void* kv, int64_t ldkv, const uint8_t* key_mask, void* ctx,
-                                     int64_t ldctx, int B, int S, int heads, int d, int dtype, nbest_stream_t stream);
+                                     int64_t ldctx, int B, int S, int heads, int d, int dtype, nbest_stream_t stream, float drop_p,
+                                     uint64_t seed, uint32_t drop_stream);
+int nbest_internal_attention_cls_bwd(const void* qkv, const uint8_t* key_mask, const void* ctx, const void* dctx, void* dqkv, float* dbias,
+                                     int accumulate, void* ws, size_t ws_bytes, int B, int S, int heads, int d, int dtype, float drop_p,
+                                     uint64_t seed, uint32_t drop_stream, nbest_stream_t stream);
 int nbest_internal_attention_cls_probs(const void* q, int64_t ldq, const void* kv, int64_t ldkv, const uint8_t* key_mask, float* probs,
                                        int64_t ldp, int B, int S, int heads, int d, int dtype, nbest_stream_t stream);
 
diff --git a/n-best-asr-transformer_amd/csrc/norm_embed.hip b/n-best-asr-transformer_amd/csrc/norm_embed.hip
--- a/n-best-asr-transformer_amd/csrc/norm_embed.hip
+++ b/n-best-asr-transformer_amd/csrc/norm_embed.hip
@@ -1385,6 +1385,44 @@
   return NBEST_OK;
 }
 
+namespace {
+template <typename T>
+__global__ __launch_bounds__(256) void rows_drop_res_kernel(const T* __restrict__ x, int64_t ldx, const T* __restrict__ R, int64_t ldr,
+                                                            T* __restrict__ y, int64_t ldy, int64_t rows, int N, int64_t row_mul,
+                                                            DropCfg drop) {
+  const int half = N >> 1;
+  const int64_t i = (int64_t)blockIdx.x * blockDim.x + threadIdx.x;
+  if (i >= rows * half) return;
+  const int64_t r = i / half;
+  const int c = (int)(i - r * half) * 2;
+  float v0 = (float)x[r * ldx + c], v1 = (float)x[r * ldx + c + 1];
+  if (drop.thr16) {
+    const uint32_t k = nb_keep2(drop, (uint32_t)(r * row_mul * N + c));
+    v0 = (k & 1u) ? v0 * drop.scale : 0.f;
+    v1 = (k & 2u) ? v1 * drop.scale : 0.f;
+  }
+  if (R) { v0 += (float)R[r * ldr + c]; v1 += (float)R[r * ldr + c + 1]; }
+  y[r * ldy + c] = (T)v0;
+  y[r * ldy + c + 1] = (T)v1;
+}
+}
+
+int nbest_internal_rows_drop_res(const void* x, int64_t ldx, const void* R, int64_t ldr, void* y, int64_t ldy, int64_t rows, int N,
+                                 int64_t row_mul, int dtype, float drop_p, uint64_t seed, uint32_t drop_stream, hipStream_t st) {
+  NB_CHECK(x && y && rows > 0 && N > 0 && N % 2 == 0 && ldx >= N && ldy >= N && (!R || ldr >= N), NBEST_ERR_ARG, "rows_drop_res: bad arguments");
+  const DropCfg d = make_drop(drop_p, seed, drop_stream);
+  NB_CHECK(d.thr16 == 0 || rows * row_mul * N < ((int64_t)1 << 32), NBEST_ERR_SHAPE, "rows_drop_res: dropout counter overflow");
+  const int64_t n = rows * (N >> 1);
+  const unsigned grid = (unsigned)((n + 255) / 256);
+  if (dtype == NBEST_F32)
+    rows_drop_res_kernel<float><<<grid, 256, 0, st>>>((const float*)x, ldx, (const float*)R, ldr, (float*)y, ldy, rows, N, row_mul, d);
+  else if (dtype == NBEST_BF16)
+    rows_drop_res_kernel<bf16><<<grid, 256, 0, st>>>((const bf16*)x, ldx, (const bf16*)R, ldr, (bf16*)y, ldy, rows, N, row_mul, d);
+  else NB_CHECK(false, NBEST_ERR_DTYPE, "rows_drop_res: bad dtype %d", dtype);
+  NB_LAUNCH_CHECK();
+  return NBEST_OK;
+}
+
 extern "C" int nbest_cast_f32_to_bf16(const float* src, void* dst, int64_t n, nbest_stream_t stream) {
   NB_CHECK(src && dst && n >= 0, NBEST_ERR_ARG, "cast: bad arguments");
   if (n == 0) return NBEST_OK;
diff --git a/n-best-asr-transformer_amd/hipabi.py b/n-best-asr-transformer_amd/hipabi.py
--- a/n-best-asr-transformer_amd/hipabi.py
+++ b/n-best-asr-transformer_amd/hipabi.py
@@ -84,7 +84,7 @@
                 ("w8", C.c_void_p), ("w8_inv_scale", C.c_void_p), ("w8t", C.c_void_p), ("gamax_prev", C.c_void_p),
                 ("gamax_new", C.c_void_p), ("fp8_bwd", C.c_int32), ("pad2", C.c_int32),
                 ("wpk", C.c_void_p), ("wpkt", C.c_void_p), ("w8p", C.c_void_p), ("w8tp", C.c_void_p),
-                ("word_perm", C.c_void_p), ("aamax_prev", C.c_void_p), ("aamax_new", C.c_void_p), ("fp8_act", C.c_int32), ("pad4", C.c_int32),
+                ("word_perm", C.c_void_p), ("aamax_prev", C.c_void_p), ("aamax_new", C.c_void_p), ("fp8_act", C.c_int32), ("cls_top", C.c_int32),
                 ("first_trainable", C.c_int32), ("no_input_grad", C.c_int32), ("wgrad_skip_host", C.c_void_p),
                 ("head_gate", C.c_void_p), ("head_gate_grad", C.c_void_p),
                 ("base_ids", C.c_void_p), ("alpha", C.c_void_p), ("no_param_grad", C.c_int32), ("pad5", C.c_int32)]
diff --git a/n-best-asr-transformer_amd/model.py b/n-best-asr-transformer_amd/model.py
--- a/n-best-asr-transformer_amd/model.py
+++ b/n-best-asr-transformer_amd/model.py
@@ -91,7 +91,7 @@
         self.B, self.S = B, S
 
 
-class _PassRecord(collections.namedtuple("_PassRecord", "ps slot inputs perm hidden gen plan")):
+class _PassRecord(collections.namedtuple("_PassRecord", "ps slot inputs perm hidden gen plan cls_top")):
     __slots__ = ()
 
     @property
@@ -198,7 +198,8 @@
         self.dropout = float(dropout)
         self.device = torch.device(device)
         self.wgrad_group = int(wgrad_group)
-        self.arena = ParamArena(cfg, labels, self.device, compute_dtype)
+        self.cls_top = True
+        self.arena =ParamArena(cfg, labels, self.device, compute_dtype)
         self.fp8_forward = bool(fp8_forward)
         self.fp8_backward = self.fp8_forward if fp8_backward is None else bool(fp8_backward)
         self._gamax_valid = False
@@ -372,7 +373,7 @@
             seg = seg.contiguous()
         return ids, seg, pos, mask
 
-    def _encode(self, slot, ids, seg, train, perm=None, plan=None):
+    def _encode(self, slot, ids, seg, train, perm=None, plan=None, full_top=False):
         B, S = ids.shape
         ps = self._pass(B, S, slot, plan.first_trainable if plan is not None else 0)
         ids, seg, pos, mask = inputs = self._inputs(ids, seg)
@@ -382,6 +383,7 @@
         d.seed = self._step_seed()
         self._set_head_gate(d)
         self._set_weights(d, "forward")
+        d.cls_top = int(not full_top and self._cls_top_ok(train, S, plan))
         act, ws = self._stash[slot][:ps.act_bytes], self._ws
         out = C.c_void_p()
         hb.check(hb.lib().nbest_encoder_forward(C.byref(d), hb.ptr(self.arena.weights), hb.ptr(self.arena.p), hb.ptr(ids),
@@ -392,7 +394,10 @@
         M, H = B * S, self.cfg.hidden_size
         esz = 2 if self.compute_dtype == torch.bfloat16 else 4
         hidden = act[off:off + M * H * esz].view(self.compute_dtype).view(M, H)
-        return _PassRecord(ps, slot, inputs, perm, hidden, self._stash_gen[slot], plan)
+        return _PassRecord(ps, slot, inputs, perm, hidden, self._stash_gen[slot], plan, bool(d.cls_top))
+
+    def _cls_top_ok(self, train, S, plan):
+        return self.cls_top and train and S >= 2 and not self.fp8_forward and self._head_mask is None
 
     def _packed_bf16_ok(self):
         return self.arena.wpk is not None and not self.arena.w16t_stale
@@ -433,6 +438,7 @@
         ps, d = rec.ps, rec.ps.desc
         B, S, H = ps.B, ps.S, self.cfg.hidden_size
         self._set_weights(d, "backward")
+        d.cls_top = int(rec.cls_top)
         dh = self._grow(vars(self), "_dh", B * S * H, self.compute_dtype)[:B * S * H].view(B * S, H)
         dh = hb.cls_grad_scatter(dcls, B, S, H, self.compute_dtype, out=dh)
         ids, seg, pos, mask = rec.inputs
@@ -475,11 +481,12 @@
                             seed=self._step_seed(), drop_stream=900, dWh=dWh, dbh=dbh, ws=ws, soft=soft)
 
     def _passes_and_heads(self, ids, seg, trans_ids, trans_seg, train, from_transcript=False, labels_f=None, need_grad=False,
-                          accumulate=False, perm=None, trans_perm=None, ws=None, plan=None, after_asr=None, distill=None, rdrop=None):
-        ra = self._encode(0, ids, seg, train, perm, plan)
+                          accumulate=False, perm=None, trans_perm=None, ws=None, plan=None, after_asr=None, distill=None, rdrop=None,
+                          full_top=False):
+        ra = self._encode(0, ids, seg, train, perm, plan, full_top)
         if after_asr is not None:
             after_asr(ra)
-        rt = None if trans_ids is None else self._encode(1, trans_ids, trans_seg, train, trans_perm, plan)
+        rt = None if trans_ids is None else self._encode(1, trans_ids, trans_seg, train, trans_perm, plan, full_top)
         r = rt if from_transcript else ra
         return ra, rt, self._heads(r.hidden, r.ps.S, labels_f, need_grad, train, accumulate, ws, distill, rdrop)
 
@@ -515,7 +522,7 @@
         after = (lambda rec: attns.extend(self._attention_maps(rec))) if return_attns else None
         ra, rt, (top, bott, fin, _, _, _, _) = self._passes_and_heads(input_ids, seg_ids, trans_input_ids, trans_seg_ids, self.training,
                                                                       from_transcript=classifier_input_type == "transcript",
-                                                                      after_asr=after)
+                                                                      after_asr=after, full_top=return_attns)
         self._end_of_step(False, advance=False)
         trans_cls = None if rt is None else rt.cls.float()
         if return_attns:
```

Result: faster. 13300 (median of 6 runs) (+4.1%).
